# Da-Tsuchi/KLab_MultiModalModel

Measured on AMD Instinct MI355X. Metric: caption-train samples/sec (224px img, 64-tok tgt), higher is better.
Workload: dtype bf16; 1 GPU; BASELINE configs[1]: Swin-V2(C=64,(2,2,6,2),224,w7) frozen + T5-small, fwd+bwd+Adam, T5 dropout 0.1 on, random-init weights; global_batch=64, per_gpu_batch=64, src_len=9, tgt_len=64, parallelism=dp1, hipgraph=False, optimizer=klab.optim.FusedAdam (Adam update of ref/train.py:28, one kernel)

## Files before the change

### klab_multimodalmodel_amd/csrc/common.h

```cpp
#pragma once
#include <hip/hip_runtime.h>
#include <stdint.h>
#include <stdlib.h>

#define KLAB_OK 0
#define KLAB_ERR_UNSUPPORTED (-2)
#define KLAB_ERR_BADARG (-3)

#define KLAB_F32 0
#define KLAB_BF16 1

typedef __bf16 bf16_t;
typedef __attribute__((ext_vector_type(8))) __bf16 bf16x8;
typedef __attribute__((ext_vector_type(4))) __bf16 bf16x4;
typedef __attribute__((ext_vector_type(4))) float f32x4;

#define KLAB_LAUNCH_CHECK()                          \
  do {                                               \
    hipError_t e__ = hipGetLastError();              \
    if (e__ != hipSuccess) return (int)e__;          \
  } while (0)

namespace klab {

inline bool env_on(const char* name) {
  const char* v = getenv(name);
  return !v || atoi(v) != 0;
}

int ensure_dyn_lds(const void* kernel, size_t bytes);

template <typename T> struct TypeTag;
template <> struct TypeTag<float> { static constexpr int id = KLAB_F32; };
template <> struct TypeTag<bf16_t> { static constexpr int id = KLAB_BF16; };

__device__ __forceinline__ float to_f32(float x) { return x; }
__device__ __forceinline__ float to_f32(bf16_t x) { return (float)x; }
template <typename T> __device__ __forceinline__ T from_f32(float x);
template <> __device__ __forceinline__ float from_f32<float>(float x) { return x; }
template <> __device__ __forceinline__ bf16_t from_f32<bf16_t>(float x) { return (bf16_t)x; }

__device__ __forceinline__ uint32_t mix32(uint32_t x) {
  x ^= x >> 16; x *= 0x85EBCA6Bu; x ^= x >> 13; x *= 0xC2B2AE35u; x ^= x >> 16;
  return x;
}
struct DropCtx {
  uint32_t key;
  uint32_t thresh;
  float scale;
  bool on;
};
__device__ __forceinline__ DropCtx make_drop(const uint32_t* seed_dev, uint32_t tag, float p) {
  DropCtx d;
  d.on = (p > 0.f) && (seed_dev != nullptr);
  d.key = 0; d.thresh = 0; d.scale = 1.f;
  if (d.on) {
    d.key = mix32(seed_dev[0] * 0x9E3779B1u + tag * 0x7FEB352Du + 0x165667B1u);
    double t = (double)p * 4294967296.0;
    d.thresh = t >= 4294967295.0 ? 0xFFFFFFFFu : (uint32_t)t;
    d.scale = 1.f / (1.f - p);
  }
  return d;
}
__device__ __forceinline__ float drop_mult(const DropCtx& d, uint64_t idx) {
  if (!d.on) return 1.f;
  uint32_t h = mix32((uint32_t)idx * 0x9E3779B1u + d.key);
  const uint32_t hi = (uint32_t)(idx >> 32);
  if (hi) h = mix32(h ^ (hi * 0x85EBCA77u + 0x27D4EB2Fu));
  return h < d.thresh ? 0.f : d.scale;
}
__device__ __forceinline__ DropCtx drop_slab(DropCtx d, uint32_t slab) {
  if (d.on) d.key = mix32(d.key ^ (slab * 0x85EBCA77u + 0x27D4EB2Fu));
  return d;
}
__device__ __forceinline__ float drop_mult32(const DropCtx& d, uint32_t off) {
  if (!d.on) return 1.f;
  return mix32(off * 0x9E3779B1u + d.key) < d.thresh ? 0.f : d.scale;
}
__device__ __forceinline__ float drop_mult32_nb(const DropCtx& d, uint32_t off) {
  return mix32(off * 0x9E3779B1u + d.key) < d.thresh ? 0.f : d.scale;
}

__device__ __forceinline__ float wave_sum(float v) {
#pragma unroll
  for (int o = 32; o > 0; o >>= 1) v += __shfl_xor(v, o, 64);
  return v;
}
__device__ __forceinline__ float wave_max(float v) {
#pragma unroll
  for (int o = 32; o > 0; o >>= 1) v = fmaxf(v, __shfl_xor(v, o, 64));
  return v;
}
template <int G> __device__ __forceinline__ float group_sum(float v) {
#pragma unroll
  for (int o = G / 2; o > 0; o >>= 1) v += __shfl_xor(v, o, 64);
  return v;
}
template <int G> __device__ __forceinline__ float group_max(float v) {
#pragma unroll
  for (int o = G / 2; o > 0; o >>= 1) v = fmaxf(v, __shfl_xor(v, o, 64));
  return v;
}

__device__ __forceinline__ float gelu_erf(float x) { return 0.5f * x * (1.f + erff(x * 0.70710678118654752440f)); }
__device__ __forceinline__ float erf_fast(float x) {
  const float ax = fabsf(x);
  const float t = __frcp_rn(fmaf(0.3275911f, ax, 1.f));
  float pl = fmaf(1.061405429f, t, -1.453152027f);
  pl = fmaf(pl, t, 1.421413741f);
  pl = fmaf(pl, t, -0.284496736f);
  pl = fmaf(pl, t, 0.254829592f);
  const float y = 1.f - pl * t * __expf(-ax * ax);
  return copysignf(y, x);
}
typedef __attribute__((ext_vector_type(2))) float f32x2;
template <typename V> __device__ __forceinline__ V gelu_poly(V x) {
  V s = x * x;
  s = __builtin_elementwise_min(s, V(20.48f));
  V q = V(7.318504830e-11f);
  q = q * s + V(-7.769299870e-09f);
  q = q * s + V(3.614930506e-07f);
  q = q * s + V(-9.785327165e-06f);
  q = q * s + V(1.732400560e-04f);
  q = q * s + V(-2.146258019e-03f);
  q = q * s + V(1.943818480e-02f);
  q = q * s + V(-1.324543953e-01f);
  q = q * s + V(7.977233529e-01f);
  V e = __builtin_elementwise_max(__builtin_elementwise_min(x * q, V(1.f)), V(-1.f));
  const V hx = x * V(0.5f);
  return hx * e + hx;
}
template <typename T> __device__ __forceinline__ float gelu_for(float x) {
  if constexpr (sizeof(T) == 2) return gelu_poly<float>(x);
  else return gelu_erf(x);
}
__device__ __forceinline__ float gelu_erf_grad(float x) {
  float cdf = 0.5f * (1.f + erff(x * 0.70710678118654752440f));
  float pdf = 0.39894228040143267794f * __expf(-0.5f * x * x);
  return cdf + x * pdf;
}

template <typename T> struct Vec16;
template <> struct Vec16<float> { typedef f32x4 type; static constexpr int N = 4; };
template <> struct Vec16<bf16_t> { typedef bf16x8 type; static constexpr int N = 8; };

}
```

### klab_multimodalmodel_amd/csrc/engine.cpp

```cpp
#include <hip/hip_runtime.h>
#include <math.h>
#include <stdio.h>
#include <string.h>

#include <string>
#include <vector>

#include "gemm_shared.h"
#include "klab_mm.h"

namespace {

#define RC(x)                 \
  do {                        \
    int rc__ = (x);           \
    if (rc__ != 0) return rc__; \
  } while (0)

struct ParamInfo {
  std::string name;
  std::vector<long> shape;
  long numel = 0;
  long grad_off = -1;
  long warena_off = -1;
  long farena_off = -1;
};

struct T5LayerIdx { int q, k, v, o, relb, ln0, cq, ck, cv, co, ln1, wi, wi1, wo, ln2; };
struct T5Idx { int shared, lm_head = -1, head = -1; std::vector<T5LayerIdx> enc, dec; int enc_final, dec_final; };
struct SwinBlockIdx { int ls, c0w, c0b, c2w, qw, qb, kw, vw, vb, pw, pb, ln1w, ln1b, f1w, f1b, f2w, f2b, ln2w, ln2b; };
struct SwinStageIdx { std::vector<SwinBlockIdx> blk; int redw, mnw, mnb; };
struct SwinIdx { int pew, peb, penw, penb; std::vector<SwinStageIdx> st; int lnw, lnb; };

struct T5LayerBufs {
  void *xn1, *qkv, *ctx; float *lse, *rstd1;
  void *xn2, *qc, *ctx2; float *lse2, *rstd2;
  void *xn3, *hmid; float* rstd3;
  void* ab;
};
struct T5StackBufs {
  std::vector<float*> h;
  std::vector<T5LayerBufs> L;
  void* out_t = nullptr; float* rstd_f = nullptr;
  float* bias = nullptr; float* dbias = nullptr; const int* bucket = nullptr;
  int M = 0, Lseq = 0;
};
inline bool swin_attn_on_image(int C) { return C == 64 || C == 128 || C == 256; }
struct SwinBlockBufs {
  float* x_in; void* xt_in;
  void *qkv, *ctx, *po; float *lse, *mean1, *rstd1; float* h1; void* h1t;
  void *z, *a, *fo; float *mean2, *rstd2; float* h2; void* h2t;
  float *bias, *table, *hidden;
  float* btab;
  float* bimg;
  int R, w, shift, H, C; long M;
};
struct SwinStageBufs { std::vector<SwinBlockBufs> blk; void *mg, *mo; float *mmean, *mrstd; float* xm; void* xmt; };

struct Bump {
  char* base; size_t off = 0;
  explicit Bump(void* b) : base((char*)b) {}
  void* take(size_t bytes) {
    off = (off + 255) & ~(size_t)255;
    void* p = base ? base + off : nullptr;
    off += bytes;
    return p;
  }
};

struct ProcSet {
  bool on = false;
  klab_logits_proc_cfg cfg{1.f};
  std::vector<int> table;
};
struct ForcedTable {
  const long long* tok = nullptr;
  long ld = 0;
  int n = 0;
};
struct AttnMaps {
  float* p = nullptr;
  size_t bytes = 0;
};
struct GenRun {
  klab_gen_cfg cfg{};
  ProcSet lp;
  ForcedTable forced;
  AttnMaps maps;
  int cur = 0;
};

}

struct klab_engine {
  klab_model_cfg cfg;
  std::vector<ParamInfo> P[3];
  SwinIdx si; T5Idx li, mi;
  long grad_elems[3] = {0, 0, 0};
  long seg_zero_off[3] = {0, 0, 0}, seg_zero_len[3] = {0, 0, 0};
  long seg_off[3] = {0, 0, 0}, seg_len[3] = {0, 0, 0};
  long warena_elems = 0, farena_elems = 0;
  long kvall_w_off = -1, kvall_g_off = -1;
  struct Bucket { long off, len; };
  std::vector<Bucket> buckets[3];
  std::vector<hipEvent_t> bucket_ev[3];
  bool bucket_ev_live[3] = {false, false, false};
  bool bucket_events_on = false;
  int pe_k0 = 0, pe_kp = 0;
  bool bound = false;
  int B = 0, Ls = 0, Lt = 0, Le = 0, Nimg = 0;
  size_t es = 4;
  std::vector<const float*> W[3];
  float* G[3] = {nullptr, nullptr, nullptr};
  void* warena = nullptr; float* farena = nullptr;
  bool fp8 = false;
  void* w8 = nullptr; float* wscale = nullptr; void* qdesc = nullptr; int n_qdesc = 0; long q_rows = 0;
  void* x8 = nullptr; float* xscale = nullptr; long x8_bytes = 0, xscale_rows = 0;
  void* x8s = nullptr; float* xscales = nullptr; long x8s_bytes = 0, xscales_rows = 0;
  const void* q8_src[2] = {nullptr, nullptr}; int q8_rows[2] = {0, 0}, q8_k[2] = {0, 0};
  void* cast_desc = nullptr; int n_cast = 0; long cast_total4 = 0;
  void* adam_desc = nullptr; int n_adam = 0; long adam_total4 = 0, adam_split4 = 0;
  void* af_desc = nullptr; int n_af = 0; long af_totals[4] = {0, 0, 0, 0};
  float* rms_part = nullptr; long rms_part_stride = 0; float** rms_dst_dev[2] = {nullptr, nullptr}; int rms_ncalls[2] = {0, 0};
  void* cast_desc_frozen = nullptr; int n_cast_frozen = 0; long cast_total4_frozen = 0;
  bool frozen_valid = false;
  void* fcast_desc = nullptr; int n_fcast = 0; long fcast_total4 = 0;
  uint32_t* seed_dev = nullptr; int* err_dev = nullptr;
  const int *enc_bucket = nullptr, *dec_bucket = nullptr, *lang_bucket = nullptr;
  std::vector<const float*> swin_coords; std::vector<const int*> swin_index; std::vector<int> swin_ntab;
  T5StackBufs lang, enc, dec;
  GenRun gen;
  ForcedTable forced_armed;
  AttnMaps attn_armed;
  void* kv_all = nullptr; void* dkv_all = nullptr;
  void* logits = nullptr; float *loss_row = nullptr, *inv_n = nullptr, *loss = nullptr;
  float *dh_a = nullptr, *dh_b = nullptr, *dxn = nullptr, *denc = nullptr;
  void *dctx = nullptr, *ds_ws = nullptr;
  void* dh_ff = nullptr;
  std::vector<void*> dy_pool, dhmid_pool, dqkv_pool, dqc_pool;
  std::vector<hipEvent_t> evpool; int ev_next = 0;
  void *cols = nullptr, *pe_out = nullptr; float *pe_mean = nullptr, *pe_rstd = nullptr; float* x0 = nullptr; void* x0t = nullptr;
  std::vector<SwinStageBufs> sw;
  float *sw_fmean = nullptr, *sw_frstd = nullptr;
  float *sdh_a = nullptr, *sdh_b = nullptr, *sdm = nullptr; void *sdy = nullptr, *sdctx = nullptr, *sdqkv = nullptr, *sda = nullptr;
  void* sattn_ws = nullptr; size_t sattn_ws_bytes = 0;
  float *sdbias = nullptr, *sdtable = nullptr, *sdbtab = nullptr;
  long sdb_stride = 0, sdt_stride = 0; size_t sdz_bytes = 0;
  void *sdyA[2] = {nullptr, nullptr}, *sdyB[2] = {nullptr, nullptr}, *sdaP[2] = {nullptr, nullptr}, *sdqkvP[2] = {nullptr, nullptr};
  hipEvent_t swin_done_ev[2] = {nullptr, nullptr};
  hipStream_t side = nullptr; hipEvent_t ev_fork = nullptr, ev_join = nullptr;
  hipEvent_t ev_zero = nullptr;
  bool seg1_zeroed = false;
  bool dbias_zeroed[2] = {false, false};
  bool denc_in_dxn = false;
  float* loss_out = nullptr;
  bool bias_ready[3] = {false, false, false};
  bool dec_embed_ready = false;
  bool inv_n_ready = false;
  bool kv_wgrad_done = false;
  hipStream_t own = nullptr; hipEvent_t ev_in = nullptr, ev_out = nullptr;
  bool use_graph = false;
  struct GraphSlot { hipGraphExec_t exec = nullptr; int uses = 0; bool failed = false; } gs[7];
  float* pixels_buf = nullptr; long long *src_buf = nullptr, *tgt_buf = nullptr; float* dloss_buf = nullptr;
  const float* pixels_cur = nullptr;
  uint32_t seed_base = 0; bool seed_set = false;
  bool probe_on = false;
  struct Probe { std::vector<hipEvent_t> a, b; std::vector<double> flops; int n = 0; } probe[2];
  float p_train = 0.f;
  const long long* last_tgt = nullptr;
};

namespace {

int add_param(std::vector<ParamInfo>& v, const std::string& name, std::vector<long> shape) {
  ParamInfo p;
  p.name = name; p.shape = shape; p.numel = 1;
  for (long s : shape) p.numel *= s;
  v.push_back(p);
  return (int)v.size() - 1;
}

void build_t5_params(const klab_t5_cfg& c, bool encoder_only, std::vector<ParamInfo>& v, T5Idx& ix) {
  const long d = c.d_model, inner = (long)c.n_heads * c.d_kv, ff = c.d_ff;
  ix.shared = add_param(v, "shared.weight", {c.vocab, d});
  ix.lm_head = (!encoder_only && !c.tie_lm_head) ? add_param(v, "lm_head.weight", {c.vocab, d}) : -1;
  ix.head = ix.lm_head >= 0 ? ix.lm_head : ix.shared;
  auto stack = [&](const char* pre, int nl, bool dec, std::vector<T5LayerIdx>& L, int& fin) {
    for (int i = 0; i < nl; ++i) {
      T5LayerIdx l;
      memset(&l, -1, sizeof(l));
      std::string bp = std::string(pre) + "block." + std::to_string(i) + ".";
      std::string ap = bp + "layer.0.SelfAttention.";
      l.q = add_param(v, ap + "q.weight", {inner, d});
      l.k = add_param(v, ap + "k.weight", {inner, d});
      l.v = add_param(v, ap + "v.weight", {inner, d});
      l.o = add_param(v, ap + "o.weight", {d, inner});
      if (i == 0) l.relb = add_param(v, ap + "relative_attention_bias.weight", {c.rel_buckets, c.n_heads});
      l.ln0 = add_param(v, bp + "layer.0.layer_norm.weight", {d});
      int li = 1;
      if (dec) {
        std::string cp = bp + "layer.1.EncDecAttention.";
        l.cq = add_param(v, cp + "q.weight", {inner, d});
        l.ck = add_param(v, cp + "k.weight", {inner, d});
        l.cv = add_param(v, cp + "v.weight", {inner, d});
        l.co = add_param(v, cp + "o.weight", {d, inner});
        l.ln1 = add_param(v, bp + "layer.1.layer_norm.weight", {d});
        li = 2;
      }
      std::string fp = bp + "layer." + std::to_string(li) + ".";
      if (c.ffn_gated) {
        l.wi = add_param(v, fp + "DenseReluDense.wi_0.weight", {ff, d});
        l.wi1 = add_param(v, fp + "DenseReluDense.wi_1.weight", {ff, d});
      } else {
        l.wi = add_param(v, fp + "DenseReluDense.wi.weight", {ff, d});
      }
      l.wo = add_param(v, fp + "DenseReluDense.wo.weight", {d, ff});
      l.ln2 = add_param(v, fp + "layer_norm.weight", {d});
      L.push_back(l);
    }
    fin = add_param(v, std::string(pre) + "final_layer_norm.weight", {d});
  };
  if (!encoder_only) stack("decoder.", c.n_dec_layers, true, ix.dec, ix.dec_final);
  stack("encoder.", c.n_layers, false, ix.enc, ix.enc_final);
}

void build_swin_params(const klab_swin_cfg& c, std::vector<ParamInfo>& v, SwinIdx& ix) {
  const long C0 = c.embed_dim;
  ix.pew = add_param(v, "embeddings.patch_embeddings.projection.weight", {C0, c.in_ch, c.patch, c.patch});
  ix.peb = add_param(v, "embeddings.patch_embeddings.projection.bias", {C0});
  ix.penw = add_param(v, "embeddings.norm.weight", {C0});
  ix.penb = add_param(v, "embeddings.norm.bias", {C0});
  for (int s = 0; s < c.n_stages; ++s) {
    SwinStageIdx st;
    const long C = C0 << s, H = c.heads[s], F = (long)c.mlp_ratio * C;
    for (int b = 0; b < c.depths[s]; ++b) {
      SwinBlockIdx k;
      memset(&k, -1, sizeof(k));
      std::string bp = "encoder.layers." + std::to_string(s) + ".blocks." + std::to_string(b) + ".";
      std::string sp = bp + "attention.self.";
      k.ls = add_param(v, sp + "logit_scale", {H, 1, 1});
      k.c0w = add_param(v, sp + "continuous_position_bias_mlp.0.weight", {512, 2});
      k.c0b = add_param(v, sp + "continuous_position_bias_mlp.0.bias", {512});
      k.c2w = add_param(v, sp + "continuous_position_bias_mlp.2.weight", {H, 512});
      k.qw = add_param(v, sp + "query.weight", {C, C});
      if (c.qkv_bias) k.qb = add_param(v, sp + "query.bias", {C});
      k.kw = add_param(v, sp + "key.weight", {C, C});
      k.vw = add_param(v, sp + "value.weight", {C, C});
      if (c.qkv_bias) k.vb = add_param(v, sp + "value.bias", {C});
      k.pw = add_param(v, bp + "attention.output.dense.weight", {C, C});
      k.pb = add_param(v, bp + "attention.output.dense.bias", {C});
      k.ln1w = add_param(v, bp + "layernorm_before.weight", {C});
      k.ln1b = add_param(v, bp + "layernorm_before.bias", {C});
      k.f1w = add_param(v, bp + "intermediate.dense.weight", {F, C});
      k.f1b = add_param(v, bp + "intermediate.dense.bias", {F});
      k.f2w = add_param(v, bp + "output.dense.weight", {C, F});
      k.f2b = add_param(v, bp + "output.dense.bias", {C});
      k.ln2w = add_param(v, bp + "layernorm_after.weight", {C});
      k.ln2b = add_param(v, bp + "layernorm_after.bias", {C});
      st.blk.push_back(k);
    }
    st.redw = st.mnw = st.mnb = -1;
    if (s < c.n_stages - 1) {
      std::string dp = "encoder.layers." + std::to_string(s) + ".downsample.";
      st.redw = add_param(v, dp + "reduction.weight", {2 * C, 4 * C});
      st.mnw = add_param(v, dp + "norm.weight", {2 * C});
      st.mnb = add_param(v, dp + "norm.bias", {2 * C});
    }
    ix.st.push_back(st);
  }
  const long Cl = C0 << (c.n_stages - 1);
  ix.lnw = add_param(v, "layernorm.weight", {Cl});
  ix.lnb = add_param(v, "layernorm.bias", {Cl});
}

inline long pad8(long n) { return (n + 7) & ~7L; }

void plan_arenas(klab_engine* e) {
  long w = 0, f = 0;
  auto putw = [&](std::vector<ParamInfo>& v, int i) { if (i >= 0) { v[i].warena_off = w; w += (v[i].numel + 15) & ~15L; } };
  auto t5 = [&](std::vector<ParamInfo>& v, T5Idx& ix, bool is_main) {
    putw(v, ix.head);
    for (auto& l : ix.dec) { putw(v, l.q); putw(v, l.k); putw(v, l.v); putw(v, l.o); putw(v, l.cq); putw(v, l.co); putw(v, l.wi); putw(v, l.wi1); putw(v, l.wo); }
    if (is_main && !ix.dec.empty()) {
      e->kvall_w_off = w;
      for (auto& l : ix.dec) { putw(v, l.ck); putw(v, l.cv); }
    }
    for (auto& l : ix.enc) { putw(v, l.q); putw(v, l.k); putw(v, l.v); putw(v, l.o); putw(v, l.wi); putw(v, l.wi1); putw(v, l.wo); }
  };
  t5(e->P[2], e->mi, true);
  {
    auto& v = e->P[1];
    for (auto& l : e->li.enc) { putw(v, l.q); putw(v, l.k); putw(v, l.v); putw(v, l.o); putw(v, l.wi); putw(v, l.wi1); putw(v, l.wo); }
  }
  {
    auto& v = e->P[0];
    {
      const klab_swin_cfg& sc = e->cfg.swin;
      e->pe_k0 = sc.in_ch * sc.patch * sc.patch;
      e->pe_kp = (e->cfg.dtype == KLAB_BF16 && sc.patch == 4) ? ((e->pe_k0 + 31) & ~31) : e->pe_k0;
      v[e->si.pew].warena_off = w;
      w += ((long)sc.embed_dim * e->pe_kp + 15) & ~15L;
    }
    for (auto& st : e->si.st) {
      for (auto& k : st.blk) {
        putw(v, k.qw); putw(v, k.kw); putw(v, k.vw); putw(v, k.pw); putw(v, k.f1w); putw(v, k.f2w);
        const long C = v[k.qw].shape[0];
        if (k.qb >= 0) { v[k.qb].farena_off = f; v[k.vb].farena_off = f + 2 * C; }
        f += 3 * C;
      }
      putw(v, st.redw);
    }
  }
// ... 330 lines not shown
}

static bool q8_room(const Ctx& c, long M, long K, bool& side) {
  klab_engine* e = c.e;
  side = c.s == e->side;
  if (!e->fp8 || c.dt != KLAB_BF16 || !fp8_weight_ok(K)) return false;
  return M * K <= (side ? e->x8s_bytes : e->x8_bytes) && M <= (side ? e->xscales_rows : e->xscale_rows);
}
int ln_fwd_for_linear(const Ctx& c, const void* y, const float* g, const float* b, const float* shortcut, float* out, void* outt, float* mean,
                      float* rstd, int M, int C, float eps) {
  klab_engine* e = c.e;
  bool side;
  if (q8_room(c, M, C, side)) {
    RC(klab_layernorm_fwd_q8(y, g, b, shortcut, out, outt, mean, rstd, side ? e->x8s : e->x8, side ? e->xscales : e->xscale, M, C, eps, c.ws()));
    e->q8_src[side] = outt; e->q8_rows[side] = M; e->q8_k[side] = C;
    return 0;
  }
  return klab_layernorm_fwd(y, c.dt, g, b, shortcut, out, outt, c.dt, mean, rstd, M, C, eps, 0, 0, 0, 0.f, nullptr, 0, c.ws());
}
int gelu_fwd_for_linear(const Ctx& c, const void* z, void* a, int M, int F) {
  klab_engine* e = c.e;
  bool side;
  if (F <= 4096 && !(F & 7) && q8_room(c, M, F, side)) {
    RC(klab_gelu_fwd_q8(z, a, side ? e->x8s : e->x8, side ? e->xscales : e->xscale, M, F, c.ws()));
    e->q8_src[side] = a; e->q8_rows[side] = M; e->q8_k[side] = F;
    return 0;
  }
  return klab_gelu_fwd(z, a, c.dt, (long)M * F, c.ws());
}

int linear_fwd(const Ctx& c, const void* x, int M, int K, long woffv, int N, void* y, long ldy, int ydt, const float* bias = nullptr,
               int act = 0) {
  klab_gemm_args g = G0(c, M, N, K, x, K, 1, woff(c, woffv), K, 1, y, ldy, ydt);
  g.bias = bias; g.act = act;
  return fwd_gemm(c, g, woffv);
}
int linear_dgrad(const Ctx& c, const void* dy, long lddy, int M, int N, long woffv, int K, void* dx, int dxdt) {
  klab_gemm_args g = G0(c, M, K, N, dy, lddy, 1, woff(c, woffv), K, 0, dx, K, dxdt);
  return klab_gemm(&g, c.ws());
}
int linear_wgrad(const Ctx& c, const void* dy, long lddy, const void* x, long ldx, int M, int N, int K, float* dw) {
  klab_gemm_args g = G0(c, N, K, M, dy, lddy, 0, x, ldx, 0, dw, K, KLAB_F32);
  g.accumulate = 1; g.atomic_ok = 1;
  return klab_gemm(&g, c.ws());
}

int t5_sublayer_out(const Ctx& c, const void* x, int M, int K, long woffv, int d, const float* resid, float* hout, float p, uint32_t tag) {
  klab_gemm_args g = G0(c, M, d, K, x, K, 1, woff(c, woffv), K, 1, hout, d, KLAB_F32);
  g.residual = resid; g.ldr = d; g.r_dtype = KLAB_F32;
  g.drop_p = p; g.seed_dev = c.e->seed_dev; g.drop_tag = tag;
  return fwd_gemm(c, g, woffv);
}

static bool attn_fused_on() {
  static const bool on = klab::env_on("KLAB_T5_ATTN_FUSED");
  return on;
}
static bool attn_bwd_fused_on() {
  static const bool on = klab::env_on("KLAB_T5_ATTN_BWD_FUSED");
  return on;
}

int t5_stack_forward(const Ctx& c, const klab_t5_cfg& cfg, const std::vector<ParamInfo>& P, const std::vector<const float*>& W,
                     const std::vector<T5LayerIdx>& L, int final_ln, T5StackBufs& s, bool dec, int stack_id, float p, int B,
                     const void* kv_all, int Lkv, long kv_ld, float* out_f32, int grp, int grp_stride, int off, float p_final) {
  const int d = cfg.d_model, H = cfg.n_heads, dk = cfg.d_kv, inner = H * dk, ff = cfg.d_ff;
  const int M = s.M, Lq = s.Lseq;
  const int relb = L[0].relb;
  if (c.e->bias_ready[stack_id]) c.e->bias_ready[stack_id] = false;
  else RC(klab_relbias_fwd(W[relb], s.bucket, s.bias, H, Lq, Lq, c.ws()));
  int j = 0;
  for (size_t i = 0; i < L.size(); ++i) {
    const T5LayerIdx& l = L[i];
    T5LayerBufs& b = s.L[i];
    {
      klab_attn_args a;
      memset(&a, 0, sizeof(a));
      a.dtype = c.dt; a.q = b.qkv; a.ldq = 3 * inner; a.k = eoff(c, b.qkv, inner); a.ldk = 3 * inner;
      a.v = eoff(c, b.qkv, 2 * inner); a.ldv = 3 * inner; a.bias = s.bias; a.causal = dec ? 1 : 0;
      a.ctx = b.ctx; a.ldo = inner; a.lse = b.lse; a.B = B; a.H = H; a.Lq = Lq; a.Lk = Lq; a.dk = dk;
      a.drop_p = p; a.seed_dev = c.e->seed_dev; a.drop_tag = tag_of(stack_id, (int)i, SITE_PROB);
      int frc = KLAB_ERR_UNSUPPORTED;
      if (attn_fused_on() && c.dt == KLAB_BF16 && !c.e->fp8 && Lq >= 32) {
        klab_attn_fused_args fa;
        memset(&fa, 0, sizeof(fa));
        fa.x = s.h[j]; fa.gamma = W[l.ln0]; fa.eps = cfg.ln_eps; fa.d_model = d; fa.w = woff(c, P[l.q].warena_off);
        fa.xn = b.xn1; fa.rstd = b.rstd1; fa.proj = b.qkv; fa.ldproj = 3 * inner; fa.cross = 0; fa.attn = a;
        frc = klab_t5_attn_fused_fwd(&fa, c.ws());
        if (frc != 0 && frc != KLAB_ERR_UNSUPPORTED) return frc;
      }
      if (frc != 0) {
        RC(rms_fwd_for_linear(c, s.h[j], W[l.ln0], b.xn1, b.rstd1, M, d, cfg.ln_eps));
        RC(linear_fwd(c, b.xn1, M, d, P[l.q].warena_off, 3 * inner, b.qkv, 3 * inner, c.dt));
        RC(klab_t5_attn_fwd(&a, c.ws()));
      }
    }
    RC(t5_sublayer_out(c, b.ctx, M, inner, P[l.o].warena_off, d, s.h[j], s.h[j + 1], p, tag_of(stack_id, (int)i, SITE_ATTN_OUT)));
    ++j;
    if (dec) {
      klab_attn_args a;
      memset(&a, 0, sizeof(a));
      a.dtype = c.dt; a.q = b.qc; a.ldq = inner;
      a.k = eoff(c, (void*)kv_all, (long)i * 2 * inner); a.ldk = kv_ld;
      a.v = eoff(c, (void*)kv_all, (long)i * 2 * inner + inner); a.ldv = kv_ld;
      a.bias = nullptr; a.causal = 0; a.ctx = b.ctx2; a.ldo = inner; a.lse = b.lse2;
      a.B = B; a.H = H; a.Lq = Lq; a.Lk = Lkv; a.dk = dk;
      a.drop_p = p; a.seed_dev = c.e->seed_dev; a.drop_tag = tag_of(stack_id, (int)i, SITE_XPROB);
      int frc = KLAB_ERR_UNSUPPORTED;
      if (attn_fused_on() && c.dt == KLAB_BF16 && !c.e->fp8 && Lq >= 32) {
        klab_attn_fused_args fa;
        memset(&fa, 0, sizeof(fa));
        fa.x = s.h[j]; fa.gamma = W[l.ln1]; fa.eps = cfg.ln_eps; fa.d_model = d; fa.w = woff(c, P[l.cq].warena_off);
        fa.xn = b.xn2; fa.rstd = b.rstd2; fa.proj = b.qc; fa.ldproj = inner; fa.cross = 1; fa.attn = a;
        frc = klab_t5_attn_fused_fwd(&fa, c.ws());
        if (frc != 0 && frc != KLAB_ERR_UNSUPPORTED) return frc;
      }
      if (frc != 0) {
        RC(rms_fwd_for_linear(c, s.h[j], W[l.ln1], b.xn2, b.rstd2, M, d, cfg.ln_eps));
        RC(linear_fwd(c, b.xn2, M, d, P[l.cq].warena_off, inner, b.qc, inner, c.dt));
        RC(klab_t5_attn_fwd(&a, c.ws()));
      }
      RC(t5_sublayer_out(c, b.ctx2, M, inner, P[l.co].warena_off, d, s.h[j], s.h[j + 1], p, tag_of(stack_id, (int)i, SITE_XOUT)));
      ++j;
    }
    RC(rms_fwd_for_linear(c, s.h[j], W[l.ln2], b.xn3, b.rstd3, M, d, cfg.ln_eps));
    if (cfg.ffn_gated) {
      RC(linear_fwd(c, b.xn3, M, d, P[l.wi].warena_off, 2 * ff, b.ab, 2 * ff, c.dt));
      RC(klab_geglu_fwd(b.ab, 2 * ff, b.hmid, ff, c.dt, M, ff, p, c.e->seed_dev, tag_of(stack_id, (int)i, SITE_MID), c.ws()));
    } else {
      klab_gemm_args g = G0(c, M, ff, d, b.xn3, d, 1, woff(c, P[l.wi].warena_off), d, 1, b.hmid, ff, c.dt);
      g.act = KLAB_ACT_RELU; g.drop_p = p; g.seed_dev = c.e->seed_dev; g.drop_tag = tag_of(stack_id, (int)i, SITE_MID);
      RC(fwd_gemm(c, g, P[l.wi].warena_off));
    }
    RC(t5_sublayer_out(c, b.hmid, M, ff, P[l.wo].warena_off, d, s.h[j], s.h[j + 1], p, tag_of(stack_id, (int)i, SITE_FFN_OUT)));
    ++j;
  }
  RC(klab_rmsnorm_fwd(s.h[j], W[final_ln], out_f32 ? nullptr : s.out_t, c.dt, out_f32, s.rstd_f, M, d, cfg.ln_eps, grp, grp_stride, off,
                      p_final, c.e->seed_dev, out_f32 ? tag_of(STACK_ENC, 0, SITE_IN) : tag_of(stack_id, 0, SITE_FINAL), c.ws()));
  return 0;
}

int side_after_main(const Ctx& c) {
  klab_engine* e = c.e;
  hipEvent_t ev = e->evpool[e->ev_next++ % e->evpool.size()];
  RC((int)hipEventRecord(ev, c.s));
  return (int)hipStreamWaitEvent(e->side, ev, 0);
}
int main_after_side(const Ctx& c) {
  klab_engine* e = c.e;
  hipEvent_t ev = e->evpool[e->ev_next++ % e->evpool.size()];
  RC((int)hipEventRecord(ev, e->side));
  return (int)hipStreamWaitEvent(c.s, ev, 0);
}
struct PendingWgrad { const void* dy; long lddy; const void* x; long ldx; int M, N, K; float* dw; };
struct WgradQueue {
  std::vector<PendingWgrad> q;
  int layers = 0;
  void push(const void* dy, long lddy, const void* x, long ldx, int M, int N, int K, float* dw) { q.push_back({dy, lddy, x, ldx, M, N, K, dw}); }
  int flush(const Ctx& c, bool now = true, bool* launched = nullptr) {
    if (launched) *launched = false;
    ++layers;
    if (q.empty()) { layers = 0; return 0; }
    if (!now && q.size() + 8 <= 32) return 0;
    if (launched) *launched = true;
    const bool large = layers >= 2;
    layers = 0;
    RC(side_after_main(c));
    Ctx cs{c.e, c.e->side, c.dt, c.es};
    std::vector<klab_gemm_args> gs;
    gs.reserve(q.size());
    for (const PendingWgrad& w : q) {
      klab_gemm_args g = G0(cs, w.N, w.K, w.M, w.dy, w.lddy, 0, w.x, w.ldx, 0, w.dw, w.K, KLAB_F32);
      g.accumulate = 1; g.atomic_ok = 1;
      gs.push_back(g);
    }
    klab_engine::Probe& pr = c.e->probe[1];
    const bool probe = c.e->probe_on && pr.n < (int)pr.a.size();
    if (probe) { klab::tl_launch_probe.a = pr.a[pr.n]; klab::tl_launch_probe.b = pr.b[pr.n]; }
    const int grc = klab_gemm_grouped_tiles(gs.data(), (int)gs.size(), large ? 1 : 0, cs.ws());
    RC(grc);
    if (probe) {
      if (klab::tl_launch_probe.a) klab::tl_launch_probe.a = nullptr;
      else {
        double fl = 0;
        for (const PendingWgrad& w : q) fl += 2.0 * w.M * (double)w.N * w.K;
        pr.flops[pr.n++] = fl;
      }
    }
    q.clear();
    return 0;
  }
};

int t5_stack_backward(const Ctx& c, const klab_t5_cfg& cfg, const std::vector<ParamInfo>& P, const std::vector<const float*>& W,
                      float* Gflat, const std::vector<T5LayerIdx>& L, int final_ln, T5StackBufs& s, bool dec, int stack_id, float p,
                      int B, const void* kv_all, void* dkv_all, int Lkv, long kv_ld, float** dh_out) {
  klab_engine* e = c.e;
  const int d = cfg.d_model, H = cfg.n_heads, dk = cfg.d_kv, inner = H * dk, ff = cfg.d_ff;
  const int M = s.M, Lq = s.Lseq;
  const int nsub = dec ? 3 : 2;
  int j = nsub * (int)L.size();
  float* dh_cur = e->dh_a;
  float* dh_oth = e->dh_b;
  auto G = [&](int pi) { return Gflat + P[pi].grad_off; };
  const float inv_keep = p > 0.f ? 1.f / (1.f - p) : 1.f;
  int dy_i = 0, deferred = 0;
  WgradQueue wq;
  const int stk = dec ? 1 : 0;
  const bool part_ok = Gflat == e->G[2] && e->rms_part && d <= 1024 && (long)klab_rmsnorm_part_rows(M) * d <= e->rms_part_stride;
  int rms_calls = 0;
  auto rms_bwd = [&](const float* dyin, const float* x, const float* w, const float* rstd, const float* dres, float* dx, void* dxt, int pidx,
                     float p_y, uint32_t tag_y, float p_prev, uint32_t tag_prev) -> int {
    if (part_ok)
      return klab_rmsnorm_bwd_part(dyin, x, w, rstd, dres, dx, dxt, c.dt, e->rms_part + (long)(rms_calls++) * e->rms_part_stride, M, d, 0, 0, 0,
                                   p_y, tag_y, p_prev, tag_prev, e->seed_dev, c.ws());
    return klab_rmsnorm_bwd(dyin, x, w, rstd, dres, dx, dxt, c.dt, G(pidx), M, d, 0, 0, 0, p_y, tag_y, p_prev, tag_prev, e->seed_dev, c.ws());
  };
  auto next_dy = [&]() { return e->dy_pool[dy_i++ % e->dy_pool.size()]; };
  if (e->dbias_zeroed[stk]) e->dbias_zeroed[stk] = false;
  else RC(hipMemsetAsync(s.dbias, 0, (size_t)H * Lq * Lq * 4, c.s));
  void* dy = next_dy();
  bool dctx_ready = false;
  auto attn_bwd = [&](klab_attn_args& a, long wo_off) -> int {
    if (attn_bwd_fused_on() && c.dt == KLAB_BF16) {
      klab_attn_bwd_fused_args fb;
      memset(&fb, 0, sizeof(fb));
      fb.dy = dy; fb.lddy = d; fb.w = woff(c, wo_off); fb.d_model = d; fb.attn = a;
      const int frc = klab_t5_attn_bwd_fused(&fb, c.ws());
      if (frc != KLAB_ERR_UNSUPPORTED) return frc;
    }
    if (!dctx_ready) { RC(linear_dgrad(c, dy, d, M, d, wo_off, inner, e->dctx, c.dt)); dctx_ready = true; }
    return klab_t5_attn_bwd(&a, c.ws());
  };
  RC(rms_bwd(e->dxn, s.h[j], W[final_ln], s.rstd_f, nullptr, dh_cur, dy, final_ln, p, tag_of(stack_id, 0, SITE_FINAL), p,
             tag_of(stack_id, (int)L.size() - 1, SITE_FFN_OUT)));
  std::vector<int> pending_buckets;
  const int Ln = (int)L.size();
  std::vector<char> flush_at(Ln, 1);
  constexpr int GROUP_TILES = 90;
  static const bool group_on = klab::env_on("KLAB_WGRAD_GROUP_TILES");
  const bool kv_in_queue = dec && dkv_all && Gflat == e->G[2] && !e->use_graph && e->kvall_g_off >= 0;
  if (group_on && Ln >= 3 && Gflat == e->G[2] && !e->use_graph) {
    auto T2 = [](int n, int k) { return (long)((n + 255) / 256) * ((k + 255) / 256); };
    const long tl = T2(d, ff) + T2(cfg.ffn_gated ? 2 * ff : ff, d) + T2(d, inner) + T2(3 * inner, d) + (dec ? T2(d, inner) + T2(inner, d) + (kv_in_queue ? T2(2 * inner, d) : 0) : 0);
    const int per_group = (int)((GROUP_TILES + tl - 1) / tl), per_layer = dec ? 7 : 4;
    if (per_group >= 2) {
      const int body = Ln - 1;
      int ng = body / per_group;
      if (ng < 1) ng = 1;
      if (((body + ng - 1) / ng) * per_layer <= 32) {
        std::fill(flush_at.begin(), flush_at.end(), 0);
        int i = Ln - 1;
        for (int gi = 0; gi < ng; ++gi) { i -= body / ng + (gi < body % ng ? 1 : 0); flush_at[i + 1] = 1; }
        flush_at[0] = 1;
      }
    }
  }
  for (int i = (int)L.size() - 1; i >= 0; --i) {
    const T5LayerIdx& l = L[i];
    T5LayerBufs& b = s.L[i];
    void* dhmid = e->dhmid_pool[i];
    void* dqkv = e->dqkv_pool[i];
    --j;
    wq.push(dy, d, b.hmid, ff, M, d, ff, G(l.wo));
    if (cfg.ffn_gated) {
      RC(linear_dgrad(c, dy, d, M, d, P[l.wo].warena_off, ff, e->dh_ff, c.dt));
      RC(klab_geglu_bwd(e->dh_ff, ff, b.ab, 2 * ff, dhmid, 2 * ff, c.dt, M, ff, p, e->seed_dev, tag_of(stack_id, i, SITE_MID), c.ws()));
      wq.push(dhmid, 2 * ff, b.xn3, d, M, 2 * ff, d, G(l.wi));
      RC(linear_dgrad(c, dhmid, 2 * ff, M, 2 * ff, P[l.wi].warena_off, d, e->dxn, KLAB_F32));
    } else {
      {
        klab_gemm_args g = G0(c, M, ff, d, dy, d, 1, woff(c, P[l.wo].warena_off), ff, 0, dhmid, ff, c.dt);
        g.aux = b.hmid; g.ldaux = ff; g.aux_mode = KLAB_AUX_NONZERO; g.aux_scale = inv_keep;
        RC(klab_gemm(&g, c.ws()));
      }
      wq.push(dhmid, ff, b.xn3, d, M, ff, d, G(l.wi));
      RC(linear_dgrad(c, dhmid, ff, M, ff, P[l.wi].warena_off, d, e->dxn, KLAB_F32));
    }
    {
      const uint32_t tprev = dec ? tag_of(stack_id, i, SITE_XOUT) : tag_of(stack_id, i, SITE_ATTN_OUT);
      dy = next_dy();
      RC(rms_bwd(e->dxn, s.h[j], W[l.ln2], b.rstd3, dh_cur, dh_oth, dy, l.ln2, 0.f, 0, p, tprev));
      float* t = dh_cur; dh_cur = dh_oth; dh_oth = t;
    }
    if (dec) {
      --j;
      void* dqc = e->dqc_pool[i];
      wq.push(dy, d, b.ctx2, inner, M, d, inner, G(l.co));
      dctx_ready = false;
      klab_attn_args a;
      memset(&a, 0, sizeof(a));
      a.dtype = c.dt; a.q = b.qc; a.ldq = inner;
      a.k = eoff(c, (void*)kv_all, (long)i * 2 * inner); a.ldk = kv_ld;
      a.v = eoff(c, (void*)kv_all, (long)i * 2 * inner + inner); a.ldv = kv_ld;
      a.ctx = b.ctx2; a.ldo = inner; a.lse = b.lse2; a.B = B; a.H = H; a.Lq = Lq; a.Lk = Lkv; a.dk = dk;
      a.drop_p = p; a.seed_dev = e->seed_dev; a.drop_tag = tag_of(stack_id, i, SITE_XPROB);
      a.dctx = e->dctx; a.lddo = inner; a.dq = dqc; a.lddq = inner;
      a.dk_out = eoff(c, dkv_all, (long)i * 2 * inner); a.lddk = kv_ld;
      a.dv = eoff(c, dkv_all, (long)i * 2 * inner + inner); a.lddv = kv_ld;
      RC(attn_bwd(a, P[l.co].warena_off));
      if (kv_in_queue) {
        wq.push(eoff(c, dkv_all, (long)i * 2 * inner), kv_ld, e->enc.out_t, d, B * Lkv, 2 * inner, d, Gflat + e->kvall_g_off + (long)i * 2 * inner * d);
        e->kv_wgrad_done = true;
      }
      wq.push(dqc, inner, b.xn2, d, M, inner, d, G(l.cq));
      RC(linear_dgrad(c, dqc, inner, M, inner, P[l.cq].warena_off, d, e->dxn, KLAB_F32));
      dy = next_dy();
      RC(rms_bwd(e->dxn, s.h[j], W[l.ln1], b.rstd2, dh_cur, dh_oth, dy, l.ln1, 0.f, 0, p, tag_of(stack_id, i, SITE_ATTN_OUT)));
      float* t = dh_cur; dh_cur = dh_oth; dh_oth = t;
    }
    --j;
    wq.push(dy, d, b.ctx, inner, M, d, inner, G(l.o));
    dctx_ready = false;
    {
      klab_attn_args a;
      memset(&a, 0, sizeof(a));
      a.dtype = c.dt; a.q = b.qkv; a.ldq = 3 * inner; a.k = eoff(c, b.qkv, inner); a.ldk = 3 * inner;
      a.v = eoff(c, b.qkv, 2 * inner); a.ldv = 3 * inner; a.bias = s.bias; a.causal = dec ? 1 : 0;
      a.ctx = b.ctx; a.ldo = inner; a.lse = b.lse; a.B = B; a.H = H; a.Lq = Lq; a.Lk = Lq; a.dk = dk;
      a.drop_p = p; a.seed_dev = e->seed_dev; a.drop_tag = tag_of(stack_id, i, SITE_PROB);
      a.dctx = e->dctx; a.lddo = inner; a.dq = dqkv; a.lddq = 3 * inner;
      a.dk_out = eoff(c, dqkv, inner); a.lddk = 3 * inner; a.dv = eoff(c, dqkv, 2 * inner); a.lddv = 3 * inner;
      a.dbias = s.dbias;
      int arc = KLAB_ERR_UNSUPPORTED;
      if (c.dt == KLAB_BF16 && deferred == (int)L.size() - 1 - i) {
        a.ds_defer = 1;
        a.ds_ws = (char*)e->ds_ws + (size_t)deferred * B * H * Lq * ((Lq + 31) & ~31) * c.es;
        arc = attn_bwd(a, P[l.o].warena_off);
        if (arc == 0) ++deferred;
      }
      if (arc == KLAB_ERR_UNSUPPORTED) { a.ds_defer = 0; a.ds_ws = nullptr; arc = attn_bwd(a, P[l.o].warena_off); }
      RC(arc);
    }
    wq.push(dqkv, 3 * inner, b.xn1, d, M, 3 * inner, d, G(l.q));
    RC(linear_dgrad(c, dqkv, 3 * inner, M, 3 * inner, P[l.q].warena_off, d, e->dxn, KLAB_F32));
    {
      const bool first = (i == 0);
      if (!first) dy = next_dy();
      RC(rms_bwd(e->dxn, s.h[j], W[l.ln0], b.rstd1, dh_cur, dh_oth, first ? nullptr : dy, l.ln0, 0.f, 0, first ? 0.f : p,
                 first ? 0u : tag_of(stack_id, i - 1, SITE_FFN_OUT)));
      float* t = dh_cur; dh_cur = dh_oth; dh_oth = t;
    }
    bool launched = false;
    RC(wq.flush(c, flush_at[i] != 0, &launched));
    pending_buckets.push_back((int)L.size() - 1 - i);
    if (launched) {
      const int seg = dec ? 0 : 1;
      for (int bi : pending_buckets)
        if (e->bucket_events_on && Gflat == e->G[2] && !e->use_graph && bi < (int)e->bucket_ev[seg].size())
          RC((int)hipEventRecord(e->bucket_ev[seg][bi], e->side));
      pending_buckets.clear();
      if (i == 0 && e->bucket_events_on && Gflat == e->G[2] && !e->use_graph && (int)L.size() - 1 < (int)e->bucket_ev[seg].size())
        e->bucket_ev_live[seg] = true;
    }
  }
  if (part_ok && rms_calls) {
    if (rms_calls != e->rms_ncalls[stk]) return KLAB_ERR_BADARG;
    RC(klab_colpart_reduce(e->rms_part, e->rms_part_stride, klab_rmsnorm_part_rows(M), d, e->rms_dst_dev[stk], rms_calls, c.ws()));
  }
  if (deferred) RC(klab_dbias_reduce(e->ds_ws, c.dt, s.dbias, deferred * B, H, Lq, Lq, c.ws()));
  RC(klab_relbias_bwd(s.dbias, s.bucket, G(L[0].relb), H, Lq, Lq, cfg.rel_buckets, c.ws()));
  *dh_out = dh_cur;
  return 0;
}

int swin_forward(const Ctx& c, const float* pixels, float p_in, bool refresh_bias) {
  klab_engine* e = c.e;
  const klab_swin_cfg& s = e->cfg.swin;
  const auto& P = e->P[0];
  const auto& W = e->W[0];
  const int B = e->B, R0 = s.image_size / s.patch, K0 = s.in_ch * s.patch * s.patch, C0 = s.embed_dim;
  const long M0 = (long)B * R0 * R0;
  const int Kp = e->pe_kp;
  (void)K0;
  static const bool fused_pe = klab::env_on("KLAB_SWIN_FUSED_EMBED");
  int perc = KLAB_ERR_UNSUPPORTED;
  if (!e->cfg.train_swin && fused_pe && !e->fp8 && Kp >= 64)
    perc = klab_swin_patch_embed_fused(pixels, woff(c, P[e->si.pew].warena_off), Kp, W[e->si.peb], W[e->si.penw], W[e->si.penb], e->x0, e->x0t, c.dt,
                                       B, s.in_ch, s.image_size, s.patch, C0, s.ln_eps, c.ws());
  if (perc != 0 && perc != KLAB_ERR_UNSUPPORTED) return perc;
  if (perc != 0) {
  RC(klab_im2col_patch_ld(pixels, e->cols, c.dt, B, s.in_ch, s.image_size, s.patch, Kp, c.ws()));
  {
    klab_gemm_args g = G0(c, (int)M0, C0, Kp, e->cols, Kp, 1, woff(c, P[e->si.pew].warena_off), Kp, 1, e->pe_out, C0, c.dt);
    g.bias = W[e->si.peb];
    RC(klab_gemm(&g, c.ws()));
  }
  RC(klab_layernorm_fwd(e->pe_out, c.dt, W[e->si.penw], W[e->si.penb], nullptr, e->x0, e->x0t, c.dt, e->pe_mean, e->pe_rstd, (int)M0, C0,
                        s.ln_eps, 0, 0, 0, 0.f, nullptr, 0, c.ws()));
  }
  float* x = e->x0;
  void* xt = e->x0t;
  long bias_off = 0;
  for (int st = 0; st < s.n_stages; ++st) {
    SwinStageBufs& sb = e->sw[st];
    for (size_t k = 0; k < sb.blk.size(); ++k) {
      SwinBlockBufs& q = sb.blk[k];
      const SwinBlockIdx& ix = e->si.st[st].blk[k];
      const int C = q.C, M = (int)q.M, F = s.mlp_ratio * C, n = q.w * q.w;
      q.x_in = x; q.xt_in = xt;
      if (refresh_bias) {
        if (q.btab)
          RC(klab_swin_cpb_table(e->swin_coords[st], W[ix.c0w], W[ix.c0b], W[ix.c2w], q.table, q.hidden, q.btab, e->swin_ntab[st], q.H, 512,
                                 c.ws()));
        else
          RC(klab_swin_cpb_bias(e->swin_coords[st], e->swin_index[st], W[ix.c0w], W[ix.c0b], W[ix.c2w], q.table, q.hidden, q.bias,
                                e->swin_ntab[st], n, q.H, 512, c.ws()));
        if (q.bimg) RC(klab_swin_bias_image(q.bias, q.bimg, q.R, q.w, q.shift, q.H, c.ws()));
      }
      const float* qkvb = ix.qb >= 0 ? e->farena + bias_off : nullptr;
      bias_off += 3 * C;
      int qrc = KLAB_ERR_UNSUPPORTED;
      if (q.bimg)
        qrc = klab_swin_qkv_attn_fused_img(xt, woff(c, P[ix.qw].warena_off), qkvb, q.ctx, q.bimg, W[ix.ls], c.dt, B, q.R, q.w, q.shift, q.H, C,
                                           c.ws());
      else if (!e->cfg.train_swin && q.bias)
        qrc = klab_swin_qkv_attn_fused(xt, woff(c, P[ix.qw].warena_off), qkvb, q.ctx, q.bias, W[ix.ls], c.dt, B, q.R, q.w, q.shift, q.H, C,
                                       c.ws());
      if (qrc != 0 && qrc != KLAB_ERR_UNSUPPORTED) return qrc;
      if (qrc != 0) {
        RC(linear_fwd(c, xt, M, C, P[ix.qw].warena_off, 3 * C, q.qkv, 3 * C, c.dt, qkvb));
        klab_swin_attn_args a;
        memset(&a, 0, sizeof(a));
        a.dtype = c.dt; a.qkv = q.qkv; a.ctx = q.ctx; a.bias = q.bias; a.bias_table = q.btab; a.logit_scale = W[ix.ls]; a.lse = q.lse;
        a.B = B; a.R = q.R; a.w = q.w; a.shift = q.shift; a.H = q.H; a.C = C;
        a.bwd_ws = e->sattn_ws; a.bwd_ws_bytes = e->sattn_ws_bytes;
        a.v_bias = qkvb ? qkvb + 2 * C : nullptr;
        RC(klab_swin_attn_fwd(&a, c.ws()));
      }
      int prc = KLAB_ERR_UNSUPPORTED;
      if (!e->cfg.train_swin)
        prc = klab_swin_proj_ln_fused(q.ctx, x, woff(c, P[ix.pw].warena_off), W[ix.pb], W[ix.ln1w], W[ix.ln1b], q.h1, q.h1t, c.dt, M, C, s.ln_eps,
                                      c.ws());
      if (prc != 0 && prc != KLAB_ERR_UNSUPPORTED) return prc;
      static const bool fused_lin_ln = klab::env_on("KLAB_SWIN_FUSED_LIN_LN");
      const bool wide_ln = !e->cfg.train_swin && !e->fp8 && fused_lin_ln;
      if (prc != 0 && wide_ln) {
        prc = klab_swin_linear_ln_fused(q.ctx, x, woff(c, P[ix.pw].warena_off), W[ix.pb], W[ix.ln1w], W[ix.ln1b], q.h1, q.h1t, c.dt, M, C, C,
                                        s.ln_eps, c.ws());
        if (prc != 0 && prc != KLAB_ERR_UNSUPPORTED) return prc;
      }
      if (prc != 0) {
        RC(linear_fwd(c, q.ctx, M, C, P[ix.pw].warena_off, C, q.po, C, c.dt, W[ix.pb]));
        RC(ln_fwd_for_linear(c, q.po, W[ix.ln1w], W[ix.ln1b], x, q.h1, q.h1t, q.mean1, q.rstd1, M, C, s.ln_eps));
      }
      if (e->cfg.train_swin) {
        RC(linear_fwd(c, q.h1t, M, C, P[ix.f1w].warena_off, F, q.z, F, c.dt, W[ix.f1b]));
        RC(gelu_fwd_for_linear(c, q.z, q.a, M, F));
      } else {
        const int frc = klab_swin_mlp_fused(q.h1t, q.h1, woff(c, P[ix.f1w].warena_off), W[ix.f1b], woff(c, P[ix.f2w].warena_off), W[ix.f2b],
                                            W[ix.ln2w], W[ix.ln2b], q.h2, q.h2t, c.dt, M, C, s.ln_eps, c.ws());
        if (frc == 0) { x = q.h2; xt = q.h2t; continue; }
        if (frc != KLAB_ERR_UNSUPPORTED) return frc;
        RC(linear_fwd(c, q.h1t, M, C, P[ix.f1w].warena_off, F, q.a, F, c.dt, W[ix.f1b], KLAB_ACT_GELU));
      }
      int f2rc = KLAB_ERR_UNSUPPORTED;
      if (wide_ln)
        f2rc = klab_swin_linear_ln_fused(q.a, q.h1, woff(c, P[ix.f2w].warena_off), W[ix.f2b], W[ix.ln2w], W[ix.ln2b], q.h2, q.h2t, c.dt, M, F, C,
                                         s.ln_eps, c.ws());
      if (f2rc != 0 && f2rc != KLAB_ERR_UNSUPPORTED) return f2rc;
      if (f2rc != 0) {
        RC(linear_fwd(c, q.a, M, F, P[ix.f2w].warena_off, C, q.fo, C, c.dt, W[ix.f2b]));
        RC(ln_fwd_for_linear(c, q.fo, W[ix.ln2w], W[ix.ln2b], q.h1, q.h2, q.h2t, q.mean2, q.rstd2, M, C, s.ln_eps));
      }
      x = q.h2; xt = q.h2t;
    }
    if (st < s.n_stages - 1) {
      const int R = R0 >> st, C = C0 << st;
      const long M2 = (long)B * (R / 2) * (R / 2);
      RC(klab_merge_gather(x, sb.mg, c.dt, B, R, C, c.ws()));
      RC(linear_fwd(c, sb.mg, (int)M2, 4 * C, P[e->si.st[st].redw].warena_off, 2 * C, sb.mo, 2 * C, c.dt));
      RC(klab_layernorm_fwd(sb.mo, c.dt, W[e->si.st[st].mnw], W[e->si.st[st].mnb], nullptr, sb.xm, sb.xmt, c.dt, sb.mmean, sb.mrstd, (int)M2,
                            2 * C, s.ln_eps, 0, 0, 0, 0.f, nullptr, 0, c.ws()));
      x = sb.xm; xt = sb.xmt;
    }
  }
  const int Cl = C0 << (s.n_stages - 1);
  RC(klab_layernorm_fwd(x, KLAB_F32, W[e->si.lnw], W[e->si.lnb], nullptr, e->enc.h[0], nullptr, c.dt, e->sw_fmean, e->sw_frstd,
                        B * e->Nimg, Cl, s.ln_eps, e->Nimg, e->Le, 0, p_in, e->seed_dev, tag_of(STACK_ENC, 0, SITE_IN), c.ws()));
  return 0;
}

int swin_backward(const Ctx& c, const float* dh0, float p_in);

}

extern "C" int klab_sizeof_t5_cfg(void) { return (int)sizeof(klab_t5_cfg); }
// ... 32 lines not shown
}

extern "C" void klab_engine_destroy(klab_engine* e) {
  if (!e) return;
  drain_engine(e);
  for (auto& g : e->gs) if (g.exec) { hipGraphExecDestroy(g.exec); g.exec = nullptr; }
  if (e->ev_fork) hipEventDestroy(e->ev_fork);
  if (e->ev_join) hipEventDestroy(e->ev_join);
  if (e->ev_zero) hipEventDestroy(e->ev_zero);
  if (e->ev_in) hipEventDestroy(e->ev_in);
  if (e->ev_out) hipEventDestroy(e->ev_out);
  for (auto ev : e->evpool) if (ev) hipEventDestroy(ev);
  for (auto& v : e->bucket_ev) for (auto ev : v) if (ev) hipEventDestroy(ev);
  for (auto ev : e->swin_done_ev) if (ev) hipEventDestroy(ev);
  for (auto& pr : e->probe) {
    for (auto ev : pr.a) if (ev) hipEventDestroy(ev);
    for (auto ev : pr.b) if (ev) hipEventDestroy(ev);
  }
  if (e->side) hipStreamDestroy(e->side);
  if (e->own) hipStreamDestroy(e->own);
  delete e;
}

extern "C" int klab_engine_num_params(const klab_engine* e, int model) {
  if (!e || model < 0 || model > 2) return -1;
  return (int)e->P[model].size();
}

extern "C" int klab_engine_param_info(const klab_engine* e, int model, int i, char* name, int name_cap, long* shape4, int* ndim,
                                      long* grad_off) {
  if (!e || model < 0 || model > 2 || i < 0 || i >= (int)e->P[model].size()) return KLAB_ERR_BADARG;
  const ParamInfo& p = e->P[model][i];
  if (name && name_cap > 0) { strncpy(name, p.name.c_str(), name_cap - 1); name[name_cap - 1] = 0; }
  if (ndim) *ndim = (int)p.shape.size();
  if (shape4) for (size_t k = 0; k < 4; ++k) shape4[k] = k < p.shape.size() ? p.shape[k] : 1;
  if (grad_off) *grad_off = p.grad_off;
  return 0;
}

extern "C" long klab_engine_grad_elems(const klab_engine* e, int model) { return (e && model >= 0 && model <= 2) ? e->grad_elems[model] : -1; }

extern "C" int klab_engine_segment(const klab_engine* e, int seg, int* model, long* off, long* len) {
  if (!e || seg < 0 || seg > 2) return KLAB_ERR_BADARG;
  if (model) *model = seg == 2 ? 0 : 2;
  if (off) *off = e->seg_off[seg];
  if (len) *len = e->seg_len[seg];
  return 0;
}

extern "C" int klab_engine_num_buckets(const klab_engine* e, int segment) {
  if (!e || segment < 0 || segment > 2) return -1;
  return (int)e->buckets[segment].size();
}
extern "C" int klab_engine_bucket(const klab_engine* e, int segment, int i, long* off, long* len) {
  if (!e || segment < 0 || segment > 2 || i < 0 || i >= (int)e->buckets[segment].size()) return KLAB_ERR_BADARG;
  if (off) *off = e->buckets[segment][i].off;
  if (len) *len = e->buckets[segment][i].len;
  return KLAB_OK;
}
extern "C" int klab_engine_set_bucket_events(klab_engine* e, int on) {
  if (!e) return KLAB_ERR_BADARG;
  e->bucket_events_on = on != 0;
  if (!on) for (auto& b : e->bucket_ev_live) b = false;
  return KLAB_OK;
}
extern "C" int klab_engine_bucket_wait(klab_engine* e, int segment, int i, void* stream) {
  if (!e || !e->bound || segment < 0 || segment > 2 || i < 0 || i >= (int)e->bucket_ev[segment].size()) return KLAB_ERR_BADARG;
  if (!e->bucket_ev_live[segment]) return KLAB_ERR_UNSUPPORTED;
  return (int)hipStreamWaitEvent((hipStream_t)stream, e->bucket_ev[segment][i], 0);
}

extern "C" size_t klab_engine_workspace_bytes(klab_engine* e, int B, int Ls, int Lt) {
  if (!e || B <= 0 || Ls <= 0 || Lt <= 0) return 0;
  klab_engine tmp;
  tmp.cfg = e->cfg;
  for (int m = 0; m < 3; ++m) tmp.P[m].resize(e->P[m].size());
  tmp.warena_elems = e->warena_elems; tmp.farena_elems = e->farena_elems; tmp.fp8 = e->fp8;
  return plan_workspace(&tmp, nullptr, B, Ls, Lt);
}

extern "C" int klab_engine_bind(klab_engine* e, int B, int Ls, int Lt, void* workspace, size_t ws_bytes, const void* const* swin_params,
                                const void* const* lang_params, const void* const* main_params, float* main_grads, float* swin_grads,
                                const int* lang_bucket, const int* enc_bucket, const int* dec_bucket, const void* const* swin_coords,
                                const void* const* swin_index, void* stream) {
  if (!e || !workspace || !swin_params || !lang_params || !main_params || !main_grads) return KLAB_ERR_BADARG;
  if (e->cfg.train_swin && !swin_grads) return KLAB_ERR_BADARG;
  uint32_t carry[3] = {0, 0, 0};
  bool carry_rng = false;
  if (e->bound) {
    e->bound = false;
    drain_engine(e);
    if (e->seed_set && e->seed_dev) carry_rng = hipMemcpy(carry, e->seed_dev, sizeof(carry), hipMemcpyDeviceToHost) == hipSuccess;
  }
  const size_t need = plan_workspace(e, workspace, B, Ls, Lt);
  if (need > ws_bytes) return KLAB_ERR_BADARG;
  const void* const* src[3] = {swin_params, lang_params, main_params};
  for (int m = 0; m < 3; ++m) {
    e->W[m].resize(e->P[m].size());
    for (size_t i = 0; i < e->P[m].size(); ++i) {
      e->W[m][i] = (const float*)src[m][i];
      if (!e->W[m][i]) return KLAB_ERR_BADARG;
    }
  }
  e->G[0] = swin_grads; e->G[2] = main_grads;
  e->lang_bucket = lang_bucket; e->enc_bucket = enc_bucket; e->dec_bucket = dec_bucket;
  e->lang.bucket = lang_bucket; e->enc.bucket = enc_bucket; e->dec.bucket = dec_bucket;
  const klab_swin_cfg& s = e->cfg.swin;
  e->swin_coords.resize(s.n_stages); e->swin_index.resize(s.n_stages); e->swin_ntab.resize(s.n_stages);
  const int R0 = s.image_size / s.patch;
  for (int st = 0; st < s.n_stages; ++st) {
    e->swin_coords[st] = (const float*)swin_coords[st];
    e->swin_index[st] = (const int*)swin_index[st];
    const int R = R0 >> st, w = R < s.window ? R : s.window;
    if (w <= 0) return KLAB_ERR_UNSUPPORTED;
    e->swin_ntab[st] = (2 * w - 1) * (2 * w - 1);
  }
  hipStream_t hs = (hipStream_t)stream;
  for (int grp = 0; grp < 2; ++grp) {
    std::vector<long> d;
    long pre = 0; int n = 0;
    for (int m = 0; m < 3; ++m) {
      const bool frozen = (m == 1) || (m == 0 && !e->cfg.train_swin);
      if (frozen != (grp == 1)) continue;
      for (size_t i = 0; i < e->P[m].size(); ++i) {
        const ParamInfo& p = e->P[m][i];
        if (p.warena_off < 0) continue;
        if (p.numel % 4) return KLAB_ERR_UNSUPPORTED;
        if (m == 0 && (int)i == e->si.pew && e->pe_kp != e->pe_k0) {
          if (e->pe_k0 % 4) return KLAB_ERR_UNSUPPORTED;
          for (int r = 0; r < e->cfg.swin.embed_dim; ++r) {
            d.push_back((long)(e->W[m][i] + (long)r * e->pe_k0)); d.push_back(p.warena_off + (long)r * e->pe_kp); d.push_back(pre);
            pre += e->pe_k0 / 4; ++n;
          }
          continue;
        }
        d.push_back((long)e->W[m][i]); d.push_back(p.warena_off); d.push_back(pre);
        pre += p.numel / 4; ++n;
      }
    }
    const size_t grp_cap = e->P[0].size() + e->P[1].size() + e->P[2].size() + e->cfg.swin.embed_dim + 1;
    void* dst = grp == 0 ? e->cast_desc : (void*)((char*)e->cast_desc + sizeof(long) * 3 * grp_cap);
    if (grp == 1) { e->cast_desc_frozen = dst; e->n_cast_frozen = n; e->cast_total4_frozen = pre; }
    if (n == 0) { if (grp == 0) { e->n_cast = 0; e->cast_total4 = 0; } continue; }
    hipError_t er0 = hipMemcpyAsync(dst, d.data(), d.size() * sizeof(long), hipMemcpyHostToDevice, hs);
    if (er0 != hipSuccess) return (int)er0;
    er0 = hipStreamSynchronize(hs);
    if (er0 != hipSuccess) return (int)er0;
    if (grp == 1) continue;
    e->n_cast = n; e->cast_total4 = pre;
  }
  e->frozen_valid = false;
  e->seg1_zeroed = e->dbias_zeroed[0] = e->dbias_zeroed[1] = e->denc_in_dxn = false;
  e->bias_ready[0] = e->bias_ready[1] = e->bias_ready[2] = e->dec_embed_ready = e->inv_n_ready = e->kv_wgrad_done = false;
  e->loss_out = nullptr;
  e->forced_armed = ForcedTable();
  e->attn_armed = AttnMaps();
  e->gen.maps = AttnMaps();
  if (e->pe_kp != e->pe_k0)
    RC((int)hipMemsetAsync((char*)e->warena + (size_t)e->P[0][e->si.pew].warena_off * e->es, 0,
                           (size_t)e->cfg.swin.embed_dim * e->pe_kp * e->es, hs));
  {
    std::vector<long> d;
    long pre = 0; int n = 0;
    for (size_t i = 0; i < e->P[0].size(); ++i) {
      const ParamInfo& p = e->P[0][i];
      if (p.farena_off < 0) continue;
      if (p.numel % 4) return KLAB_ERR_UNSUPPORTED;
      d.push_back((long)e->W[0][i]); d.push_back(p.farena_off); d.push_back(pre);
      pre += p.numel / 4; ++n;
    }
    e->n_fcast = n; e->fcast_total4 = pre;
    RC((int)hipMemsetAsync(e->farena, 0, (size_t)e->farena_elems * 4, hs));
    if (n) {
      hipError_t er = hipMemcpyAsync(e->fcast_desc, d.data(), d.size() * sizeof(long), hipMemcpyHostToDevice, hs);
      if (er != hipSuccess) return (int)er;
      er = hipStreamSynchronize(hs);
      if (er != hipSuccess) return (int)er;
    }
  }
  if (e->fp8) {
    std::vector<long> d;
    long row0 = 0; int n = 0;
    for (int m = 0; m < 3; ++m)
      for (size_t i = 0; i < e->P[m].size(); ++i) {
        const ParamInfo& p = e->P[m][i];
        if (p.warena_off < 0 || p.shape.empty() || (m == 0 && (int)i == e->si.pew)) continue;
        const long rows = p.shape[0], K = p.numel / rows;
        if (!fp8_weight_ok(K) || (p.warena_off & 15)) continue;
        d.push_back(p.warena_off); d.push_back(rows); d.push_back(K); d.push_back(row0);
        row0 += rows; ++n;
      }
    e->n_qdesc = n; e->q_rows = row0;
    if (n) {
      hipError_t er = hipMemcpyAsync(e->qdesc, d.data(), d.size() * sizeof(long), hipMemcpyHostToDevice, hs);
      if (er != hipSuccess) return (int)er;
      er = hipStreamSynchronize(hs);
      if (er != hipSuccess) return (int)er;
    }
  }
  std::vector<long> adam_tab;
  {
    std::vector<long> d;
    long pre = 0; int n = 0;
    bool ok = true;
    for (int seg = 0; seg < 2 && ok; ++seg) {
      if (seg == 1) e->adam_split4 = pre;
      for (size_t i = 0; i < e->P[2].size(); ++i) {
        const ParamInfo& p = e->P[2][i];
        if (p.grad_off < 0 || (p.grad_off >= e->seg_off[1]) != (seg == 1)) continue;
        if (p.numel % 4 || (p.grad_off & 3) || (p.warena_off >= 0 && (p.warena_off & 3))) { ok = false; break; }
        d.push_back((long)e->W[2][i]); d.push_back(p.grad_off); d.push_back(p.warena_off); d.push_back(pre);
        pre += p.numel / 4; ++n;
      }
    }
    e->n_adam = ok ? n : 0; e->adam_total4 = pre;
    if (e->n_adam) {
      hipError_t er = hipMemcpyAsync(e->adam_desc, d.data(), d.size() * sizeof(long), hipMemcpyHostToDevice, hs);
      if (er != hipSuccess) return (int)er;
    }
    adam_tab.swap(d);
  }
  {
    std::vector<long> rows, cols, idx;
    std::vector<int> fact;
    for (int seg = 0; seg < 2; ++seg)
      for (size_t i = 0; i < e->P[2].size(); ++i) {
        const ParamInfo& p = e->P[2][i];
        if (p.grad_off < 0 || (p.grad_off >= e->seg_off[1]) != (seg == 1)) continue;
        const long c = p.shape.empty() ? 1 : p.shape.back();
        fact.push_back(p.shape.size() >= 2); rows.push_back(p.shape.size() >= 2 ? p.numel / c : 1);
        cols.push_back(p.shape.size() >= 2 ? c : p.numel); idx.push_back((long)i);
      }
    const int n = (int)idx.size();
    std::vector<long> plan((size_t)n * 4), d;
    e->n_af = 0;
    if (e->n_adam == n && n > 0 && klab_adafactor_plan(n, rows.data(), cols.data(), fact.data(), plan.data(), e->af_totals) == KLAB_OK) {
      for (int k = 0; k < n; ++k) {
        const ParamInfo& p = e->P[2][idx[k]];
        const long v[10] = {(long)e->W[2][idx[k]], p.grad_off, p.warena_off, rows[k], cols[k], plan[k * 4 + 0], plan[k * 4 + 1],
                            plan[k * 4 + 2], plan[k * 4 + 3], (long)fact[k]};
        d.insert(d.end(), v, v + 10);
      }
      hipError_t er = hipMemcpyAsync(e->af_desc, d.data(), d.size() * sizeof(long), hipMemcpyHostToDevice, hs);
      if (er != hipSuccess) return (int)er;
      e->n_af = n;
    }
    if (e->n_adam) {
      hipError_t er = hipStreamSynchronize(hs);
      if (er != hipSuccess) return (int)er;
    }
  }
  for (int st = 0; st < 2; ++st) {
    const bool dec = st == 1;
    const auto& L = dec ? e->mi.dec : e->mi.enc;
    std::vector<float*> dst;
    float* Gm = e->G[2];
    dst.push_back(Gm + e->P[2][dec ? e->mi.dec_final : e->mi.enc_final].grad_off);
    for (int i = (int)L.size() - 1; i >= 0; --i) {
      dst.push_back(Gm + e->P[2][L[i].ln2].grad_off);
      if (dec) dst.push_back(Gm + e->P[2][L[i].ln1].grad_off);
      dst.push_back(Gm + e->P[2][L[i].ln0].grad_off);
    }
    e->rms_ncalls[st] = (int)dst.size();
    hipError_t er = hipMemcpyAsync(e->rms_dst_dev[st], dst.data(), dst.size() * sizeof(float*), hipMemcpyHostToDevice, hs);
    if (er != hipSuccess) return (int)er;
    er = hipStreamSynchronize(hs);
    if (er != hipSuccess) return (int)er;
  }
  RC((int)hipMemsetAsync(e->seed_dev, 0, 512, hs));
  for (auto& g : e->gs) {
    if (g.exec) hipGraphExecDestroy(g.exec);
    g = klab_engine::GraphSlot();
  }
  e->seed_set = false;
  if (carry_rng) {
    RC((int)hipMemcpyAsync(e->seed_dev, carry, sizeof(carry), hipMemcpyHostToDevice, hs));
    RC((int)hipStreamSynchronize(hs));
    e->seed_set = true;
  }
  if (!e->side) {
    RC((int)hipStreamCreateWithFlags(&e->side, hipStreamNonBlocking));
    RC((int)hipEventCreateWithFlags(&e->ev_fork, hipEventDisableTiming));
    RC((int)hipEventCreateWithFlags(&e->ev_join, hipEventDisableTiming));
    RC((int)hipEventCreateWithFlags(&e->ev_zero, hipEventDisableTiming));
    RC((int)hipStreamCreateWithFlags(&e->own, hipStreamNonBlocking));
    e->evpool.resize(256);
    for (auto& ev : e->evpool) RC((int)hipEventCreateWithFlags(&ev, hipEventDisableTiming));
    RC((int)hipEventCreateWithFlags(&e->ev_in, hipEventDisableTiming));
    RC((int)hipEventCreateWithFlags(&e->ev_out, hipEventDisableTiming));
    for (auto& ev : e->swin_done_ev) RC((int)hipEventCreateWithFlags(&ev, hipEventDisableTiming));
    for (int sg = 0; sg < 3; ++sg) {
      e->bucket_ev[sg].assign(e->buckets[sg].size(), nullptr);
      for (auto& ev : e->bucket_ev[sg]) RC((int)hipEventCreateWithFlags(&ev, hipEventDisableTiming));
    }
  }
  for (int sg = 0; sg < 3; ++sg) e->bucket_ev_live[sg] = false;
  e->bound = true;
  return 0;
}

namespace {

__global__ void seed_set_kernel(uint32_t* st, uint32_t base) { st[1] = base; st[2] = 0; }
__global__ void seed_restore_kernel(uint32_t* st, uint32_t base, uint32_t counter) { st[1] = base; st[2] = counter; }
__global__ void seed_step_kernel(uint32_t* st) {
  const uint32_t n = st[2] + 1;
// ... 521 lines not shown
  e->forced_armed.tok = tokens_dev; e->forced_armed.ld = ld; e->forced_armed.n = n_forced;
  return 0;
}

static size_t gen_attn_bytes(const klab_engine* e, const klab_gen_cfg& g) {
  if (g.mode == KLAB_GEN_BEAM) return 0;
  return (size_t)e->cfg.main.n_dec_layers * e->B * g.n * g.max_length * e->Le * sizeof(float);
}

extern "C" size_t klab_engine_gen_attn_bytes(klab_engine* e, const klab_gen_cfg* cfg) {
  ProcSet lp;
  if (!e || !cfg || make_procs(e, cfg->procs, lp) || !gen_shape_ok(e, *cfg, lp)) return 0;
  return gen_attn_bytes(e, *cfg);
}

extern "C" int klab_engine_gen_set_attn(klab_engine* e, float* maps_dev, size_t bytes, void* stream) {
  (void)stream;
  if (!e) return KLAB_ERR_BADARG;
  e->attn_armed = AttnMaps();
  if (!maps_dev && bytes == 0) return 0;
  if (!maps_dev || bytes == 0) return KLAB_ERR_BADARG;
  e->attn_armed.p = maps_dev; e->attn_armed.bytes = bytes;
  return 0;
}

extern "C" int klab_engine_gen_begin(klab_engine* e, const klab_gen_cfg* cfg, void* ws, void* stream) {
  if (!e) return KLAB_ERR_BADARG;
  const ForcedTable forced = e->forced_armed;
  e->forced_armed = ForcedTable();
  const AttnMaps maps = e->attn_armed;
  e->attn_armed = AttnMaps();
  if (!cfg || !ws) return KLAB_ERR_BADARG;
  ProcSet lp;
  RC(make_procs(e, cfg->procs, lp));
  if (!gen_shape_ok(e, *cfg, lp)) return KLAB_ERR_BADARG;
  if (maps.p && (cfg->mode == KLAB_GEN_BEAM || maps.bytes < gen_attn_bytes(e, *cfg))) return KLAB_ERR_BADARG;
  if (cfg->mode == KLAB_GEN_FORCE ? forced.n < cfg->max_length - 1
                                  : forced.n > 0 && (cfg->mode == KLAB_GEN_BEAM || forced.n > cfg->max_length - 1 || cfg->want_logprobs))
    return KLAB_ERR_BADARG;
  GenRun& g = e->gen;
  g.cfg = *cfg; g.cfg.procs = nullptr;
  g.lp = std::move(lp);
  g.forced = forced;
  g.maps = maps;
  g.cur = 0;
  Ctx c{e, (hipStream_t)stream, e->cfg.dtype, e->es};
  const klab_t5_cfg& mc = e->cfg.main;
  const int n = g.cfg.n, Lm = g.cfg.max_length, B = e->B, inner = mc.n_heads * mc.d_kv;
  GenWs w;
  plan_gen(e, g.cfg, g.lp, ws, w);
  if (!g.lp.table.empty()) RC((int)hipMemcpyAsync(w.table, g.lp.table.data(), g.lp.table.size() * 4, hipMemcpyHostToDevice, c.s));
  if (g.cfg.mode == KLAB_GEN_BEAM) {
    klab_beam_update_args a = beam_args(e, w, 1);
    RC(klab_beam_init(&a, mc.start_id, g.cfg.pad_id, c.ws()));
  } else {
    RC((int)hipMemsetAsync(w.done, 0, (size_t)B * n * 4, c.s));
    RC((int)hipMemsetAsync(w.stop, 0, (size_t)Lm * 4, c.s));
    if (w.logprob) RC((int)hipMemsetAsync(w.logprob, 0, (size_t)B * n * Lm * 4, c.s));
  }
  for (int i = 0; i < mc.n_dec_layers; ++i)
    RC(klab_beam_copy_rows((int)e->es, e->dec.L[i].qkv, (long)e->Lt * 3 * inner, n, eoff(c, w.rows.cache, (long)i * w.rows.cache_layer),
                           (long)Lm * 3 * inner, B * n, 3 * inner, c.ws()));
  if (g.maps.p) {
    const int Le = e->Le;
    const long kv_ld = (long)mc.n_dec_layers * 2 * inner;
    RC((int)hipMemsetAsync(g.maps.p, 0, gen_attn_bytes(e, g.cfg), c.s));
    for (int i = 0; i < mc.n_dec_layers; ++i)
      RC(klab_t5_decode_attn_map(c.dt, e->dec.L[i].qc, (long)e->Lt * inner, n, eoff(c, e->kv_all, (long)i * 2 * inner), (long)Le * kv_ld,
                                 kv_ld, n, nullptr, 0, w.done, g.maps.p + (((long)i * B * n * Lm) + 1) * Le, (long)Lm * Le, B * n,
                                 mc.n_heads, Le, mc.d_kv, c.ws()));
  }
  RC(gen_pos(e, c, w, e->logits, (long)e->Lt * mc.vocab, n, 1));
  g.cur = 1;
  return 0;
}

extern "C" int klab_engine_gen_step(klab_engine* e, int t, void* ws, void* stream) {
  if (!e || !ws) return KLAB_ERR_BADARG;
  GenRun& g = e->gen;
  if (g.cur < 1 || t != g.cur || t > g.cfg.max_length - 2 || !gen_shape_ok(e, g.cfg, g.lp)) return KLAB_ERR_BADARG;
  Ctx c{e, (hipStream_t)stream, e->cfg.dtype, e->es};
  GenWs w;
  plan_gen(e, g.cfg, g.lp, ws, w);
  DecodeRows r = w.rows;
  if (g.cfg.mode == KLAB_GEN_BEAM) r.kv_slot = w.slot[t & 1];
  if (g.maps.p) { r.maps = g.maps.p; r.done = w.done; }
  RC(decode_rows(e, c, t, w.prev, r));
  RC(gen_pos(e, c, w, r.logits, e->cfg.main.vocab, 1, t + 1));
  g.cur = t + 1;
  return 0;
}

extern "C" const int* klab_engine_gen_stop_word(klab_engine* e, void* ws, int pos) {
  if (!e || !ws || e->gen.cur < 1 || pos < 1 || pos >= e->gen.cfg.max_length) return nullptr;
  GenWs w;
  plan_gen(e, e->gen.cfg, e->gen.lp, ws, w);
  return w.stop + pos;
}

extern "C" const void* klab_engine_gen_buffer(klab_engine* e, void* ws, const char* name, long* rows, long* cols, int* dtype) {
  if (!e || !ws || !name || e->gen.cur < 1) return nullptr;
  GenWs w;
  plan_gen(e, e->gen.cfg, e->gen.lp, ws, w);
  if (rows) *rows = w.rows.M;
  if (!strcmp(name, "logits")) {
    if (cols) *cols = e->cfg.main.vocab;
    if (dtype) *dtype = e->cfg.dtype;
    return w.rows.logits;
  }
  if (!strcmp(name, "tokens")) {
    if (cols) *cols = 1;
    return w.prev;
  }
  if (!strcmp(name, "logprobs") && w.logprob) {
    if (cols) *cols = e->gen.cfg.max_length;
    if (dtype) *dtype = KLAB_F32;
    return w.logprob;
  }
  return nullptr;
}

extern "C" int klab_engine_gen_result(klab_engine* e, void* ws, int n, int length, long long* seq, float* scores, int* len, void* stream) {
  if (!e || !ws || e->gen.cur < 1 || !seq) return KLAB_ERR_BADARG;
  const klab_gen_cfg& g = e->gen.cfg;
  GenWs w;
  plan_gen(e, g, e->gen.lp, ws, w);
  const size_t Lm = g.max_length, k = g.n, B = e->B;
  hipStream_t s = (hipStream_t)stream;
  if (g.mode != KLAB_GEN_BEAM) {
    if (n != g.n || length < 1 || length > e->gen.cur + 1) return KLAB_ERR_BADARG;
    return (int)hipMemcpy2DAsync(seq, (size_t)length * 8, w.seq, Lm * 8, (size_t)length * 8, B * k, hipMemcpyDeviceToDevice, s);
  }
  if (n < 1 || n > g.n || length != g.max_length || !scores || !len) return KLAB_ERR_BADARG;
  hipError_t rc = hipMemcpy2DAsync(seq, n * Lm * 8, w.fin_seq[e->gen.cur & 1], k * Lm * 8, n * Lm * 8, B, hipMemcpyDeviceToDevice, s);
  if (rc == hipSuccess) rc = hipMemcpy2DAsync(scores, n * 4, w.fin_score, k * 4, n * 4, B, hipMemcpyDeviceToDevice, s);
  if (rc == hipSuccess) rc = hipMemcpy2DAsync(len, n * 4, w.fin_len, k * 4, n * 4, B, hipMemcpyDeviceToDevice, s);
  return (int)rc;
}

extern "C" int klab_engine_gen_scores(klab_engine* e, void* ws, int length, int n_out, float length_penalty, float* token_logprobs,
                                      float* score, int* len, int* order, void* stream) {
  if (!e || !ws || e->gen.cur < 1 || !e->gen.cfg.want_logprobs || !score || !len) return KLAB_ERR_BADARG;
  const klab_gen_cfg& g = e->gen.cfg;
  if (length < 2 || length > e->gen.cur + 1) return KLAB_ERR_BADARG;
  GenWs w;
  plan_gen(e, g, e->gen.lp, ws, w);
  const size_t Lm = g.max_length;
  RC(klab_gen_finalize(w.logprob, (long)Lm, w.seq, (long)Lm, e->B, g.n, length, g.eos_id, length_penalty, n_out, score, len, order, stream));
  if (!token_logprobs) return 0;
  return (int)hipMemcpy2DAsync(token_logprobs, (size_t)length * 4, w.logprob, Lm * 4, (size_t)length * 4, (size_t)e->B * g.n,
                               hipMemcpyDeviceToDevice, (hipStream_t)stream);
}

static int backward_segment(klab_engine* e, int segment, const float* dloss_dev, void* stream) {
  Ctx c{e, (hipStream_t)stream, e->cfg.dtype, e->es};
  const klab_model_cfg& cfg = e->cfg;
  const int B = e->B, d = cfg.main.d_model, inner = cfg.main.n_heads * cfg.main.d_kv, nld = cfg.main.n_dec_layers;
  const float p = e->p_train;
  float* Gm = e->G[2];
  e->bucket_ev_live[segment] = false;
  if (segment == 0) {
    e->ev_next = 0;
    const int Md = B * e->Lt, V = cfg.main.vocab;
    const float alpha = cfg.main.scale_decoder_outputs ? 1.f / sqrtf((float)d) : 1.f;
    Ctx cs{e, e->side, c.dt, c.es};
    static const bool zero_side = klab::env_on("KLAB_ZERO_ON_SIDE");
    const bool zside = zero_side && !e->use_graph;
    if (zside) {
      RC(side_after_main(c));
      RC((int)hipMemsetAsync(Gm + e->seg_off[0], 0, (size_t)e->seg_len[0] * 4, e->side));
      RC((int)hipMemsetAsync(Gm + e->seg_off[1], 0, (size_t)e->seg_len[1] * 4, e->side));
      RC((int)hipMemsetAsync(e->dec.dbias, 0, (size_t)cfg.main.n_heads * e->Lt * e->Lt * 4, e->side));
      RC((int)hipMemsetAsync(e->enc.dbias, 0, (size_t)cfg.main.n_heads * e->Le * e->Le * 4, e->side));
      RC((int)hipEventRecord(e->ev_zero, e->side));
      e->seg1_zeroed = e->dbias_zeroed[0] = e->dbias_zeroed[1] = true;
    } else {
      RC((int)hipMemsetAsync(Gm + e->seg_off[0], 0, (size_t)e->seg_len[0] * 4, c.s));
    }
    {
      RC((int)hipMemsetAsync(e->dxn, 0, (size_t)Md * d * 4, c.s));
      klab_gemm_args g = G0(c, Md, d, V, e->logits, V, 1, woff(c, e->P[2][e->mi.head].warena_off), d, 0, e->dxn, d, KLAB_F32);
      g.alpha = alpha; g.alpha_dev = dloss_dev; g.accumulate = 1; g.atomic_ok = 1;
      RC(klab_gemm(&g, c.ws()));
    }
    if (zside) RC((int)hipStreamWaitEvent(c.s, e->ev_zero, 0));
    RC(side_after_main(c));
    {
      klab_gemm_args g = G0(cs, V, d, Md, e->logits, V, 0, e->dec.out_t, d, 0, Gm + e->P[2][e->mi.head].grad_off, d, KLAB_F32);
      g.alpha = alpha; g.alpha_dev = dloss_dev; g.accumulate = 1; g.atomic_ok = 1;
      RC(klab_gemm(&g, cs.ws()));
    }
    float* dh0 = nullptr;
    RC(t5_stack_backward(c, cfg.main, e->P[2], e->W[2], Gm, e->mi.dec, e->mi.dec_final, e->dec, true, STACK_DEC, p, B, e->kv_all, e->dkv_all,
                         e->Le, (long)nld * 2 * inner, &dh0));
    RC(side_after_main(c));
    RC(klab_embed_bwd(e->last_tgt, 1, e->Lt, cfg.main.start_id, cfg.main.pad_id, dh0, Gm + e->P[2][e->mi.shared].grad_off, V, Md, d, p,
                      e->seed_dev, tag_of(STACK_DEC, 0, SITE_IN), cs.ws()));
    const int Me = B * e->Le, Nkv = nld * 2 * inner;
    if (e->kv_wgrad_done) e->kv_wgrad_done = false;
    else RC(linear_wgrad(cs, e->dkv_all, Nkv, e->enc.out_t, d, Me, Nkv, d, Gm + e->kvall_g_off));
    e->denc_in_dxn = !e->use_graph;
    RC(linear_dgrad(c, e->dkv_all, Nkv, Me, Nkv, e->kvall_w_off, d, e->denc_in_dxn ? e->dxn : e->denc, KLAB_F32));
    return main_after_side(c);
  }
  if (segment == 1) {
    e->ev_next = 0;
    if (e->seg1_zeroed) e->seg1_zeroed = false;
    else RC((int)hipMemsetAsync(Gm + e->seg_off[1], 0, (size_t)e->seg_len[1] * 4, c.s));
    const int Me = B * e->Le;
    if (e->denc_in_dxn) e->denc_in_dxn = false;
    else RC((int)hipMemcpyAsync(e->dxn, e->denc, (size_t)Me * d * 4, hipMemcpyDeviceToDevice, c.s));
    float* dh0 = nullptr;
    RC(t5_stack_backward(c, cfg.main, e->P[2], e->W[2], Gm, e->mi.enc, e->mi.enc_final, e->enc, false, STACK_ENC, p, B, nullptr, nullptr, 0, 0,
                         &dh0));
    if (cfg.train_swin) RC((int)hipMemcpyAsync(e->denc, dh0, (size_t)Me * d * 4, hipMemcpyDeviceToDevice, c.s));
    return main_after_side(c);
  }
  if (segment == 2) {
    if (!cfg.train_swin) return 0;
    return swin_backward(c, e->denc, p);
  }
  return KLAB_ERR_BADARG;
}


extern "C" int klab_engine_backward(klab_engine* e, int segment, const float* dloss_dev, void* stream) {
  if (!e || !e->bound || segment < 0 || segment > 2) return KLAB_ERR_BADARG;
  int erc = 0;
  const hipStream_t s = enter_stream(e, (hipStream_t)stream, erc);
  if (erc) return erc;
  const float* dl = e->dloss_buf;
  if (segment == 0) {
    if (dloss_dev && !e->use_graph) dl = dloss_dev;
    else if (dloss_dev) RC((int)hipMemcpyAsync(e->dloss_buf, dloss_dev, 4, hipMemcpyDeviceToDevice, s));
    else { static const float one = 1.f; RC((int)hipMemcpyAsync(e->dloss_buf, &one, 4, hipMemcpyHostToDevice, s)); }
  }
  RC(run_graphed(e, 4 + segment, s, [&]() { return backward_segment(e, segment, dl, (void*)s); }));
  return leave_stream(e, (hipStream_t)stream, s);
}

namespace {

int swin_backward(const Ctx& c, const float* dh0, float p_in) {
  klab_engine* e = c.e;
  const klab_swin_cfg& s = e->cfg.swin;
  const auto& P = e->P[0];
  const auto& W = e->W[0];
  float* Gs = e->G[0];
  auto G = [&](int pi) { return Gs + P[pi].grad_off; };
  const int B = e->B, R0 = s.image_size / s.patch, C0 = s.embed_dim;
  RC((int)hipMemsetAsync(Gs + e->seg_off[2], 0, (size_t)e->seg_len[2] * 4, c.s));
  RC((int)hipMemsetAsync(e->sdbias, 0, e->sdz_bytes, c.s));
  const int last = s.n_stages - 1;
  const int Cl = C0 << last;
  const SwinStageBufs& lsb = e->sw[last];
  const float* xlast = lsb.blk.empty() ? (last > 0 ? e->sw[last - 1].xm : e->x0) : lsb.blk.back().h2;
  float* dh = e->sdh_a;
  float* dh2 = e->sdh_b;
  RC(klab_layernorm_bwd(dh0, xlast, KLAB_F32, W[e->si.lnw], e->sw_fmean, e->sw_frstd, dh, G(e->si.lnw), G(e->si.lnb), B * e->Nimg, Cl,
                        e->Nimg, e->Le, 0, p_in, e->seed_dev, tag_of(STACK_ENC, 0, SITE_IN), c.ws()));
  long bias_off_total = 0;
  for (int st = 0; st < s.n_stages; ++st) bias_off_total += 3L * (C0 << st) * s.depths[st];
  long bias_off = bias_off_total;
  (void)bias_off;
  int swin_bucket = 0, blk_no = 0;
  const bool side_on = e->sdyA[0] != nullptr;
  const Ctx cs{e, e->side, c.dt, c.es};
  for (int st = last; st >= 0; --st) {
    SwinStageBufs& sb = e->sw[st];
    const int R = R0 >> st, C = C0 << st;
    if (st < last) {
      const long M2 = (long)B * (R / 2) * (R / 2);
      RC(klab_layernorm_bwd(dh, sb.mo, c.dt, W[e->si.st[st].mnw], sb.mmean, sb.mrstd, e->sdy, G(e->si.st[st].mnw), G(e->si.st[st].mnb), (int)M2,
                            2 * C, 0, 0, 0, 0.f, nullptr, 0, c.ws()));
      RC(linear_wgrad(c, e->sdy, 2 * C, sb.mg, 4 * C, (int)M2, 2 * C, 4 * C, G(e->si.st[st].redw)));
      RC(linear_dgrad(c, e->sdy, 2 * C, (int)M2, 2 * C, P[e->si.st[st].redw].warena_off, 4 * C, e->sdm, KLAB_F32));
      RC(klab_merge_scatter(e->sdm, dh2, B, R, C, c.ws()));
      float* t = dh; dh = dh2; dh2 = t;
    }
    for (int k = (int)sb.blk.size() - 1; k >= 0; --k) {
      SwinBlockBufs& q = sb.blk[k];
      const SwinBlockIdx& ix = e->si.st[st].blk[k];
      const int M = (int)q.M, F = s.mlp_ratio * C, n = q.w * q.w;
      const int par = blk_no & 1;
      if (side_on && blk_no >= 2) RC((int)hipStreamWaitEvent(c.s, e->swin_done_ev[par], 0));
      void* dyA = side_on ? e->sdyA[par] : e->sdy;
      void* dyB = side_on ? e->sdyB[par] : e->sdy;
      void* da = side_on ? e->sdaP[par] : e->sda;
      void* dqkv = side_on ? e->sdqkvP[par] : e->sdqkv;
      const Ctx& cw = side_on ? cs : c;
      RC(klab_layernorm_bwd_bias(dh, q.fo, c.dt, W[ix.ln2w], q.mean2, q.rstd2, dyA, G(ix.ln2w), G(ix.ln2b), G(ix.f2b), M, C, 0, 0, 0, 0.f, nullptr,
                                 0, c.ws()));
      if (!side_on) RC(linear_wgrad(c, dyA, C, q.a, F, M, C, F, G(ix.f2w)));
      {
        klab_gemm_args g = G0(c, M, F, C, dyA, C, 1, woff(c, P[ix.f2w].warena_off), F, 0, da, F, c.dt);
        g.aux = q.z; g.ldaux = F; g.aux_mode = KLAB_AUX_DGELU;
        RC(klab_gemm(&g, c.ws()));
      }
      if (!side_on) {
        RC(klab_colsum(da, F, c.dt, M, F, G(ix.f1b), c.ws()));
        RC(linear_wgrad(c, da, F, q.h1t, C, M, F, C, G(ix.f1w)));
      }
      {
        klab_gemm_args g = G0(c, M, C, F, da, F, 1, woff(c, P[ix.f1w].warena_off), C, 0, dh, C, KLAB_F32);
        g.accumulate = 1;
        RC(klab_gemm(&g, c.ws()));
      }
      RC(klab_layernorm_bwd_bias(dh, q.po, c.dt, W[ix.ln1w], q.mean1, q.rstd1, dyB, G(ix.ln1w), G(ix.ln1b), G(ix.pb), M, C, 0, 0, 0, 0.f, nullptr,
                                 0, c.ws()));
      if (!side_on) RC(linear_wgrad(c, dyB, C, q.ctx, C, M, C, C, G(ix.pw)));
      RC(linear_dgrad(c, dyB, C, M, C, P[ix.pw].warena_off, C, e->sdctx, c.dt));
      klab_swin_attn_args a;
      memset(&a, 0, sizeof(a));
      a.dtype = c.dt; a.qkv = q.qkv; a.ctx = q.ctx; a.bias = q.bias; a.bias_table = q.btab; a.logit_scale = W[ix.ls]; a.lse = q.lse;
      a.B = B; a.R = q.R; a.w = q.w; a.shift = q.shift; a.H = q.H; a.C = C;
      a.dctx = e->sdctx; a.dqkv = dqkv; a.dlogit_scale = G(ix.ls);
      a.bwd_ws = e->sattn_ws; a.bwd_ws_bytes = e->sattn_ws_bytes;
      if (ix.vb >= 0) { a.v_bias = e->farena + P[ix.vb].farena_off; a.dv_bias = G(ix.vb); }
      float* blk_dbias = e->sdbias + blk_no * e->sdb_stride;
      float* blk_dbtab = e->sdbtab + blk_no * e->sdt_stride;
      float* blk_dtable = e->sdtable + blk_no * e->sdt_stride;
      if (q.btab) {
        a.dbias_table = blk_dbtab;
        RC(klab_swin_attn_bwd(&a, c.ws()));
        RC(klab_swin_cpb_table_bwd(blk_dbtab, q.btab, e->swin_coords[st], q.hidden, W[ix.c2w], blk_dtable, G(ix.c0w), G(ix.c0b), G(ix.c2w),
                                   e->swin_ntab[st], q.H, 512, c.ws()));
      } else {
        a.dbias = blk_dbias;
        RC(klab_swin_attn_bwd(&a, c.ws()));
        RC(klab_swin_cpb_bias_bwd_pz(blk_dbias, q.bias, e->swin_index[st], e->swin_coords[st], q.hidden, W[ix.c0w], W[ix.c2w], blk_dtable,
                                     G(ix.c0w), G(ix.c0b), G(ix.c2w), e->swin_ntab[st], n, q.H, 512, 1, c.ws()));
      }
      if (side_on) {
        RC(side_after_main(c));
        RC(klab_colsum(da, F, c.dt, M, F, G(ix.f1b), cw.ws()));
      }
      if (ix.qb >= 0) {
        RC(klab_colsum(dqkv, 3 * C, c.dt, M, C, G(ix.qb), cw.ws()));
        RC(klab_colsum((char*)dqkv + (size_t)2 * C * c.es, 3 * C, c.dt, M, C, G(ix.vb), cw.ws()));
      }
      if (side_on) {
        klab_gemm_args gs[4];
        auto wg = [&](int i, const void* dy, long lddy, const void* x, long ldx, int N, int K, float* dw) {
          gs[i] = G0(cw, N, K, M, dy, lddy, 0, x, ldx, 0, dw, K, KLAB_F32);
          gs[i].accumulate = 1; gs[i].atomic_ok = 1;
        };
        wg(0, dyA, C, q.a, F, C, F, G(ix.f2w));
        wg(1, da, F, q.h1t, C, F, C, G(ix.f1w));
        wg(2, dyB, C, q.ctx, C, C, C, G(ix.pw));
        wg(3, dqkv, 3 * C, q.xt_in, C, 3 * C, C, G(ix.qw));
        RC(klab_gemm_grouped(gs, 4, cw.ws()));
      } else {
        RC(linear_wgrad(cw, dqkv, 3 * C, q.xt_in, C, M, 3 * C, C, G(ix.qw)));
      }
      if (e->bucket_events_on && !e->use_graph && swin_bucket < (int)e->bucket_ev[2].size())
        RC((int)hipEventRecord(e->bucket_ev[2][swin_bucket], cw.s));
      ++swin_bucket;
      if (side_on) RC((int)hipEventRecord(e->swin_done_ev[par], cs.s));
      ++blk_no;
      {
// ... 18 lines not shown
```

### klab_multimodalmodel_amd/csrc/gemm.hip

```cpp
#include <stdlib.h>

#include <map>
#include <mutex>
#include <vector>

#include "common.h"
#include <type_traits>
#include <utility>
#include "klab_mm.h"
#include "gemm_shared.h"

#ifndef KLAB_GLDS_STAGES
#define KLAB_GLDS_STAGES 4
#endif

namespace klab {

template <typename T> struct MmaTraits;
template <> struct MmaTraits<bf16_t> {
  static constexpr int BK = 64;
  static constexpr int KSTEP = 32;
};
template <> struct MmaTraits<float> {
  static constexpr int BK = 32;
// ... 62 lines not shown
        if (!ok) z = V{};
        v[c] = z;
      }
    }
  }
  __device__ __forceinline__ void store(char* lds, int tid) const {
    if constexpr (KMAJOR) {
#pragma unroll
      for (int c = 0; c < NCH; ++c) {
        int ch = tid + c * 256;
        int r = ch >> 3, kc = ch & 7;
        *reinterpret_cast<V*>(lds + r * ROWB + kc * 16) = v[c];
      }
    } else if constexpr (TR) {
      constexpr int CPR = ROWS / 8;
      using TL = TrLayout<ROWS>;
#pragma unroll
      for (int c = 0; c < NCH; ++c) {
        int ch = tid + c * 256;
        int kk = ch / CPR, m8 = ch % CPR;
        *reinterpret_cast<V*>(lds + (kk >> 3) * TL::GROUPB + (kk & 7) * TL::PITCHB + m8 * 16) = v[c];
      }
    } else {
      constexpr int RG = ROWS / VEC;
      int rg = tid % RG, kg = tid / RG;
#pragma unroll
      for (int i = 0; i < VEC; ++i) {
        T* dst = reinterpret_cast<T*>(lds + (rg * VEC + i) * ROWB) + kg * KPT;
#pragma unroll
        for (int c = 0; c < KPT; ++c) dst[c] = v[c][i];
      }
    }
  }
};

template <int ROWS, bool KMAJOR>
__device__ __forceinline__ bf16x8 load_frag_bf16(const char* tile, int r0, int ks, int lane) {
  if constexpr (KMAJOR) {
    return *reinterpret_cast<const bf16x8*>(tile + (r0 + (lane & 15)) * ROWB + ks * 64 + (lane >> 4) * 16);
  } else {
    using TL = TrLayout<ROWS>;
    typedef __attribute__((address_space(3))) bf16x4 lds_bf16x4;
    const int q = (lane & 15) >> 2, pp = lane & 3;
    const char* base = tile + (ks * 4 + (lane >> 4)) * TL::GROUPB + q * TL::PITCHB + (r0 + 4 * pp) * 2;
    bf16x4 lo = __builtin_amdgcn_ds_read_tr16_b64_v4bf16((lds_bf16x4*)(base));
    bf16x4 hi = __builtin_amdgcn_ds_read_tr16_b64_v4bf16((lds_bf16x4*)(base + 4 * TL::PITCHB));
    return bf16x8{lo[0], lo[1], lo[2], lo[3], hi[0], hi[1], hi[2], hi[3]};
  }
}



template <int ROWS> __device__ __forceinline__ int mmajor_f(int kr) {
  if constexpr (ROWS == 128) return (kr & 3) | (((kr >> 3) & 1) << 2);
  else return ((kr >> 1) & 1) | (((kr >> 3) & 1) << 1);
}

typedef __attribute__((ext_vector_type(4))) unsigned u32x4;
typedef __attribute__((ext_vector_type(2))) unsigned u32x2;

template <int OFF> __device__ __forceinline__ u32x4 lds_read_b128(unsigned addr) {
  u32x4 v;
  asm volatile("ds_read_b128 %0, %1 offset:%2" : "=v"(v) : "v"(addr), "n"(OFF) : "memory");
  return v;
}
template <int OFF> __device__ __forceinline__ u32x2 lds_read_tr(unsigned addr) {
  u32x2 v;
  asm volatile("ds_read_b64_tr_b16 %0, %1 offset:%2" : "=v"(v) : "v"(addr), "n"(OFF) : "memory");
  return v;
}
__device__ __forceinline__ void mfma_bf16_asm(f32x4& acc, const u32x4& x, const u32x4& y) {
  asm volatile("v_mfma_f32_16x16x32_bf16 %0, %1, %2, %0" : "+v"(acc) : "v"(x), "v"(y));
}
template <int LPS> __device__ __forceinline__ void wait_groups(int g) {
  switch (g) {
    case 0: wait_vmcnt<0>(); break;
    case 1: wait_vmcnt<LPS>(); break;
    case 2: wait_vmcnt<2 * LPS>(); break;
    default: wait_vmcnt<3 * LPS>(); break;
  }
}

template <int ROWS, bool KMAJOR, int NWAVES = 4, int NFRAG = ROWS / 32, typename E = bf16_t>
struct GldsOperand {
  static_assert(KMAJOR || sizeof(E) == 2, "the transposing LDS read is a 16-bit one");
  static constexpr int L = ROWS / (16 * NWAVES);
  static constexpr int BYTES = ROWS * 64;
  static constexpr int NF = NFRAG;
  static constexpr int RPF = KMAJOR ? 1 : 2;
  const E* src[L];
  long kstep;
  unsigned foff[KMAJOR ? 1 : NF];
  __device__ __forceinline__ void init(const E* base, long ld, int row0, int nrows, int wave, int lane, int wrow0) {
    if constexpr (KMAJOR) {
      const int lrow = lane >> 2, lpos = lane & 3;
      const int lchunk = lpos ^ (((lrow >> 2) & 1) << 1);
#pragma unroll
      for (int i = 0; i < L; ++i) {
        int r = row0 + (wave * L + i) * 16 + lrow;
        r = r < nrows ? r : nrows - 1;
        src[i] = base + (long)r * ld + lchunk * (16 / (int)sizeof(E));
      }
      kstep = 64 / (int)sizeof(E);
      const int fr = lane & 15, fc = lane >> 4;
      foff[0] = (unsigned)((wrow0 + fr) * 64 + ((fc ^ (((fr >> 2) & 1) << 1)) * 16));
    } else {
      constexpr int CPR = ROWS / 8, KR = 64 / CPR;
      const int kl = lane / CPR, pos = lane % CPR;
#pragma unroll
      for (int i = 0; i < L; ++i) {
        const int kr = (wave * L + i) * KR + kl;
        int m = row0 + ((pos ^ (mmajor_f<ROWS>(kr) << 1)) * 8);
        m = m + 8 <= nrows ? m : nrows - 8;
        src[i] = base + (long)kr * ld + m;
      }
      kstep = 32 * ld;
      const int g = lane >> 4, q4 = (lane & 15) >> 2, pp = lane & 3;
      const int kr0 = 8 * g + q4;
#pragma unroll
      for (int i = 0; i < NF; ++i) {
        const int chunk = ((wrow0 + i * 16) >> 3) + (pp >> 1);
        foff[i] = (unsigned)(kr0 * (ROWS * 2) + ((chunk ^ (mmajor_f<ROWS>(kr0) << 1)) * 16) + (pp & 1) * 8);
      }
    }
  }
  __device__ __forceinline__ void issue1(int i, int kt, char* stage, int wave) const {
    __builtin_amdgcn_global_load_lds((const __attribute__((address_space(1))) void*)(src[i] + kt * kstep),
                                     (__attribute__((address_space(3))) void*)(stage + (wave * L + i) * 1024), 16, 0, 0);
  }
  template <int R, int SOFF>
  __device__ __forceinline__ void read1(unsigned sbase, u32x4 (&fr)[NF]) const {
    if constexpr (KMAJOR) {
      fr[R] = lds_read_b128<SOFF + R * 1024>(sbase + foff[0]);
    } else {
      constexpr int i = R >> 1;
      const u32x2 h = lds_read_tr<SOFF + (R & 1) * 8 * ROWS>(sbase + foff[i]);
      if constexpr ((R & 1) == 0) { fr[i][0] = h[0]; fr[i][1] = h[1]; }
      else { fr[i][2] = h[0]; fr[i][3] = h[1]; }
    }
  }
};

#define KLAB_GLDS_WORK(BK)                                                              \
  const int tiles = ((p.M + BM - 1) / BM) * ((p.N + BN - 1) / BN);                      \
  const int tile = bid % tiles, split = bid / tiles;                                    \
  int bm0, bn0;                                                                         \
  tile_of_block(p, BM, BN, tile, bm0, bn0);                                             \
  const int nt_all = p.K / (BK);                                                        \
  const int per = (nt_all + p.splits - 1) / p.splits;                                   \
  const int kt0 = split * per, kt1 = (kt0 + per < nt_all) ? kt0 + per : nt_all;         \
  const int nt = kt1 - kt0;                                                             \
  if (nt <= 0) return;

template <int BM, int BN, bool AK, bool BKM, bool ATOMIC>
__device__ __forceinline__ void gemm_glds_body(const GemmP& p, const int bid = blockIdx.x) {
  typedef bf16_t T;
  constexpr int WTM = BM / 2, WTN = BN / 2, MI = WTM / 16, NI = WTN / 16;
  typedef GldsOperand<BM, AK> OA;
  typedef GldsOperand<BN, BKM> OB;
  extern __shared__ __attribute__((aligned(16))) char smem[];
  const int tid = threadIdx.x, lane = tid & 63;
  const int wave = __builtin_amdgcn_readfirstlane(tid >> 6);
  const int wm = (wave >> 1) * WTM, wn = (wave & 1) * WTN;
  KLAB_GLDS_WORK(32)

  OA oa; OB ob;
  oa.init(reinterpret_cast<const T*>(p.A), p.lda, bm0, p.M, wave, lane, wm);
  ob.init(reinterpret_cast<const T*>(p.B), p.ldb, bn0, p.N, wave, lane, wn);
#define KLAB_RING_MMA(ACC, A, B) if constexpr (ATOMIC) mfma_bf16_asm(ACC, A, B); else mfma_bf16_asm(ACC, B, A);
#define KLAB_RING_TWO_BASES 0
#define KLAB_RING_DRAIN4 1
#include "gemm_glds_loop.h"
  float alpha = p.alpha;
  if (p.alpha_dev) alpha *= p.alpha_dev[0];
  if constexpr (ATOMIC) {
    float* Cf = reinterpret_cast<float*>(p.C);
#pragma unroll
    for (int i = 0; i < MI; ++i)
#pragma unroll
      for (int j = 0; j < NI; ++j) {
        const int n = bn0 + wn + j * 16 + (lane & 15);
        if (n >= p.N) continue;
#pragma unroll
        for (int r = 0; r < 4; ++r) {
          const int m = bm0 + wm + i * 16 + (lane >> 4) * 4 + r;
          if (m < p.M) atomicAdd(Cf + (long)m * p.ldc + n, acc[i][j][r] * alpha);
        }
      }
  } else {
    __syncthreads();
    staged_epilogue<T, BM, BN, MI, NI>(p, acc, alpha, smem, bm0, bn0, wm, wn, tid, lane);
  }
}
template <bool BKM>
__device__ __forceinline__ void gemm_glds_w8_body(const GemmP& p, const int bid = blockIdx.x) {
  typedef bf16_t T;
  constexpr int BM = 256, BN = 128;
  constexpr int WTM = BM / 4, WTN = BN / 2, MI = WTM / 16, NI = WTN / 16;
  typedef GldsOperand<BM, true, 8, MI> OA;
  typedef GldsOperand<BN, BKM, 8, NI> OB;
  extern __shared__ __attribute__((aligned(16))) char smem[];
  const int tid = threadIdx.x, lane = tid & 63;
  const int wave = __builtin_amdgcn_readfirstlane(tid >> 6);
  const int wm = (wave >> 1) * WTM, wn = (wave & 1) * WTN;
  KLAB_GLDS_WORK(32)

  OA oa; OB ob;
  oa.init(reinterpret_cast<const T*>(p.A), p.lda, bm0, p.M, wave, lane, wm);
  ob.init(reinterpret_cast<const T*>(p.B), p.ldb, bn0, p.N, wave, lane, wn);
#define KLAB_RING_MMA(ACC, A, B) mfma_bf16_asm(ACC, B, A);
#define KLAB_RING_TWO_BASES 1
#define KLAB_RING_DRAIN4 0
#include "gemm_glds_loop.h"
  float alpha = p.alpha;
  if (p.alpha_dev) alpha *= p.alpha_dev[0];
  __syncthreads();
  staged_epilogue<T, BM, BN, MI, NI, 512>(p, acc, alpha, smem, bm0, bn0, wm, wn, tid, lane);
}
template <bool BKM>
__global__ __launch_bounds__(512) void gemm_glds_w8_kernel(GemmP p) { gemm_glds_w8_body<BKM>(p); }

template <int BM, int BN, bool AK, bool BKM, bool ATOMIC>
__global__ __launch_bounds__(256) void gemm_glds_kernel(GemmP p) { gemm_glds_body<BM, BN, AK, BKM, ATOMIC>(p); }

struct GroupEntry { const void* A; long lda; const void* B; long ldb; float* C; long ldc; int M, N, K, splits, start; float alpha; };
struct GroupP { GroupEntry e[8]; int n; };
template <int BN>
__global__ __launch_bounds__(256) void gemm_glds_grouped_tn_kernel(GroupP g) {
  int k = 0;
#pragma unroll
  for (int i = 1; i < 8; ++i)
    if (i < g.n && (int)blockIdx.x >= g.e[i].start) k = i;
  const GroupEntry& e = g.e[k];
  GemmP p;
  p.M = e.M; p.N = e.N; p.K = e.K;
  p.A = e.A; p.lda = e.lda; p.a_kmajor = 0; p.B = e.B; p.ldb = e.ldb; p.b_kmajor = 0;
  p.C = e.C; p.ldc = e.ldc; p.c_f32 = 1; p.accumulate = 1;
  p.alpha = e.alpha; p.alpha_dev = nullptr; p.bias = nullptr; p.act = 0;
  p.aux = nullptr; p.ldaux = 0; p.aux_mode = 0; p.aux_scale = 1.f; p.residual = nullptr; p.ldr = 0; p.r_f32 = 1;
  p.drop_p = 0.f; p.seed = nullptr; p.tag = 0; p.splits = e.splits; p.epi = 0;
  gemm_glds_body<128, BN, false, false, true>(p, (int)blockIdx.x - e.start);
}

template <typename T, int BM, int BN, bool AK, bool BKM, bool ATOMIC>
__device__ __forceinline__ void gemm_body(const GemmP& p) {
  constexpr int BK = MmaTraits<T>::BK;
  constexpr int WTM = BM / 2, WTN = BN / 2;
  constexpr int MI = WTM / 16, NI = WTN / 16;
  constexpr int ABYTES = TileBytes<T, BM, AK>::value, BBYTES = TileBytes<T, BN, BKM>::value;
  constexpr int STAGE = ABYTES + BBYTES;
  extern __shared__ __attribute__((aligned(16))) char smem[];

  const int tid = threadIdx.x, lane = tid & 63, wave = tid >> 6;
  const int wm = (wave >> 1) * WTM, wn = (wave & 1) * WTN;
  const int tiles_m = (p.M + BM - 1) / BM, tiles_n = (p.N + BN - 1) / BN;
  const int tiles = tiles_m * tiles_n;
  const int tile = blockIdx.x % tiles, split = blockIdx.x / tiles;
  int bm0, bn0;
  tile_of_block(p, BM, BN, tile, bm0, bn0);

  const T* A = reinterpret_cast<const T*>(p.A);
  const T* B = reinterpret_cast<const T*>(p.B);
  Stager<T, BM, AK> sa;
  Stager<T, BN, BKM> sb;

  f32x4 acc[MI][NI];
#pragma unroll
  for (int i = 0; i < MI; ++i)
#pragma unroll
    for (int j = 0; j < NI; ++j) acc[i][j] = f32x4{0.f, 0.f, 0.f, 0.f};

  const int nt_all = (p.K + BK - 1) / BK;
  const int per = (nt_all + p.splits - 1) / p.splits;
  const int kt0 = split * per, kt1 = (kt0 + per < nt_all) ? kt0 + per : nt_all;
  const int nt = kt1 - kt0;
  if (nt <= 0) return;
  sa.load(A, p.lda, bm0, kt0 * BK, p.M, p.K, tid);
  sb.load(B, p.ldb, bn0, kt0 * BK, p.N, p.K, tid);
  sa.store(smem, tid);
  sb.store(smem + ABYTES, tid);
  __syncthreads();

  for (int t = 0; t < nt; ++t) {
    const int cur = t & 1;
    if (t + 1 < nt) {
      sa.load(A, p.lda, bm0, (kt0 + t + 1) * BK, p.M, p.K, tid);
      sb.load(B, p.ldb, bn0, (kt0 + t + 1) * BK, p.N, p.K, tid);
    }
    const char* ta = smem + cur * STAGE;
    const char* tb = ta + ABYTES;
    if constexpr (sizeof(T) == 2) {
#pragma unroll
      for (int ks = 0; ks < BK / 32; ++ks) {
        bf16x8 af[MI], bfr[NI];
#pragma unroll
        for (int i = 0; i < MI; ++i) af[i] = load_frag_bf16<BM, AK>(ta, wm + i * 16, ks, lane);
#pragma unroll
        for (int j = 0; j < NI; ++j) bfr[j] = load_frag_bf16<BN, BKM>(tb, wn + j * 16, ks, lane);
#pragma unroll
        for (int i = 0; i < MI; ++i)
#pragma unroll
          for (int j = 0; j < NI; ++j) {
            if constexpr (ATOMIC) acc[i][j] = __builtin_amdgcn_mfma_f32_16x16x32_bf16(af[i], bfr[j], acc[i][j], 0, 0, 0);
            else acc[i][j] = __builtin_amdgcn_mfma_f32_16x16x32_bf16(bfr[j], af[i], acc[i][j], 0, 0, 0);
          }
      }
    } else {
      const char* la = ta + (wm + (lane & 15)) * ROWB;
      const char* lb = tb + (wn + (lane & 15)) * ROWB;
#pragma unroll
      for (int ks = 0; ks < BK / 4; ++ks) {
        float af[MI], bfr[NI];
        const int koff = (ks * 4 + (lane >> 4)) * 4;
#pragma unroll
        for (int i = 0; i < MI; ++i) af[i] = *reinterpret_cast<const float*>(la + i * 16 * ROWB + koff);
#pragma unroll
        for (int j = 0; j < NI; ++j) bfr[j] = *reinterpret_cast<const float*>(lb + j * 16 * ROWB + koff);
#pragma unroll
        for (int i = 0; i < MI; ++i)
#pragma unroll
          for (int j = 0; j < NI; ++j) {
            if constexpr (ATOMIC) acc[i][j] = __builtin_amdgcn_mfma_f32_16x16x4f32(af[i], bfr[j], acc[i][j], 0, 0, 0);
            else acc[i][j] = __builtin_amdgcn_mfma_f32_16x16x4f32(bfr[j], af[i], acc[i][j], 0, 0, 0);
          }
      }
    }
    if (t + 1 < nt) {
      sa.store(smem + (cur ^ 1) * STAGE, tid);
      sb.store(smem + (cur ^ 1) * STAGE + ABYTES, tid);
    }
    __syncthreads();
  }

  float alpha = p.alpha;
  if (p.alpha_dev) alpha *= p.alpha_dev[0];
  if constexpr (ATOMIC) {
    float* Cf = reinterpret_cast<float*>(p.C);
#pragma unroll
    for (int i = 0; i < MI; ++i)
#pragma unroll
      for (int j = 0; j < NI; ++j) {
        const int n = bn0 + wn + j * 16 + (lane & 15);
        if (n >= p.N) continue;
#pragma unroll
        for (int r = 0; r < 4; ++r) {
          const int m = bm0 + wm + i * 16 + (lane >> 4) * 4 + r;
          if (m < p.M) atomicAdd(Cf + (long)m * p.ldc + n, acc[i][j][r] * alpha);
        }
      }
  } else {
    staged_epilogue<T, BM, BN, MI, NI>(p, acc, alpha, smem, bm0, bn0, wm, wn, tid, lane);
  }
}

template <typename T, int BM, int BN, bool AK, bool BKM, bool ATOMIC>
__global__ __launch_bounds__(256) void gemm_kernel(GemmP p) { gemm_body<T, BM, BN, AK, BKM, ATOMIC>(p); }
template <typename T>
__global__ __launch_bounds__(256) void klab_lmhead_gemm(GemmP p) {
  if constexpr (sizeof(T) == 2) gemm_glds_body<128, 128, true, true, false>(p);
  else gemm_body<T, 128, 128, true, true, false>(p);
}

template <typename K>
static int launch_kernel(K kern, const GemmP& p, int BM, int BN, size_t lds, hipStream_t s) {
  {
    const int rc = ensure_dyn_lds(reinterpret_cast<const void*>(kern), lds);
    if (rc) return rc;
  }
  const long tm = (p.M + BM - 1) / BM, tn = (p.N + BN - 1) / BN;
  probed_launch(kern, dim3((unsigned)(tm * tn * p.splits)), dim3(256), lds, s, p);
  KLAB_LAUNCH_CHECK();
  return KLAB_OK;
}

template <typename T, int BM, int BN, bool AK, bool BKM>
static int launch_gemm(const GemmP& p, bool atomic, hipStream_t s) {
  size_t lds = 2 * (size_t)(TileBytes<T, BM, AK>::value + TileBytes<T, BN, BKM>::value);
  const size_t epi = (size_t)epilogue_lds_bytes<BM, BN>(p.c_f32 || sizeof(T) == 4);
  if (!atomic && epi > lds) lds = epi;
  if (atomic) return launch_kernel(gemm_kernel<T, BM, BN, AK, BKM, true>, p, BM, BN, lds, s);
  return launch_kernel(gemm_kernel<T, BM, BN, AK, BKM, false>, p, BM, BN, lds, s);
}

template <int BM, int BN, bool AK, bool BKM>
static int launch_glds(const GemmP& p, bool atomic, hipStream_t s) {
  const int nt = (p.K / 32 + p.splits - 1) / p.splits;
  size_t lds = (size_t)(nt < KLAB_GLDS_STAGES ? nt : KLAB_GLDS_STAGES) * (BM + BN) * 64;
  if (!atomic) {
    const size_t epi = (size_t)epilogue_lds_bytes<BM, BN>(p.c_f32);
    if (epi > lds) lds = epi;
    return launch_kernel(gemm_glds_kernel<BM, BN, AK, BKM, false>, p, BM, BN, lds, s);
  }
  return launch_kernel(gemm_glds_kernel<BM, BN, AK, BKM, true>, p, BM, BN, lds, s);
}
// ... 146 lines not shown
    if (t + 1 < nt) store(smem + (cur ^ 1) * STAGE);
    __syncthreads();
  }
#pragma unroll
  for (int i = 0; i < MI; ++i) {
    const int m = bm0 + wm + i * 16 + (lane & 15);
    const float sam = sc.sa[m < p.M ? m : p.M - 1];
#pragma unroll
    for (int j = 0; j < NI; ++j) {
      const int n0 = bn0 + wn + j * 16 + (lane >> 4) * 4;
#pragma unroll
      for (int r = 0; r < 4; ++r) {
        const int n = n0 + r < p.N ? n0 + r : p.N - 1;
        acc[i][j][r] *= sam * sc.sb[(long)n * sc.sb_stride];
      }
    }
  }
  float alpha = p.alpha;
  if (p.alpha_dev) alpha *= p.alpha_dev[0];
  staged_epilogue<bf16_t, BM, BN, MI, NI>(p, acc, alpha, smem, bm0, bn0, wm, wn, tid, lane);
}


__device__ __forceinline__ void mfma_fp8_asm2(f32x4& acc, const u32x4& x, const u32x4& y) {
  asm volatile("v_mfma_f32_16x16x32_fp8_fp8 %0, %1, %2, %0\n\tv_mfma_f32_16x16x32_fp8_fp8 %0, %3, %4, %0"
               : "+v"(acc)
               : "v"(__builtin_shufflevector(x, x, 0, 1)), "v"(__builtin_shufflevector(y, y, 0, 1)), "v"(__builtin_shufflevector(x, x, 2, 3)),
                 "v"(__builtin_shufflevector(y, y, 2, 3)));
}

template <int BM, int BN>
__device__ __forceinline__ void gemm_glds_fp8_body(const GemmP& p, const Fp8Scales& sc, const int bid = blockIdx.x) {
  typedef bf16_t T;
  constexpr int BK = 64;
  constexpr int WTM = BM / 2, WTN = BN / 2, MI = WTM / 16, NI = WTN / 16;
  typedef GldsOperand<BM, true, 4, BM / 32, char> OA;
  typedef GldsOperand<BN, true, 4, BN / 32, char> OB;
  extern __shared__ __attribute__((aligned(16))) char smem[];
  const int tid = threadIdx.x, lane = tid & 63;
  const int wave = __builtin_amdgcn_readfirstlane(tid >> 6);
  const int wm = (wave >> 1) * WTM, wn = (wave & 1) * WTN;
  KLAB_GLDS_WORK(BK)

  OA oa; OB ob;
  oa.init(reinterpret_cast<const char*>(p.A), p.lda, bm0, p.M, wave, lane, wm);
  ob.init(reinterpret_cast<const char*>(p.B), p.ldb, bn0, p.N, wave, lane, wn);
#define KLAB_RING_MMA(ACC, A, B) mfma_fp8_asm2(ACC, B, A);
#define KLAB_RING_TWO_BASES 0
#define KLAB_RING_DRAIN4 0
#include "gemm_glds_loop.h"
  float alpha = p.alpha;
  if (p.alpha_dev) alpha *= p.alpha_dev[0];
#pragma unroll
  for (int i = 0; i < MI; ++i) {
    const int m = bm0 + wm + i * 16 + (lane & 15);
    const float sam = sc.sa[m < p.M ? m : p.M - 1];
#pragma unroll
    for (int j = 0; j < NI; ++j) {
      const int n0 = bn0 + wn + j * 16 + (lane >> 4) * 4;
#pragma unroll
      for (int r = 0; r < 4; ++r) {
        const int n = n0 + r < p.N ? n0 + r : p.N - 1;
        acc[i][j][r] *= sam * sc.sb[(long)n * sc.sb_stride];
      }
    }
  }
  __syncthreads();
  staged_epilogue<T, BM, BN, MI, NI>(p, acc, alpha, smem, bm0, bn0, wm, wn, tid, lane);
}
template <int BM, int BN>
__global__ __launch_bounds__(256) void gemm_glds_fp8_kernel(GemmP p, Fp8Scales sc) { gemm_glds_fp8_body<BM, BN>(p, sc); }

__device__ __forceinline__ uint32_t pack4_fp8(float a, float b, float c, float d) {
  int w = __builtin_amdgcn_cvt_pk_fp8_f32(a, b, 0, false);
  w = __builtin_amdgcn_cvt_pk_fp8_f32(c, d, w, true);
  return (uint32_t)w;
}
__device__ __forceinline__ void quant_row_fp8(const bf16_t* __restrict__ src, int K, uint8_t* __restrict__ dst, float* __restrict__ scale, int lane) {
  constexpr int MAXV = 8;
  bf16x8 v[MAXV];
  float amax = 0.f;
#pragma unroll
  for (int u = 0; u < MAXV; ++u) {
    const int k = (u * 64 + lane) * 8;
    v[u] = bf16x8{};
    if (k < K) {
      v[u] = *reinterpret_cast<const bf16x8*>(src + k);
#pragma unroll
      for (int e = 0; e < 8; ++e) amax = fmaxf(amax, fabsf((float)v[u][e]));
    }
  }
#pragma unroll
  for (int o = 32; o > 0; o >>= 1) amax = fmaxf(amax, __shfl_xor(amax, o, 64));
  const float sc = amax > 0.f ? amax * (1.f / 448.f) : 1.f;
  const float inv = 1.f / sc;
  if (lane == 0) *scale = sc;
#pragma unroll
  for (int u = 0; u < MAXV; ++u) {
    const int k = (u * 64 + lane) * 8;
    if (k < K) {
      float f[8];
#pragma unroll
      for (int e = 0; e < 8; ++e) f[e] = fminf(fmaxf((float)v[u][e] * inv, -448.f), 448.f);
      uint2 o2;
      o2.x = pack4_fp8(f[0], f[1], f[2], f[3]);
      o2.y = pack4_fp8(f[4], f[5], f[6], f[7]);
      *reinterpret_cast<uint2*>(dst + k) = o2;
    }
  }
}
__global__ __launch_bounds__(256) void quant_fp8_rows_kernel(const bf16_t* __restrict__ x, long ldx, int M, int K, uint8_t* __restrict__ x8,
                                                             long ld8, float* __restrict__ scale, long scale_stride) {
  const int row = blockIdx.x * 4 + (threadIdx.x >> 6);
  if (row >= M) return;
  quant_row_fp8(x + (long)row * ldx, K, x8 + (long)row * ld8, scale + (long)row * scale_stride, threadIdx.x & 63);
}
struct QuantDesc { long off; long rows; long K; long row0; };
__global__ __launch_bounds__(256) void quant_fp8_arena_kernel(const QuantDesc* __restrict__ dglob, int nd, long total_rows,
                                                              const bf16_t* __restrict__ arena, uint8_t* __restrict__ w8,
                                                              float* __restrict__ wscale) {
  constexpr int MAXD = 1024;
  __shared__ QuantDesc dsh[MAXD];
  const bool in_lds = nd <= MAXD;
  if (in_lds) {
    for (int i = threadIdx.x; i < nd; i += blockDim.x) dsh[i] = dglob[i];
    __syncthreads();
  }
  const QuantDesc* d = in_lds ? dsh : dglob;
  for (long row = (long)blockIdx.x * 4 + (threadIdx.x >> 6); row < total_rows; row += (long)gridDim.x * 4) {
    int lo = 0, hi = nd - 1;
    while (lo < hi) {
      const int mid = (lo + hi + 1) >> 1;
      if (d[mid].row0 <= row) lo = mid; else hi = mid - 1;
    }
    const long e = d[lo].off + (row - d[lo].row0) * d[lo].K;
    quant_row_fp8(arena + e, (int)d[lo].K, w8 + e, wscale + (e >> 3), threadIdx.x & 63);
  }
}

}

extern "C" int klab_gemm(const klab_gemm_args* a, void* stream);
extern "C" int klab_gemm_grouped_tiles(const klab_gemm_args* list, int n, int large_tiles, void* stream) {
  using namespace klab;
  if (!list || n < 0) return KLAB_ERR_BADARG;
  {
    const int rc = mm8p_grouped_try(list, n, large_tiles != 0, (hipStream_t)stream);
    if (rc != KLAB_ERR_UNSUPPORTED) return rc;
  }
  GroupP g;
  g.n = 0;
  int blocks = 0;
  auto fits = [&](const klab_gemm_args* a) {
    return a->dtype == KLAB_BF16 && !a->a_kmajor && !a->b_kmajor && a->c_dtype == KLAB_F32 && a->accumulate && a->atomic_ok &&
           !a->bias && !a->act && !a->aux && !a->residual && a->drop_p == 0.f && !a->alpha_dev && a->name_tag == 0 && a->M >= 128 &&
           a->N >= 64 && (a->K % 32) == 0 && a->K >= 512 && !(a->M & 7) && !(a->N & 7) && !(a->lda & 7) && !(a->ldb & 7) &&
           !((uintptr_t)a->A & 15) && !((uintptr_t)a->B & 15) && !((uintptr_t)a->C & 15);
  };
  bool wide = true;
  for (int i = 0; i < n; ++i)
    if (fits(&list[i]) && list[i].N < 128) wide = false;
  const int BNr = wide ? 128 : 64;
  auto flush = [&]() -> int {
    if (!g.n) return KLAB_OK;
    const size_t lds = (size_t)KLAB_GLDS_STAGES * (128 + BNr) * 64;
    int rc = ensure_dyn_lds(wide ? reinterpret_cast<const void*>(gemm_glds_grouped_tn_kernel<128>)
                                 : reinterpret_cast<const void*>(gemm_glds_grouped_tn_kernel<64>), lds);
    if (rc) return rc;
    if (wide) probed_launch(gemm_glds_grouped_tn_kernel<128>, dim3((unsigned)blocks), dim3(256), lds, (hipStream_t)stream, g);
    else probed_launch(gemm_glds_grouped_tn_kernel<64>, dim3((unsigned)blocks), dim3(256), lds, (hipStream_t)stream, g);
    KLAB_LAUNCH_CHECK();
    g.n = 0; blocks = 0;
    return KLAB_OK;
  };
  long work = 0;
  for (int i = 0; i < n; ++i)
    if (fits(&list[i])) work += (long)((list[i].M + 127) / 128) * ((list[i].N + BNr - 1) / BNr) * (list[i].K / 32);
  constexpr int GROUP_TARGET = 384;
  long per_wg = work / (wide ? GROUP_TARGET / 2 : GROUP_TARGET);
  if (per_wg < 16) per_wg = 16;
  for (int i = 0; i < n; ++i) {
    const klab_gemm_args* a = &list[i];
    if (!fits(a)) {
      const int rc = klab_gemm(a, stream);
      if (rc) return rc;
      continue;
    }
    const long t = (long)((a->M + 127) / 128) * ((a->N + BNr - 1) / BNr);
    const int nt = a->K / 32;
    long sp = (nt + per_wg / 2) / per_wg;
    if (sp > nt / 16) sp = nt / 16;
    if (sp > 16) sp = 16;
    if (sp < 1) sp = 1;
    GroupEntry& e = g.e[g.n];
    e.A = a->A; e.lda = a->lda; e.B = a->B; e.ldb = a->ldb; e.C = (float*)a->C; e.ldc = a->ldc;
    e.M = a->M; e.N = a->N; e.K = a->K; e.splits = (int)sp; e.start = blocks; e.alpha = a->alpha;
    blocks += (int)(t * sp);
    if (++g.n == 8) { const int rc = flush(); if (rc) return rc; }
  }
  return flush();
}
extern "C" int klab_gemm_grouped(const klab_gemm_args* list, int n, void* stream) { return klab_gemm_grouped_tiles(list, n, 0, stream); }

namespace klab {
static void fill_gemmp(const klab_gemm_args* a, GemmP& p) {
  p.M = a->M; p.N = a->N; p.K = a->K;
  p.A = a->A; p.lda = a->lda; p.a_kmajor = a->a_kmajor;
  p.B = a->B; p.ldb = a->ldb; p.b_kmajor = a->b_kmajor;
  p.C = a->C; p.ldc = a->ldc; p.c_f32 = (a->c_dtype == KLAB_F32); p.accumulate = a->accumulate;
  p.alpha = a->alpha; p.alpha_dev = a->alpha_dev; p.bias = a->bias; p.act = a->act;
  p.aux = a->aux; p.ldaux = a->ldaux; p.aux_mode = a->aux_mode; p.aux_scale = a->aux_scale;
  p.residual = a->residual; p.ldr = a->ldr; p.r_f32 = (a->r_dtype == KLAB_F32);
  p.drop_p = a->drop_p; p.seed = a->seed_dev; p.tag = a->drop_tag;
  p.splits = 1;
  {
    int f = 0;
    if (a->bias) f |= EF_BIAS;
    if (a->act == KLAB_ACT_RELU) f |= EF_RELU;
    if (a->act == KLAB_ACT_GELU) f |= EF_GELU;
    if (a->aux && a->aux_mode == KLAB_AUX_NONZERO) f |= EF_AUXNZ;
    if (a->aux && a->aux_mode == KLAB_AUX_DGELU) f |= EF_DGELU;
    if (a->drop_p > 0.f && a->seed_dev) f |= EF_DROP;
    if (a->residual) f |= EF_RES;
    if (!a->accumulate && a->dtype == KLAB_BF16) {
      if (f == EF_AUXNZ && a->c_dtype == KLAB_BF16 && !(a->N & 7) && !(a->ldc & 7) && !(a->ldaux & 7) && !((uintptr_t)a->aux & 15)) f = EF_AUXNZ_CO;
      if (f == EF_DGELU && a->c_dtype == KLAB_BF16 && !(a->N & 7) && !(a->ldc & 7) && !(a->ldaux & 7) && !((uintptr_t)a->aux & 15)) f = EF_DGELU_CO;
      if ((f == EF_RES || f == (EF_DROP | EF_RES)) && a->c_dtype == KLAB_F32 && a->r_dtype == KLAB_F32 && !(a->N & 3) && !(a->ldc & 3) &&
          !(a->ldr & 3) && !((uintptr_t)a->residual & 15))
        f = (f & ~EF_RES) | EF_RES_CO;
    }
    if ((f & EF_DROP) && (long)a->M * a->N >= (1L << 32)) f = EF_GENERIC;
    p.epi = f;
  }
}
}

namespace klab {
struct GemmProbe {
  std::mutex mu;
  bool on = false;
  std::vector<hipEvent_t> a, b;
  std::vector<double> flops;
  size_t n = 0;
};
static GemmProbe& gemm_probe() { static GemmProbe p; return p; }
}
static int klab_gemm_impl(const klab_gemm_args* a, void* stream);
extern "C" int klab_gemm_probe_enable(int on) {
  klab::GemmProbe& pr = klab::gemm_probe();
  std::lock_guard<std::mutex> lk(pr.mu);
  if (on && pr.a.empty()) {
    const size_t cap = 8192;
    pr.a.assign(cap, nullptr); pr.b.assign(cap, nullptr); pr.flops.assign(cap, 0.0);
    for (size_t i = 0; i < cap; ++i)
      if (hipEventCreate(&pr.a[i]) != hipSuccess || hipEventCreate(&pr.b[i]) != hipSuccess) return KLAB_ERR_UNSUPPORTED;
  }
  pr.on = on != 0;
  if (on) pr.n = 0;
  return KLAB_OK;
}
extern "C" int klab_gemm_probe_read(int* launches, float* total_ms, double* flops_total) {
  klab::GemmProbe& pr = klab::gemm_probe();
  std::lock_guard<std::mutex> lk(pr.mu);
  float tot = 0.f;
  double fl = 0;
  int cnt = 0;
  for (size_t i = 0; i < pr.n; ++i) {
    if (pr.flops[i] < 0) continue;
    float ms = 0.f;
    const hipError_t er = hipEventElapsedTime(&ms, pr.a[i], pr.b[i]);
    if (er != hipSuccess) { (void)hipGetLastError(); continue; }
    tot += ms;
    fl += pr.flops[i];
    ++cnt;
  }
  if (launches) *launches = cnt;
  if (total_ms) *total_ms = tot;
  if (flops_total) *flops_total = fl;
  return KLAB_OK;
}
extern "C" int klab_gemm(const klab_gemm_args* a, void* stream) {
  klab::GemmProbe& pr = klab::gemm_probe();
  if (!pr.on || !a) return klab_gemm_impl(a, stream);
  size_t slot;
  {
    std::lock_guard<std::mutex> lk(pr.mu);
    if (pr.n >= pr.a.size()) return klab_gemm_impl(a, stream);
    slot = pr.n++;
    pr.flops[slot] = 2.0 * a->M * (double)a->N * a->K;
  }
  klab::tl_launch_probe.a = pr.a[slot];
  klab::tl_launch_probe.b = pr.b[slot];
  const int rc = klab_gemm_impl(a, stream);
  if (klab::tl_launch_probe.a) {
    klab::tl_launch_probe.a = nullptr;
    std::lock_guard<std::mutex> lk(pr.mu);
    pr.flops[slot] = -1.0;
  }
  return rc;
}

namespace klab { int lmhead_areg_try(const GemmP& p, hipStream_t s); }
static int klab_gemm_impl(const klab_gemm_args* a, void* stream) {
  using namespace klab;
  if (!a || !a->A || !a->B || !a->C) return KLAB_ERR_BADARG;
  if (a->M <= 0 || a->N <= 0 || a->K <= 0) return KLAB_OK;
  const int vec = a->dtype == KLAB_BF16 ? 8 : 4;
  if (a->lda % vec || a->ldb % vec) return KLAB_ERR_UNSUPPORTED;
  if (a->a_kmajor ? (a->K % vec) : (a->M % vec)) return KLAB_ERR_UNSUPPORTED;
  if (a->b_kmajor ? (a->K % vec) : (a->N % vec)) return KLAB_ERR_UNSUPPORTED;
  if (((uintptr_t)a->A & 15) || ((uintptr_t)a->B & 15) || ((uintptr_t)a->C & 15)) return KLAB_ERR_UNSUPPORTED;
  if (a->dtype != KLAB_F32 && a->dtype != KLAB_BF16) return KLAB_ERR_BADARG;
  if (a->c_dtype != KLAB_F32 && a->c_dtype != a->dtype) return KLAB_ERR_BADARG;
  GemmP p;
  fill_gemmp(a, p);
  hipStream_t s = (hipStream_t)stream;
  if (a->name_tag == 1 && a->a_kmajor && a->b_kmajor) {
    if (a->dtype == KLAB_BF16) {
      if (a->K % 32) return KLAB_ERR_UNSUPPORTED;
      {
        const int rc = lmhead_areg_try(p, s);
        if (rc != KLAB_ERR_UNSUPPORTED) return rc;
      }
      size_t lds = KLAB_GLDS_STAGES * (size_t)(128 + 128) * 64;
      const size_t epi = (size_t)epilogue_lds_bytes<128, 128>(p.c_f32);
      return launch_kernel(klab_lmhead_gemm<bf16_t>, p, 128, 128, epi > lds ? epi : lds, s);
    }
    size_t lds = 2 * (size_t)(128 + 128) * ROWB;
    const size_t epi = (size_t)epilogue_lds_bytes<128, 128>(true);
    return launch_kernel(klab_lmhead_gemm<float>, p, 128, 128, epi > lds ? epi : lds, s);
  }
  const bool atomic_ok = a->atomic_ok && p.c_f32 && a->accumulate && !a->bias && !a->act && !a->aux && !a->residual && a->drop_p == 0.f;
  const int p8_force = a->name_tag == 2 ? 1 : (a->name_tag == 3 ? -1 : 0);
  if (a->dtype == KLAB_BF16) return dispatch_tile<bf16_t>(p, atomic_ok, s, p8_force);
  return dispatch_tile<float>(p, atomic_ok, s);
}

extern "C" int klab_quant_fp8_rows(const void* x, long ldx, int M, int K, void* x8, long ld8, float* row_scale, void* stream) {
  using namespace klab;
  if (!x || !x8 || !row_scale) return KLAB_ERR_BADARG;
  if (M <= 0) return KLAB_OK;
  if (K <= 0 || K > 4096 || (K & 7) || (ldx & 7) || (ld8 & 7) || ((uintptr_t)x & 15) || ((uintptr_t)x8 & 7)) return KLAB_ERR_UNSUPPORTED;
  hipLaunchKernelGGL(quant_fp8_rows_kernel, dim3((unsigned)((M + 3) / 4)), dim3(256), 0, (hipStream_t)stream, (const bf16_t*)x, ldx, M, K,
                     (uint8_t*)x8, ld8, row_scale, 1L);
  KLAB_LAUNCH_CHECK();
  return KLAB_OK;
}

extern "C" int klab_quant_fp8_arena(const void* desc_dev, int ndesc, long total_rows, const void* arena_bf16, void* arena_fp8, float* scales,
// ... 66 lines not shown
```

### klab_multimodalmodel_amd/csrc/misc.hip

```cpp
#include <math.h>

#include <map>
#include <mutex>

#include "common.h"
#include "klab_mm.h"

namespace klab {

int ensure_dyn_lds(const void* kernel, size_t bytes) {
  static std::mutex mu;
  static std::map<const void*, size_t> set;
  if (bytes > 160 * 1024) return KLAB_ERR_UNSUPPORTED;
  std::lock_guard<std::mutex> g(mu);
  auto it = set.find(kernel);
  if (it != set.end() && it->second >= bytes) return KLAB_OK;
  hipError_t e = hipFuncSetAttribute(kernel, hipFuncAttributeMaxDynamicSharedMemorySize, (int)bytes);
  if (e != hipSuccess) return (int)e;
  set[kernel] = bytes;
  return KLAB_OK;
}

struct CastDesc { const float* src; long dst_off; long n4_prefix; };

// ... 292 lines not shown
  if ((threadIdx.x & 63) == 0) red[threadIdx.x >> 6] = a;
  __syncthreads();
  if (threadIdx.x == 0) loss[0] = (red[0] + red[1] + red[2] + red[3]) * inv_n[0];
}

template <typename T>
__global__ __launch_bounds__(256) void im2col_kernel(const float* __restrict__ pix, T* __restrict__ out, int B, int Cin, int Himg, int P) {
  const int R = Himg / P;
  const int K = Cin * P * P;
  const long total = (long)B * R * R * K;
  for (long idx = (long)blockIdx.x * blockDim.x + threadIdx.x; idx < total; idx += (long)gridDim.x * blockDim.x) {
    const int k = idx % K;
    const long t = idx / K;
    const int px = k % P, py = (k / P) % P, c = k / (P * P);
    const int x = t % R, y = (t / R) % R;
    const long b = t / ((long)R * R);
    out[idx] = from_f32<T>(pix[((b * Cin + c) * Himg + (y * P + py)) * Himg + (x * P + px)]);
  }
}

template <typename T>
__global__ __launch_bounds__(256) void im2col4_kernel(const float* __restrict__ pix, T* __restrict__ out, int B, int Cin, int Himg, int ldo) {
  const int R = Himg / 4;
  const long npatch = (long)B * R * R;
  for (long t = (long)blockIdx.x * blockDim.x + threadIdx.x; t < npatch; t += (long)gridDim.x * blockDim.x) {
    const int x = t % R, y = (t / R) % R;
    const long b = t / ((long)R * R);
    T* o = out + t * ldo;
    for (int c = 0; c < Cin; ++c) {
      f32x4 v[4];
#pragma unroll
      for (int py = 0; py < 4; ++py) v[py] = *reinterpret_cast<const f32x4*>(pix + ((b * Cin + c) * Himg + (y * 4 + py)) * Himg + x * 4);
      if constexpr (sizeof(T) == 2) {
        *reinterpret_cast<bf16x8*>(o + c * 16) = bf16x8{(bf16_t)v[0][0], (bf16_t)v[0][1], (bf16_t)v[0][2], (bf16_t)v[0][3],
                                                        (bf16_t)v[1][0], (bf16_t)v[1][1], (bf16_t)v[1][2], (bf16_t)v[1][3]};
        *reinterpret_cast<bf16x8*>(o + c * 16 + 8) = bf16x8{(bf16_t)v[2][0], (bf16_t)v[2][1], (bf16_t)v[2][2], (bf16_t)v[2][3],
                                                            (bf16_t)v[3][0], (bf16_t)v[3][1], (bf16_t)v[3][2], (bf16_t)v[3][3]};
      } else {
#pragma unroll
        for (int py = 0; py < 4; ++py) *reinterpret_cast<f32x4*>(o + c * 16 + py * 4) = v[py];
      }
    }
    for (int k = Cin * 16; k < ldo; k += 8) {
      if constexpr (sizeof(T) == 2) *reinterpret_cast<bf16x8*>(o + k) = bf16x8{};
      else { *reinterpret_cast<f32x4*>(o + k) = f32x4{0.f, 0.f, 0.f, 0.f}; *reinterpret_cast<f32x4*>(o + k + 4) = f32x4{0.f, 0.f, 0.f, 0.f}; }
    }
  }
}

template <typename T>
__global__ __launch_bounds__(256) void merge_gather_kernel(const float* __restrict__ x, T* __restrict__ out, int B, int R, int C) {
  const int R2 = R / 2;
  const long total4 = (long)B * R2 * R2 * C;
  for (long g = (long)blockIdx.x * blockDim.x + threadIdx.x; g < total4; g += (long)gridDim.x * blockDim.x) {
    const int c4 = g % C;
    const long t = g / C;
    const int q = (c4 * 4) / C, c = (c4 * 4) % C;
    const int dy = q & 1, dx = q >> 1;
    const int x2 = t % R2, y2 = (t / R2) % R2;
    const long b = t / ((long)R2 * R2);
    const f32x4 v = *reinterpret_cast<const f32x4*>(x + ((b * R + (2 * y2 + dy)) * R + (2 * x2 + dx)) * C + c);
    T* o = out + t * 4L * C + c4 * 4;
    if constexpr (sizeof(T) == 2) *reinterpret_cast<bf16x4*>(o) = bf16x4{(bf16_t)v[0], (bf16_t)v[1], (bf16_t)v[2], (bf16_t)v[3]};
    else *reinterpret_cast<f32x4*>(o) = v;
  }
}
__global__ __launch_bounds__(256) void merge_scatter_kernel(const float* __restrict__ dm, float* __restrict__ dx, int B, int R, int C) {
  const int R2 = R / 2;
  const long total4 = (long)B * R2 * R2 * C;
  for (long g = (long)blockIdx.x * blockDim.x + threadIdx.x; g < total4; g += (long)gridDim.x * blockDim.x) {
    const int c4 = g % C;
    const long t = g / C;
    const int q = (c4 * 4) / C, c = (c4 * 4) % C;
    const int dy = q & 1, dxo = q >> 1;
    const int x2 = t % R2, y2 = (t / R2) % R2;
    const long b = t / ((long)R2 * R2);
    *reinterpret_cast<f32x4*>(dx + ((b * R + (2 * y2 + dy)) * R + (2 * x2 + dxo)) * C + c) =
        *reinterpret_cast<const f32x4*>(dm + t * 4L * C + c4 * 4);
  }
}

template <typename T>
__global__ __launch_bounds__(256) void colsum_kernel(const T* __restrict__ dy, long ld, int M, int N, float* __restrict__ out) {
  __shared__ float red[4][64];
  const int col = blockIdx.x * 64 + (threadIdx.x & 63);
  const int rl = threadIdx.x >> 6;
  float a = 0.f;
  if (col < N)
    for (long m = (long)blockIdx.y * 4 + rl; m < M; m += (long)gridDim.y * 4) a += to_f32(dy[m * ld + col]);
  red[rl][threadIdx.x & 63] = a;
  __syncthreads();
  if (rl == 0 && col < N) atomicAdd(out + col, red[0][threadIdx.x] + red[1][threadIdx.x] + red[2][threadIdx.x] + red[3][threadIdx.x]);
}

__global__ __launch_bounds__(256) void colsum8_kernel(const bf16_t* __restrict__ dy, long ld, int M, int N, float* __restrict__ out) {
  __shared__ float red[32][65];
  const int cl = threadIdx.x & 7, rl = threadIdx.x >> 3;
  const int col = blockIdx.x * 64 + cl * 8;
  float a[8] = {0.f, 0.f, 0.f, 0.f, 0.f, 0.f, 0.f, 0.f};
  if (col < N)
    for (long m = (long)blockIdx.y * 32 + rl; m < M; m += (long)gridDim.y * 32) {
      const bf16x8 v = *reinterpret_cast<const bf16x8*>(dy + m * ld + col);
#pragma unroll
      for (int u = 0; u < 8; ++u) a[u] += (float)v[u];
    }
#pragma unroll
  for (int u = 0; u < 8; ++u) red[rl][cl * 8 + u] = a[u];
  __syncthreads();
  if (threadIdx.x < 64 && blockIdx.x * 64 + threadIdx.x < N) {
    float t = 0.f;
#pragma unroll
    for (int r = 0; r < 32; ++r) t += red[r][threadIdx.x];
    atomicAdd(out + blockIdx.x * 64 + threadIdx.x, t);
  }
}

template <typename T>
__global__ __launch_bounds__(256) void convert_kernel(const float* __restrict__ x, T* __restrict__ y, long n4, float scale) {
  for (long g = (long)blockIdx.x * blockDim.x + threadIdx.x; g < n4; g += (long)gridDim.x * blockDim.x) {
    f32x4 v = *reinterpret_cast<const f32x4*>(x + g * 4);
    if constexpr (sizeof(T) == 2) *reinterpret_cast<bf16x4*>(y + g * 4) = bf16x4{(bf16_t)(v[0] * scale), (bf16_t)(v[1] * scale), (bf16_t)(v[2] * scale), (bf16_t)(v[3] * scale)};
    else *reinterpret_cast<f32x4*>(y + g * 4) = f32x4{v[0] * scale, v[1] * scale, v[2] * scale, v[3] * scale};
  }
}
__global__ __launch_bounds__(256) void add_f32_kernel(float* __restrict__ y, const float* __restrict__ x, long n4) {
  for (long g = (long)blockIdx.x * blockDim.x + threadIdx.x; g < n4; g += (long)gridDim.x * blockDim.x) {
    f32x4 a = *reinterpret_cast<const f32x4*>(y + g * 4);
    const f32x4 b = *reinterpret_cast<const f32x4*>(x + g * 4);
    a[0] += b[0]; a[1] += b[1]; a[2] += b[2]; a[3] += b[3];
    *reinterpret_cast<f32x4*>(y + g * 4) = a;
  }
}

template <typename T>
__global__ __launch_bounds__(256) void gelu_fwd_kernel(const T* __restrict__ x, T* __restrict__ y, long n) {
  constexpr int VEC = Vec16<T>::N;
  using VT = typename Vec16<T>::type;
  for (long g = (long)blockIdx.x * blockDim.x + threadIdx.x; g < n / VEC; g += (long)gridDim.x * blockDim.x) {
    VT v = *reinterpret_cast<const VT*>(x + g * VEC);
    VT o;
#pragma unroll
    for (int u = 0; u < VEC; ++u) o[u] = from_f32<T>(gelu_for<T>(to_f32(v[u])));
    *reinterpret_cast<VT*>(y + g * VEC) = o;
  }
}

static inline unsigned stream_grid(long work_items) {
  long g = (work_items + 255) / 256;
  if (g < 1) g = 1;
  if (g > 2048) g = 2048;
  return (unsigned)g;
}

}

using namespace klab;

extern "C" int klab_cast_pack(const void* desc_dev, int ndesc, long total4, void* dst, int dtype, void* stream) {
  if (!desc_dev || !dst || ndesc <= 0) return KLAB_ERR_BADARG;
  hipStream_t s = (hipStream_t)stream;
  if (dtype == KLAB_BF16)
    hipLaunchKernelGGL(cast_pack_kernel<bf16_t>, dim3(stream_grid((total4 + 7) / 8)), dim3(256), 0, s, (const CastDesc*)desc_dev, ndesc, total4, (bf16_t*)dst);
  else
    hipLaunchKernelGGL(cast_pack_kernel<float>, dim3(stream_grid((total4 + 7) / 8)), dim3(256), 0, s, (const CastDesc*)desc_dev, ndesc, total4, (float*)dst);
  KLAB_LAUNCH_CHECK();
  return KLAB_OK;
}

extern "C" int klab_adam_step_range(const void* desc_dev, int ndesc, long begin4, long end4, const float* grads, float* m, float* v, void* arena,
                                    int dtype, float lr, float beta1, float beta2, float eps, float weight_decay, float bias_corr1,
                                    float bias_corr2, void* stream) {
  if (!desc_dev || ndesc <= 0 || !grads || !m || !v || !arena || bias_corr1 <= 0.f || bias_corr2 <= 0.f || begin4 < 0 || end4 < begin4)
    return KLAB_ERR_BADARG;
  if (end4 == begin4) return KLAB_OK;
  AdamHyper h{lr / bias_corr1, beta1, beta2, eps, weight_decay, 1.f / sqrtf(bias_corr2)};
  hipStream_t s = (hipStream_t)stream;
  constexpr int ADAM_GRID = 1024;
  constexpr int U = 4;
  long gl = ((end4 - begin4 + U - 1) / U + 255) / 256;
  const unsigned grid = (unsigned)(gl < 1 ? 1 : (gl > ADAM_GRID ? ADAM_GRID : gl));
  if (dtype == KLAB_BF16)
    hipLaunchKernelGGL((adam_step_kernel<bf16_t, U>), dim3(grid), dim3(256), 0, s, (const AdamDesc*)desc_dev, ndesc, begin4, end4, grads, m, v,
                       (bf16_t*)arena, h);
  else
    hipLaunchKernelGGL((adam_step_kernel<float, U>), dim3(grid), dim3(256), 0, s, (const AdamDesc*)desc_dev, ndesc, begin4, end4, grads, m, v,
                       (float*)arena, h);
  KLAB_LAUNCH_CHECK();
  return KLAB_OK;
}
extern "C" int klab_adam_step(const void* desc_dev, int ndesc, long total4, const float* grads, float* m, float* v, void* arena, int dtype,
                              float lr, float beta1, float beta2, float eps, float weight_decay, float bias_corr1, float bias_corr2,
                              void* stream) {
  return klab_adam_step_range(desc_dev, ndesc, 0, total4, grads, m, v, arena, dtype, lr, beta1, beta2, eps, weight_decay, bias_corr1, bias_corr2,
                              stream);
}

extern "C" int klab_embed_fwd(const long long* ids, int shift_right, int L, int start_id, int pad_id, const float* table, int vocab,
                              float* out, int rows, int d, float drop_p, const uint32_t* seed_dev, uint32_t tag, int* err_flag,
                              void* stream) {
  if (!ids || !table || !out || (d & 3)) return KLAB_ERR_BADARG;
  if (rows <= 0) return KLAB_OK;
  hipLaunchKernelGGL(embed_fwd_kernel, dim3(stream_grid((long)rows * 64)), dim3(256), 0, (hipStream_t)stream, ids, shift_right, L, start_id,
                     pad_id, table, vocab, out, rows, d, drop_p, seed_dev, tag, err_flag);
  KLAB_LAUNCH_CHECK();
  return KLAB_OK;
}

extern "C" int klab_embed_bwd(const long long* ids, int shift_right, int L, int start_id, int pad_id, const float* dh, float* dtable,
                              int vocab, int rows, int d, float drop_p, const uint32_t* seed_dev, uint32_t tag, void* stream) {
  if (!ids || !dh || !dtable) return KLAB_ERR_BADARG;
  if (rows <= 0) return KLAB_OK;
  hipLaunchKernelGGL(embed_bwd_kernel, dim3(stream_grid((long)rows * 64)), dim3(256), 0, (hipStream_t)stream, ids, shift_right, L, start_id,
                     pad_id, dh, dtable, vocab, rows, d, drop_p, seed_dev, tag);
  KLAB_LAUNCH_CHECK();
  return KLAB_OK;
}

extern "C" int klab_relbias_fwd(const float* table, const int* bucket, float* bias, int heads, int Lq, int Lk, void* stream) {
  if (!table || !bucket || !bias) return KLAB_ERR_BADARG;
  const long tot = (long)heads * Lq * Lk;
  hipLaunchKernelGGL(relbias_fwd_kernel, dim3((unsigned)((tot + 255) / 256)), dim3(256), 0, (hipStream_t)stream, table, bucket, bias, heads, Lq * Lk);
  KLAB_LAUNCH_CHECK();
  return KLAB_OK;
}

extern "C" int klab_relbias_bwd(const float* dbias, const int* bucket, float* dtable, int heads, int Lq, int Lk, int nbuckets, void* stream) {
  if (!dbias || !bucket || !dtable) return KLAB_ERR_BADARG;
  if (nbuckets > 64) return KLAB_ERR_UNSUPPORTED;
  hipLaunchKernelGGL(relbias_bwd_kernel, dim3(heads), dim3(256), 0, (hipStream_t)stream, dbias, bucket, dtable, heads, Lq * Lk, nbuckets);
  KLAB_LAUNCH_CHECK();
  return KLAB_OK;
}

extern "C" int klab_ce_count(const long long* labels, int rows, float* inv_n, void* stream) {
  if (!labels || !inv_n || rows <= 0) return KLAB_ERR_BADARG;
  hipLaunchKernelGGL(ce_count_kernel, dim3(1), dim3(256), 0, (hipStream_t)stream, labels, rows, inv_n);
  KLAB_LAUNCH_CHECK();
  return KLAB_OK;
}

extern "C" int klab_ce_fwd(void* logits, long ld, int dtype, const long long* labels, int rows, int V, float* inv_n, float* loss_row,
                           float* loss, int write_grad, void* stream) {
  if (!logits || !labels || !inv_n || !loss_row || !loss) return KLAB_ERR_BADARG;
  const int vec = dtype == KLAB_BF16 ? 8 : 4;
  if (V % vec || ld % vec) return KLAB_ERR_UNSUPPORTED;
  hipStream_t s = (hipStream_t)stream;
  if (!(write_grad & 2)) {
    hipLaunchKernelGGL(ce_count_kernel, dim3(1), dim3(256), 0, s, labels, rows, inv_n);
    KLAB_LAUNCH_CHECK();
  }
  write_grad &= 1;
  if (dtype == KLAB_BF16 && V <= 256 * 8 * 16 && V > 256 * 8 * 8)
    hipLaunchKernelGGL((ce_fwd_onepass_kernel<bf16_t, 16>), dim3(rows), dim3(256), 0, s, (bf16_t*)logits, ld, labels, V, inv_n, loss_row, write_grad);
  else if (dtype == KLAB_BF16 && V <= 256 * 8 * 8)
    hipLaunchKernelGGL((ce_fwd_onepass_kernel<bf16_t, 8>), dim3(rows), dim3(256), 0, s, (bf16_t*)logits, ld, labels, V, inv_n, loss_row, write_grad);
  else if (dtype == KLAB_BF16)
    hipLaunchKernelGGL(ce_fwd_kernel<bf16_t>, dim3(rows), dim3(256), 0, s, (bf16_t*)logits, ld, labels, V, inv_n, loss_row, write_grad);
  else
    hipLaunchKernelGGL(ce_fwd_kernel<float>, dim3(rows), dim3(256), 0, s, (float*)logits, ld, labels, V, inv_n, loss_row, write_grad);
  KLAB_LAUNCH_CHECK();
  hipLaunchKernelGGL(ce_reduce_kernel, dim3(1), dim3(256), 0, s, loss_row, rows, inv_n, loss);
  KLAB_LAUNCH_CHECK();
  return KLAB_OK;
}

extern "C" int klab_im2col_patch(const float* pixels, void* out, int dtype, int B, int Cin, int Himg, int P, void* stream) {
  if (!pixels || !out || Himg % P) return KLAB_ERR_BADARG;
  const long total = (long)B * (Himg / P) * (Himg / P) * Cin * P * P;
  hipStream_t s = (hipStream_t)stream;
  if (dtype == KLAB_BF16) hipLaunchKernelGGL(im2col_kernel<bf16_t>, dim3(stream_grid(total)), dim3(256), 0, s, pixels, (bf16_t*)out, B, Cin, Himg, P);
  else hipLaunchKernelGGL(im2col_kernel<float>, dim3(stream_grid(total)), dim3(256), 0, s, pixels, (float*)out, B, Cin, Himg, P);
  KLAB_LAUNCH_CHECK();
  return KLAB_OK;
}

extern "C" int klab_im2col_patch_ld(const float* pixels, void* out, int dtype, int B, int Cin, int Himg, int P, int ldo, void* stream) {
  if (!pixels || !out || Himg % P || ldo < Cin * P * P) return KLAB_ERR_BADARG;
  if (P != 4 || (Himg & 3) || (ldo & 7) || ((uintptr_t)pixels & 15) || ((uintptr_t)out & 15)) {
    if (ldo == Cin * P * P) return klab_im2col_patch(pixels, out, dtype, B, Cin, Himg, P, stream);
    return KLAB_ERR_UNSUPPORTED;
  }
  const long npatch = (long)B * (Himg / 4) * (Himg / 4);
  hipStream_t s = (hipStream_t)stream;
  if (dtype == KLAB_BF16) hipLaunchKernelGGL(im2col4_kernel<bf16_t>, dim3(stream_grid(npatch)), dim3(256), 0, s, pixels, (bf16_t*)out, B, Cin, Himg, ldo);
  else hipLaunchKernelGGL(im2col4_kernel<float>, dim3(stream_grid(npatch)), dim3(256), 0, s, pixels, (float*)out, B, Cin, Himg, ldo);
  KLAB_LAUNCH_CHECK();
  return KLAB_OK;
}

extern "C" int klab_merge_gather(const float* x, void* out, int dtype, int B, int R, int C, void* stream) {
  if (!x || !out || (R & 1) || (C & 3)) return KLAB_ERR_BADARG;
  const long total4 = (long)B * (R / 2) * (R / 2) * C;
  hipStream_t s = (hipStream_t)stream;
  if (dtype == KLAB_BF16) hipLaunchKernelGGL(merge_gather_kernel<bf16_t>, dim3(stream_grid(total4)), dim3(256), 0, s, x, (bf16_t*)out, B, R, C);
  else hipLaunchKernelGGL(merge_gather_kernel<float>, dim3(stream_grid(total4)), dim3(256), 0, s, x, (float*)out, B, R, C);
  KLAB_LAUNCH_CHECK();
  return KLAB_OK;
}

extern "C" int klab_merge_scatter(const float* dmerged, float* dx, int B, int R, int C, void* stream) {
  if (!dmerged || !dx || (R & 1) || (C & 3)) return KLAB_ERR_BADARG;
  const long total4 = (long)B * (R / 2) * (R / 2) * C;
  hipLaunchKernelGGL(merge_scatter_kernel, dim3(stream_grid(total4)), dim3(256), 0, (hipStream_t)stream, dmerged, dx, B, R, C);
  KLAB_LAUNCH_CHECK();
  return KLAB_OK;
}
// ... 101 lines not shown
```

### klab_multimodalmodel_amd/csrc/mm8p.hip

```cpp
#include <stdlib.h>

#include <type_traits>

#include "gemm_shared.h"

namespace klab {

namespace p8 {
constexpr int BM = 256, BN = 256, BK = 64, NT = 512;
constexpr int HALF = 16384;
constexpr int LDS_RING = 8 * HALF;
typedef __attribute__((address_space(3))) char lds_char;

__device__ __forceinline__ int mmajor_f(int kr) { return (kr & 3) | (((kr >> 3) & 1) << 2); }

template <bool KMAJOR, int BLK>
struct Operand {
  static __device__ __forceinline__ int tile_row(int R, int H) { return (R / BLK) * (2 * BLK) + H * BLK + (R % BLK); }
  const bf16_t* src[2][2];
  long kstep;
  __device__ __forceinline__ void init(const bf16_t* base, long ld, int row0, int nrows, int wave, int lane) {
#pragma unroll
    for (int h = 0; h < 2; ++h)
#pragma unroll
// ... 201 lines not shown
#pragma unroll
    for (int j = 0; j < 4; ++j) acc[i][j] = f32x4{0.f, 0.f, 0.f, 0.f};

  issue_half(0, W0{}, 0); issue_half(0, W1{}, 1); issue_half(0, W2{}, 2); issue_half(0, W3{}, 3);
  issue_half(1, W0{}, 4); issue_half(1, W1{}, 5); issue_half(1, W2{}, 6);
  if (nt >= 2) wait_vmcnt<6>(); else wait_vmcnt<0>();
  __builtin_amdgcn_s_barrier();

  const int a_img_row0 = (wave >> 2) * 64;
  const int b_img_row0 = (wave & 3) * 32;

  auto ktile_body = [&](auto buf_c, int t) {
    constexpr int BUF = decltype(buf_c)::value;
    const char* A0 = smem + (BUF * 4 + 0) * HALF;
    const char* B0 = smem + (BUF * 4 + 1) * HALF;
    const char* B1 = smem + (BUF * 4 + 2) * HALF;
    const char* A1 = smem + (BUF * 4 + 3) * HALF;
    bf16x8 af[4][2], bf0[2][2], bf1[2][2];
#pragma unroll
    for (int i = 0; i < 4; ++i)
#pragma unroll
      for (int s = 0; s < 2; ++s) af[i][s] = frag<AK>(A0, (a_img_row0 >> 4) + i, s, lane);
#pragma unroll
    for (int j = 0; j < 2; ++j)
#pragma unroll
      for (int s = 0; s < 2; ++s) bf0[j][s] = frag<BKM>(B0, (b_img_row0 >> 4) + j, s, lane);
    issue_half(t + 1, W3{}, (BUF ^ 1) * 4 + 3);
    __builtin_amdgcn_sched_barrier(0);
    __builtin_amdgcn_s_barrier();
    wait_lgkmcnt<0>();
    __builtin_amdgcn_sched_barrier(0);
    __builtin_amdgcn_s_setprio(1);
#pragma unroll
    for (int s = 0; s < 2; ++s)
#pragma unroll
      for (int i = 0; i < 4; ++i)
#pragma unroll
        for (int j = 0; j < 2; ++j) {
          if constexpr (ATOMIC) acc[i][j] = __builtin_amdgcn_mfma_f32_16x16x32_bf16(af[i][s], bf0[j][s], acc[i][j], 0, 0, 0);
          else acc[i][j] = __builtin_amdgcn_mfma_f32_16x16x32_bf16(bf0[j][s], af[i][s], acc[i][j], 0, 0, 0);
        }
    __builtin_amdgcn_s_setprio(0);
    __builtin_amdgcn_sched_barrier(0);
    __builtin_amdgcn_s_barrier();
#pragma unroll
    for (int j = 0; j < 2; ++j)
#pragma unroll
      for (int s = 0; s < 2; ++s) bf1[j][s] = frag<BKM>(B1, (b_img_row0 >> 4) + j, s, lane);
    issue_half(t + 2, W0{}, BUF * 4 + 0);
    __builtin_amdgcn_sched_barrier(0);
    __builtin_amdgcn_s_barrier();
    wait_lgkmcnt<0>();
    __builtin_amdgcn_sched_barrier(0);
    __builtin_amdgcn_s_setprio(1);
#pragma unroll
    for (int s = 0; s < 2; ++s)
#pragma unroll
      for (int i = 0; i < 4; ++i)
#pragma unroll
        for (int j = 0; j < 2; ++j) {
          if constexpr (ATOMIC) acc[i][2 + j] = __builtin_amdgcn_mfma_f32_16x16x32_bf16(af[i][s], bf1[j][s], acc[i][2 + j], 0, 0, 0);
          else acc[i][2 + j] = __builtin_amdgcn_mfma_f32_16x16x32_bf16(bf1[j][s], af[i][s], acc[i][2 + j], 0, 0, 0);
        }
    __builtin_amdgcn_s_setprio(0);
    __builtin_amdgcn_sched_barrier(0);
    __builtin_amdgcn_s_barrier();
#pragma unroll
    for (int i = 0; i < 4; ++i)
#pragma unroll
      for (int s = 0; s < 2; ++s) af[i][s] = frag<AK>(A1, (a_img_row0 >> 4) + i, s, lane);
    issue_half(t + 2, W1{}, BUF * 4 + 1);
    __builtin_amdgcn_sched_barrier(0);
    __builtin_amdgcn_s_barrier();
    wait_lgkmcnt<0>();
    __builtin_amdgcn_sched_barrier(0);
    __builtin_amdgcn_s_setprio(1);
#pragma unroll
    for (int s = 0; s < 2; ++s)
#pragma unroll
      for (int i = 0; i < 4; ++i)
#pragma unroll
        for (int j = 0; j < 2; ++j) {
          if constexpr (ATOMIC) acc[4 + i][2 + j] = __builtin_amdgcn_mfma_f32_16x16x32_bf16(af[i][s], bf1[j][s], acc[4 + i][2 + j], 0, 0, 0);
          else acc[4 + i][2 + j] = __builtin_amdgcn_mfma_f32_16x16x32_bf16(bf1[j][s], af[i][s], acc[4 + i][2 + j], 0, 0, 0);
        }
    __builtin_amdgcn_s_setprio(0);
    __builtin_amdgcn_sched_barrier(0);
    __builtin_amdgcn_s_barrier();
    issue_half(t + 2, W2{}, BUF * 4 + 2);
    if (t + 2 < nt) wait_vmcnt<6>(); else wait_vmcnt<0>();
    __builtin_amdgcn_sched_barrier(0);
    __builtin_amdgcn_s_barrier();
    __builtin_amdgcn_sched_barrier(0);
    __builtin_amdgcn_s_setprio(1);
#pragma unroll
    for (int s = 0; s < 2; ++s)
#pragma unroll
      for (int i = 0; i < 4; ++i)
#pragma unroll
        for (int j = 0; j < 2; ++j) {
          if constexpr (ATOMIC) acc[4 + i][j] = __builtin_amdgcn_mfma_f32_16x16x32_bf16(af[i][s], bf0[j][s], acc[4 + i][j], 0, 0, 0);
          else acc[4 + i][j] = __builtin_amdgcn_mfma_f32_16x16x32_bf16(bf0[j][s], af[i][s], acc[4 + i][j], 0, 0, 0);
        }
    __builtin_amdgcn_s_setprio(0);
    __builtin_amdgcn_sched_barrier(0);
    __builtin_amdgcn_s_barrier();
  };

  int t = 0;
  for (; t + 1 < nt; t += 2) {
    ktile_body(std::integral_constant<int, 0>{}, t);
    ktile_body(std::integral_constant<int, 1>{}, t + 1);
  }
  if (t < nt) ktile_body(std::integral_constant<int, 0>{}, t);

  wait_vmcnt<0>();
  float alpha = p.alpha;
  if (p.alpha_dev) alpha *= p.alpha_dev[0];
  if constexpr (ATOMIC) {
    float* Cf = reinterpret_cast<float*>(p.C);
#pragma unroll
    for (int i = 0; i < 8; ++i)
#pragma unroll
      for (int j = 0; j < 4; ++j) {
        const int n = bn0 + wn + j * 16 + (lane & 15);
        if (n >= p.N) continue;
#pragma unroll
        for (int r = 0; r < 4; ++r) {
          const int m = bm0 + wm + i * 16 + (lane >> 4) * 4 + r;
          if (m < p.M) atomicAdd(Cf + (long)m * p.ldc + n, acc[i][j][r] * alpha);
        }
      }
  } else {
#pragma unroll 1
    for (int half = 0; half < 2; ++half) {
      __syncthreads();
      if ((wave >> 2) == half) {
#pragma unroll
        for (int i = 0; i < 8; ++i)
#pragma unroll
          for (int j = 0; j < 4; ++j)
            *reinterpret_cast<f32x4*>(smem + (i * 16 + (lane & 15)) * SLAB_PITCH + (wn + j * 16 + (lane >> 4) * 4) * 4) = acc[i][j];
      }
      __syncthreads();
      if (p.c_f32) slab_out<float>(p, smem, bm0 + half * 128, bn0, tid, alpha);
      else slab_out<bf16_t>(p, smem, bm0 + half * 128, bn0, tid, alpha);
    }
  }
}

template <bool AK, bool BKM, bool ATOMIC>
__global__ __launch_bounds__(512) void mm8p_kernel(GemmP p) { mm8p_body<AK, BKM, ATOMIC>(p, blockIdx.x); }

struct Group8Entry { const void* A; long lda; const void* B; long ldb; float* C; long ldc; int M, N, K, start; float alpha; };
constexpr int GROUP_MAX = 32;
struct Group8P { Group8Entry e[GROUP_MAX]; int n; };
__global__ __launch_bounds__(512) void mm8p_grouped_tn_kernel(Group8P g) {
  int i = 0;
#pragma unroll
  for (int k = 1; k < GROUP_MAX; ++k)
    if (k < g.n && (int)blockIdx.x >= g.e[k].start) i = k;
  const Group8Entry& e = g.e[i];
  GemmP p;
  p.M = e.M; p.N = e.N; p.K = e.K;
  p.A = e.A; p.lda = e.lda; p.a_kmajor = 0;
  p.B = e.B; p.ldb = e.ldb; p.b_kmajor = 0;
  p.C = e.C; p.ldc = e.ldc; p.c_f32 = 1; p.accumulate = 1;
  p.alpha = e.alpha; p.alpha_dev = nullptr; p.bias = nullptr; p.act = 0;
  p.aux = nullptr; p.ldaux = 0; p.aux_mode = 0; p.aux_scale = 1.f;
  p.residual = nullptr; p.ldr = 0; p.r_f32 = 1;
  p.drop_p = 0.f; p.seed = nullptr; p.tag = 0;
  p.splits = 1; p.epi = 0;
  mm8p_body<false, false, false>(p, (int)blockIdx.x - e.start);
}

}

int mm8p_grouped_try(const klab_gemm_args* list, int n, bool large_tiles, hipStream_t s) {
  using namespace p8;
  if (!large_tiles || n <= 0 || n > GROUP_MAX) return KLAB_ERR_UNSUPPORTED;
  Group8P g;
  g.n = 0;
  int blocks = 0;
  for (int i = 0; i < n; ++i) {
    const klab_gemm_args* a = &list[i];
    const bool ok = a->dtype == KLAB_BF16 && !a->a_kmajor && !a->b_kmajor && a->c_dtype == KLAB_F32 && a->accumulate && !a->bias && !a->act &&
                    !a->aux && !a->residual && a->drop_p == 0.f && !a->alpha_dev && a->M >= 128 && a->N >= 128 && (a->K % BK) == 0 &&
                    a->K >= 1024 && !(a->M & 7) && !(a->N & 7) && !(a->lda & 7) && !(a->ldb & 7) && !(a->ldc & 3) &&
                    !((uintptr_t)a->A & 15) && !((uintptr_t)a->B & 15) && !((uintptr_t)a->C & 15);
    if (!ok) return KLAB_ERR_UNSUPPORTED;
    Group8Entry& e = g.e[g.n++];
    e.A = a->A; e.lda = a->lda; e.B = a->B; e.ldb = a->ldb; e.C = (float*)a->C; e.ldc = a->ldc;
    e.M = a->M; e.N = a->N; e.K = a->K; e.start = blocks; e.alpha = a->alpha;
    blocks += ((a->M + BM - 1) / BM) * ((a->N + BN - 1) / BN);
  }
  const size_t epi_bytes = (size_t)128 * SLAB_PITCH;
  const size_t lds = LDS_RING > epi_bytes ? LDS_RING : epi_bytes;
  int rc = ensure_dyn_lds(reinterpret_cast<const void*>(mm8p_grouped_tn_kernel), lds);
  if (rc) return rc;
  probed_launch(mm8p_grouped_tn_kernel, dim3((unsigned)blocks), dim3(NT), lds, s, g);
  KLAB_LAUNCH_CHECK();
  return KLAB_OK;
}

int mm8p_try(const GemmP& pin, bool atomic_ok, int force, hipStream_t s) {
  using namespace p8;
  static const bool on = env_on("KLAB_GEMM_P8");
  if (!on && force <= 0) return KLAB_ERR_UNSUPPORTED;
  GemmP p = pin;
  if (p.K % BK || p.K < 2 * BK) return KLAB_ERR_UNSUPPORTED;
  if (!p.a_kmajor && (p.M % 8)) return KLAB_ERR_UNSUPPORTED;
  if (!p.b_kmajor && (p.N % 8)) return KLAB_ERR_UNSUPPORTED;
  if (p.M < 8 || p.N < 8) return KLAB_ERR_UNSUPPORTED;
  const long tiles = (long)((p.M + BM - 1) / BM) * ((p.N + BN - 1) / BN);
  const int ncu = 256;
  int splits = 1;
  if (atomic_ok) {
    const int nt = p.K / BK;
    while (tiles * splits * 2 <= ncu && nt / (splits * 2) >= 8) splits *= 2;
  }
  if (force <= 0) {
    const long wgs = tiles * splits;
    const long rounds = (wgs + ncu - 1) / ncu;
    const long tiles_m = (p.M + BM - 1) / BM, tiles_n = (p.N + BN - 1) / BN;
    if (p.K / splits < 1024) return KLAB_ERR_UNSUPPORTED;
    if (wgs * 100 < rounds * ncu * (p.K / splits >= 2048 ? 80 : 90)) return KLAB_ERR_UNSUPPORTED;
    if (splits == 1 && (tiles_m < 4 || tiles_n < 4)) return KLAB_ERR_UNSUPPORTED;
  }
  p.splits = splits;
  if (p.epi == EF_AUXNZ_CO) p.epi = EF_AUXNZ;
  else if (p.epi == EF_DGELU_CO) p.epi = EF_DGELU;
  else if (p.epi == EF_RES_CO) p.epi = EF_RES;
  else if (p.epi == (EF_DROP | EF_RES_CO)) p.epi = EF_DROP | EF_RES;
  const bool atomic = atomic_ok && splits > 1;
  const size_t epi_bytes = (size_t)128 * (BN + 4) * 4;
  const size_t lds = LDS_RING > epi_bytes ? LDS_RING : epi_bytes;
  const dim3 grid((unsigned)(tiles * splits));
  int rc;
#define KLAB_P8(AKv, BKv, ATv)                                                                           \
  {                                                                                                     \
    rc = ensure_dyn_lds(reinterpret_cast<const void*>(mm8p_kernel<AKv, BKv, ATv>), lds);                \
    if (rc) return rc;                                                                                  \
    probed_launch(mm8p_kernel<AKv, BKv, ATv>, grid, dim3(NT), lds, s, p);                               \
  }
  if (atomic) {
    if (p.a_kmajor && p.b_kmajor) KLAB_P8(true, true, true)
    else if (p.a_kmajor) KLAB_P8(true, false, true)
    else if (p.b_kmajor) KLAB_P8(false, true, true)
    else KLAB_P8(false, false, true)
  } else {
    if (p.a_kmajor && p.b_kmajor) KLAB_P8(true, true, false)
    else if (p.a_kmajor) KLAB_P8(true, false, false)
    else if (p.b_kmajor) KLAB_P8(false, true, false)
    else KLAB_P8(false, false, false)
  }
#undef KLAB_P8
  KLAB_LAUNCH_CHECK();
  return KLAB_OK;
}

}
```

Measured before the change: 11940 samples/s.

## Store weight gradients directly instead of zero-then-accumulate for grouped wgrads

Weight-gradient GEMMs that are flushed in grouped batches now write their results with plain stores instead of atomically adding into a pre-zeroed buffer. A write plan records which gradient ranges will be fully overwritten, and the memsets are replaced by a multi-range zeroing kernel that clears only the remaining gaps. The aim is to cut memset traffic and atomic-add overhead on the fp32 gradient arena. In exchange, store-mode entries lose split-K (splits forced to 1), and the bookkeeping must stay consistent with graph mode and the KV-gradient path.

```diff
diff --git a/klab_multimodalmodel_amd/csrc/common.h b/klab_multimodalmodel_amd/csrc/common.h
--- a/klab_multimodalmodel_amd/csrc/common.h
+++ b/klab_multimodalmodel_amd/csrc/common.h
@@ -29,6 +29,9 @@
 }
 
 int ensure_dyn_lds(const void* kernel, size_t bytes);
+
+constexpr int ZERO_RANGES_MAX = 16;
+int zero_ranges(float* const* ptrs, const long* counts, int n, hipStream_t s);
 
 template <typename T> struct TypeTag;
 template <> struct TypeTag<float> { static constexpr int id = KLAB_F32; };
diff --git a/klab_multimodalmodel_amd/csrc/engine.cpp b/klab_multimodalmodel_amd/csrc/engine.cpp
--- a/klab_multimodalmodel_amd/csrc/engine.cpp
+++ b/klab_multimodalmodel_amd/csrc/engine.cpp
@@ -3,7 +3,9 @@
 #include <stdio.h>
 #include <string.h>
 
+#include <algorithm>
 #include <string>
+#include <utility>
 #include <vector>
 
 #include "gemm_shared.h"
@@ -158,6 +160,13 @@
   bool dec_embed_ready = false;
   bool inv_n_ready = false;
   bool kv_wgrad_done = false;
+  struct WritePlan {
+    bool valid = false, graph = false, kv = false;
+    bool head_store = false, any_store = false;
+    std::vector<char> store[2];
+    std::vector<std::pair<long, long>> stored;
+    std::vector<std::pair<long, long>> clear[2];
+  } wplan;
   hipStream_t own = nullptr; hipEvent_t ev_in = nullptr, ev_out = nullptr;
   bool use_graph = false;
   struct GraphSlot { hipGraphExec_t exec = nullptr; int uses = 0; bool failed = false; } gs[7];
@@ -794,11 +803,66 @@
   RC((int)hipEventRecord(ev, e->side));
   return (int)hipStreamWaitEvent(c.s, ev, 0);
 }
-struct PendingWgrad { const void* dy; long lddy; const void* x; long ldx; int M, N, K; float* dw; };
+static bool wgrad_store_on() {
+  static const bool on = klab::env_on("KLAB_WGRAD_STORE");
+  return on;
+}
+struct WgradRelease { std::vector<char> flush_at, store; bool kv_in_queue = false; };
+static WgradRelease wgrad_release_plan(const klab_engine* e, const klab_t5_cfg& cfg, int Ln, bool dec, bool have_dkv, const float* Gflat) {
+  const int d = cfg.d_model, inner = cfg.n_heads * cfg.d_kv, ff = cfg.d_ff;
+  WgradRelease r;
+  r.flush_at.assign(Ln, 1);
+  r.store.assign(Ln, 0);
+  constexpr int GROUP_TILES = 90;
+  static const bool group_on = klab::env_on("KLAB_WGRAD_GROUP_TILES");
+  const bool eager_main = Gflat == e->G[2] && !e->use_graph;
+  r.kv_in_queue = dec && have_dkv && eager_main && e->kvall_g_off >= 0;
+  if (group_on && Ln >= 3 && eager_main) {
+    auto T2 = [](int n, int k) { return (long)((n + 255) / 256) * ((k + 255) / 256); };
+    const long tl = T2(d, ff) + T2(cfg.ffn_gated ? 2 * ff : ff, d) + T2(d, inner) + T2(3 * inner, d) + (dec ? T2(d, inner) + T2(inner, d) + (r.kv_in_queue ? T2(2 * inner, d) : 0) : 0);
+    const int per_group = (int)((GROUP_TILES + tl - 1) / tl), per_layer = dec ? 7 : 4;
+    if (per_group >= 2) {
+      const int body = Ln - 1;
+      int ng = body / per_group;
+      if (ng < 1) ng = 1;
+      if (((body + ng - 1) / ng) * per_layer <= 32) {
+        std::fill(r.flush_at.begin(), r.flush_at.end(), 0);
+        int i = Ln - 1;
+        for (int gi = 0; gi < ng; ++gi) { i -= body / ng + (gi < body % ng ? 1 : 0); r.flush_at[i + 1] = 1; }
+        r.flush_at[0] = 1;
+      }
+    }
+  }
+  if (wgrad_store_on() && eager_main) {
+    const size_t per_layer = dec ? 6 + (r.kv_in_queue ? 1 : 0) : 4;
+    size_t queued = 0;
+    int first = Ln - 1;
+    for (int i = Ln - 1; i >= 0; --i) {
+      queued += per_layer;
+      if (!r.flush_at[i] && queued + 8 <= 32) continue;
+      if (first - i + 1 >= 2)
+        for (int k = i; k <= first; ++k) r.store[k] = 1;
+      queued = 0; first = i - 1;
+    }
+  }
+  return r;
+}
+
+struct PendingWgrad { const void* dy; long lddy; const void* x; long ldx; int M, N, K; float* dw; bool store; };
 struct WgradQueue {
   std::vector<PendingWgrad> q;
   int layers = 0;
-  void push(const void* dy, long lddy, const void* x, long ldx, int M, int N, int K, float* dw) { q.push_back({dy, lddy, x, ldx, M, N, K, dw}); }
+  const klab_engine::WritePlan* plan = nullptr; const float* Gbase = nullptr;
+  int push(const void* dy, long lddy, const void* x, long ldx, int M, int N, int K, float* dw, bool store = false) {
+    if (store) {
+      bool ok = false;
+      if (plan && plan->valid)
+        for (const auto& s : plan->stored) ok = ok || (s.first == dw - Gbase && s.second == (long)N * K);
+      if (!ok) return KLAB_ERR_BADARG;
+    }
+    q.push_back({dy, lddy, x, ldx, M, N, K, dw, store});
+    return 0;
+  }
   int flush(const Ctx& c, bool now = true, bool* launched = nullptr) {
     if (launched) *launched = false;
     ++layers;
@@ -813,7 +877,7 @@
     gs.reserve(q.size());
     for (const PendingWgrad& w : q) {
       klab_gemm_args g = G0(cs, w.N, w.K, w.M, w.dy, w.lddy, 0, w.x, w.ldx, 0, w.dw, w.K, KLAB_F32);
-      g.accumulate = 1; g.atomic_ok = 1;
+      g.accumulate = w.store ? 0 : 1; g.atomic_ok = 1;
       gs.push_back(g);
     }
     klab_engine::Probe& pr = c.e->probe[1];
@@ -877,38 +941,24 @@
   RC(rms_bwd(e->dxn, s.h[j], W[final_ln], s.rstd_f, nullptr, dh_cur, dy, final_ln, p, tag_of(stack_id, 0, SITE_FINAL), p,
              tag_of(stack_id, (int)L.size() - 1, SITE_FFN_OUT)));
   std::vector<int> pending_buckets;
-  const int Ln = (int)L.size();
-  std::vector<char> flush_at(Ln, 1);
-  constexpr int GROUP_TILES = 90;
-  static const bool group_on = klab::env_on("KLAB_WGRAD_GROUP_TILES");
-  const bool kv_in_queue = dec && dkv_all && Gflat == e->G[2] && !e->use_graph && e->kvall_g_off >= 0;
-  if (group_on && Ln >= 3 && Gflat == e->G[2] && !e->use_graph) {
-    auto T2 = [](int n, int k) { return (long)((n + 255) / 256) * ((k + 255) / 256); };
-    const long tl = T2(d, ff) + T2(cfg.ffn_gated ? 2 * ff : ff, d) + T2(d, inner) + T2(3 * inner, d) + (dec ? T2(d, inner) + T2(inner, d) + (kv_in_queue ? T2(2 * inner, d) : 0) : 0);
-    const int per_group = (int)((GROUP_TILES + tl - 1) / tl), per_layer = dec ? 7 : 4;
-    if (per_group >= 2) {
-      const int body = Ln - 1;
-      int ng = body / per_group;
-      if (ng < 1) ng = 1;
-      if (((body + ng - 1) / ng) * per_layer <= 32) {
-        std::fill(flush_at.begin(), flush_at.end(), 0);
-        int i = Ln - 1;
-        for (int gi = 0; gi < ng; ++gi) { i -= body / ng + (gi < body % ng ? 1 : 0); flush_at[i + 1] = 1; }
-        flush_at[0] = 1;
-      }
-    }
-  }
+  const WgradRelease rel = wgrad_release_plan(e, cfg, (int)L.size(), dec, dkv_all != nullptr, Gflat);
+  const std::vector<char>& flush_at = rel.flush_at;
+  const bool kv_in_queue = rel.kv_in_queue;
+  const bool plan_live = Gflat == e->G[2];
+  if (plan_live && (!e->wplan.valid || e->wplan.store[stk] != rel.store)) return KLAB_ERR_BADARG;
+  wq.plan = &e->wplan; wq.Gbase = Gflat;
   for (int i = (int)L.size() - 1; i >= 0; --i) {
     const T5LayerIdx& l = L[i];
     T5LayerBufs& b = s.L[i];
     void* dhmid = e->dhmid_pool[i];
     void* dqkv = e->dqkv_pool[i];
+    const bool st = plan_live && rel.store[i];
     --j;
-    wq.push(dy, d, b.hmid, ff, M, d, ff, G(l.wo));
+    RC(wq.push(dy, d, b.hmid, ff, M, d, ff, G(l.wo), st));
     if (cfg.ffn_gated) {
       RC(linear_dgrad(c, dy, d, M, d, P[l.wo].warena_off, ff, e->dh_ff, c.dt));
       RC(klab_geglu_bwd(e->dh_ff, ff, b.ab, 2 * ff, dhmid, 2 * ff, c.dt, M, ff, p, e->seed_dev, tag_of(stack_id, i, SITE_MID), c.ws()));
-      wq.push(dhmid, 2 * ff, b.xn3, d, M, 2 * ff, d, G(l.wi));
+      RC(wq.push(dhmid, 2 * ff, b.xn3, d, M, 2 * ff, d, G(l.wi), st));
       RC(linear_dgrad(c, dhmid, 2 * ff, M, 2 * ff, P[l.wi].warena_off, d, e->dxn, KLAB_F32));
     } else {
       {
@@ -916,7 +966,7 @@
         g.aux = b.hmid; g.ldaux = ff; g.aux_mode = KLAB_AUX_NONZERO; g.aux_scale = inv_keep;
         RC(klab_gemm(&g, c.ws()));
       }
-      wq.push(dhmid, ff, b.xn3, d, M, ff, d, G(l.wi));
+      RC(wq.push(dhmid, ff, b.xn3, d, M, ff, d, G(l.wi), st));
       RC(linear_dgrad(c, dhmid, ff, M, ff, P[l.wi].warena_off, d, e->dxn, KLAB_F32));
     }
     {
@@ -928,7 +978,7 @@
     if (dec) {
       --j;
       void* dqc = e->dqc_pool[i];
-      wq.push(dy, d, b.ctx2, inner, M, d, inner, G(l.co));
+      RC(wq.push(dy, d, b.ctx2, inner, M, d, inner, G(l.co), st));
       dctx_ready = false;
       klab_attn_args a;
       memset(&a, 0, sizeof(a));
@@ -942,17 +992,17 @@
       a.dv = eoff(c, dkv_all, (long)i * 2 * inner + inner); a.lddv = kv_ld;
       RC(attn_bwd(a, P[l.co].warena_off));
       if (kv_in_queue) {
-        wq.push(eoff(c, dkv_all, (long)i * 2 * inner), kv_ld, e->enc.out_t, d, B * Lkv, 2 * inner, d, Gflat + e->kvall_g_off + (long)i * 2 * inner * d);
+        RC(wq.push(eoff(c, dkv_all, (long)i * 2 * inner), kv_ld, e->enc.out_t, d, B * Lkv, 2 * inner, d, Gflat + e->kvall_g_off + (long)i * 2 * inner * d, st));
         e->kv_wgrad_done = true;
       }
-      wq.push(dqc, inner, b.xn2, d, M, inner, d, G(l.cq));
+      RC(wq.push(dqc, inner, b.xn2, d, M, inner, d, G(l.cq), st));
       RC(linear_dgrad(c, dqc, inner, M, inner, P[l.cq].warena_off, d, e->dxn, KLAB_F32));
       dy = next_dy();
       RC(rms_bwd(e->dxn, s.h[j], W[l.ln1], b.rstd2, dh_cur, dh_oth, dy, l.ln1, 0.f, 0, p, tag_of(stack_id, i, SITE_ATTN_OUT)));
       float* t = dh_cur; dh_cur = dh_oth; dh_oth = t;
     }
     --j;
-    wq.push(dy, d, b.ctx, inner, M, d, inner, G(l.o));
+    RC(wq.push(dy, d, b.ctx, inner, M, d, inner, G(l.o), st));
     dctx_ready = false;
     {
       klab_attn_args a;
@@ -974,7 +1024,7 @@
       if (arc == KLAB_ERR_UNSUPPORTED) { a.ds_defer = 0; a.ds_ws = nullptr; arc = attn_bwd(a, P[l.o].warena_off); }
       RC(arc);
     }
-    wq.push(dqkv, 3 * inner, b.xn1, d, M, 3 * inner, d, G(l.q));
+    RC(wq.push(dqkv, 3 * inner, b.xn1, d, M, 3 * inner, d, G(l.q), st));
     RC(linear_dgrad(c, dqkv, 3 * inner, M, 3 * inner, P[l.q].warena_off, d, e->dxn, KLAB_F32));
     {
       const bool first = (i == 0);
@@ -1313,6 +1363,7 @@
   e->frozen_valid = false;
   e->seg1_zeroed = e->dbias_zeroed[0] = e->dbias_zeroed[1] = e->denc_in_dxn = false;
   e->bias_ready[0] = e->bias_ready[1] = e->bias_ready[2] = e->dec_embed_ready = e->inv_n_ready = e->kv_wgrad_done = false;
+  e->wplan.valid = false;
   e->loss_out = nullptr;
   e->forced_armed = ForcedTable();
   e->attn_armed = AttnMaps();
@@ -2140,6 +2191,64 @@
                                hipMemcpyDeviceToDevice, (hipStream_t)stream);
 }
 
+static void wgrad_write_plan(klab_engine* e) {
+  klab_engine::WritePlan& w = e->wplan;
+  const klab_t5_cfg& cfg = e->cfg.main;
+  const auto& P = e->P[2];
+  const long d = cfg.d_model, inner = (long)cfg.n_heads * cfg.d_kv, ff = cfg.d_ff;
+  w = klab_engine::WritePlan();
+  w.graph = e->use_graph; w.kv = e->dkv_all != nullptr;
+  w.head_store = wgrad_store_on() && !e->use_graph && e->mi.head >= 0 && P[e->mi.head].grad_off >= 0;
+  if (w.head_store) w.stored.push_back({P[e->mi.head].grad_off, (long)cfg.vocab * d});
+  for (int stk = 0; stk < 2; ++stk) {
+    const bool dec = stk == 1;
+    const std::vector<T5LayerIdx>& L = dec ? e->mi.dec : e->mi.enc;
+    const WgradRelease rel = wgrad_release_plan(e, cfg, (int)L.size(), dec, dec && e->dkv_all != nullptr, e->G[2]);
+    w.store[stk] = rel.store;
+    for (size_t i = 0; i < L.size(); ++i) {
+      if (!rel.store[i]) continue;
+      const T5LayerIdx& l = L[i];
+      w.stored.push_back({P[l.wo].grad_off, d * ff});
+      w.stored.push_back({P[l.wi].grad_off, (cfg.ffn_gated ? 2 * ff : ff) * d});
+      w.stored.push_back({P[l.o].grad_off, d * inner});
+      w.stored.push_back({P[l.q].grad_off, 3 * inner * d});
+      if (dec) {
+        w.stored.push_back({P[l.co].grad_off, d * inner});
+        w.stored.push_back({P[l.cq].grad_off, inner * d});
+        if (rel.kv_in_queue) w.stored.push_back({e->kvall_g_off + (long)i * 2 * inner * d, 2 * inner * d});
+      }
+    }
+  }
+  std::sort(w.stored.begin(), w.stored.end());
+  w.any_store = !w.stored.empty();
+  for (int seg = 0; seg < 2; ++seg) {
+    const long end = e->seg_off[seg] + e->seg_len[seg];
+    long cur = e->seg_off[seg];
+    for (const auto& s : w.stored) {
+      if (s.first + s.second <= cur || s.first >= end) continue;
+      if (s.first > cur) w.clear[seg].push_back({cur, s.first - cur});
+      cur = s.first + s.second;
+    }
+    if (cur < end) w.clear[seg].push_back({cur, end - cur});
+  }
+  w.valid = true;
+}
+static bool wgrad_write_plan_current(const klab_engine* e) {
+  return e->wplan.valid && e->wplan.graph == e->use_graph && e->wplan.kv == (e->dkv_all != nullptr);
+}
+static int clear_planned(klab_engine* e, int seg_lo, int seg_hi, bool with_dbias, hipStream_t s) {
+  std::vector<float*> zp;
+  std::vector<long> zn;
+  for (int seg = seg_lo; seg <= seg_hi; ++seg)
+    for (const auto& r : e->wplan.clear[seg]) { zp.push_back(e->G[2] + r.first); zn.push_back(r.second); }
+  if (with_dbias) {
+    const long H = e->cfg.main.n_heads;
+    zp.push_back((float*)e->dec.dbias); zn.push_back(H * e->Lt * e->Lt);
+    zp.push_back((float*)e->enc.dbias); zn.push_back(H * e->Le * e->Le);
+  }
+  return klab::zero_ranges(zp.data(), zn.data(), (int)zp.size(), s);
+}
+
 static int backward_segment(klab_engine* e, int segment, const float* dloss_dev, void* stream) {
   Ctx c{e, (hipStream_t)stream, e->cfg.dtype, e->es};
   const klab_model_cfg& cfg = e->cfg;
@@ -2154,14 +2263,21 @@
     Ctx cs{e, e->side, c.dt, c.es};
     static const bool zero_side = klab::env_on("KLAB_ZERO_ON_SIDE");
     const bool zside = zero_side && !e->use_graph;
+    if (!wgrad_write_plan_current(e)) wgrad_write_plan(e);
+    const bool ranged = e->wplan.any_store;
     if (zside) {
       RC(side_after_main(c));
-      RC((int)hipMemsetAsync(Gm + e->seg_off[0], 0, (size_t)e->seg_len[0] * 4, e->side));
-      RC((int)hipMemsetAsync(Gm + e->seg_off[1], 0, (size_t)e->seg_len[1] * 4, e->side));
-      RC((int)hipMemsetAsync(e->dec.dbias, 0, (size_t)cfg.main.n_heads * e->Lt * e->Lt * 4, e->side));
-      RC((int)hipMemsetAsync(e->enc.dbias, 0, (size_t)cfg.main.n_heads * e->Le * e->Le * 4, e->side));
+      if (ranged) RC(clear_planned(e, 0, 1, true, e->side));
+      else {
+        RC((int)hipMemsetAsync(Gm + e->seg_off[0], 0, (size_t)e->seg_len[0] * 4, e->side));
+        RC((int)hipMemsetAsync(Gm + e->seg_off[1], 0, (size_t)e->seg_len[1] * 4, e->side));
+        RC((int)hipMemsetAsync(e->dec.dbias, 0, (size_t)cfg.main.n_heads * e->Lt * e->Lt * 4, e->side));
+        RC((int)hipMemsetAsync(e->enc.dbias, 0, (size_t)cfg.main.n_heads * e->Le * e->Le * 4, e->side));
+      }
       RC((int)hipEventRecord(e->ev_zero, e->side));
       e->seg1_zeroed = e->dbias_zeroed[0] = e->dbias_zeroed[1] = true;
+    } else if (ranged) {
+      RC(clear_planned(e, 0, 0, false, c.s));
     } else {
       RC((int)hipMemsetAsync(Gm + e->seg_off[0], 0, (size_t)e->seg_len[0] * 4, c.s));
     }
@@ -2175,7 +2291,7 @@
     RC(side_after_main(c));
     {
       klab_gemm_args g = G0(cs, V, d, Md, e->logits, V, 0, e->dec.out_t, d, 0, Gm + e->P[2][e->mi.head].grad_off, d, KLAB_F32);
-      g.alpha = alpha; g.alpha_dev = dloss_dev; g.accumulate = 1; g.atomic_ok = 1;
+      g.alpha = alpha; g.alpha_dev = dloss_dev; g.accumulate = e->wplan.head_store ? 0 : 1; g.atomic_ok = 1;
       RC(klab_gemm(&g, cs.ws()));
     }
     float* dh0 = nullptr;
@@ -2193,7 +2309,9 @@
   }
   if (segment == 1) {
     e->ev_next = 0;
+    if (!wgrad_write_plan_current(e)) { wgrad_write_plan(e); e->seg1_zeroed = false; }
     if (e->seg1_zeroed) e->seg1_zeroed = false;
+    else if (e->wplan.any_store) RC(clear_planned(e, 1, 1, false, c.s));
     else RC((int)hipMemsetAsync(Gm + e->seg_off[1], 0, (size_t)e->seg_len[1] * 4, c.s));
     const int Me = B * e->Le;
     if (e->denc_in_dxn) e->denc_in_dxn = false;
diff --git a/klab_multimodalmodel_amd/csrc/gemm.hip b/klab_multimodalmodel_amd/csrc/gemm.hip
--- a/klab_multimodalmodel_amd/csrc/gemm.hip
+++ b/klab_multimodalmodel_amd/csrc/gemm.hip
@@ -238,7 +238,7 @@
   const int nt = kt1 - kt0;                                                             \
   if (nt <= 0) return;
 
-template <int BM, int BN, bool AK, bool BKM, bool ATOMIC>
+template <int BM, int BN, bool AK, bool BKM, bool ATOMIC, bool MAY_STORE = false>
 __device__ __forceinline__ void gemm_glds_body(const GemmP& p, const int bid = blockIdx.x) {
   typedef bf16_t T;
   constexpr int WTM = BM / 2, WTN = BN / 2, MI = WTM / 16, NI = WTN / 16;
@@ -261,6 +261,8 @@
   if (p.alpha_dev) alpha *= p.alpha_dev[0];
   if constexpr (ATOMIC) {
     float* Cf = reinterpret_cast<float*>(p.C);
+    bool store = false;
+    if constexpr (MAY_STORE) store = !p.accumulate;
 #pragma unroll
     for (int i = 0; i < MI; ++i)
 #pragma unroll
@@ -270,7 +272,9 @@
 #pragma unroll
         for (int r = 0; r < 4; ++r) {
           const int m = bm0 + wm + i * 16 + (lane >> 4) * 4 + r;
-          if (m < p.M) atomicAdd(Cf + (long)m * p.ldc + n, acc[i][j][r] * alpha);
+          if (m >= p.M) continue;
+          if (store) Cf[(long)m * p.ldc + n] = acc[i][j][r] * alpha;
+          else atomicAdd(Cf + (long)m * p.ldc + n, acc[i][j][r] * alpha);
         }
       }
   } else {
@@ -309,7 +313,7 @@
 template <int BM, int BN, bool AK, bool BKM, bool ATOMIC>
 __global__ __launch_bounds__(256) void gemm_glds_kernel(GemmP p) { gemm_glds_body<BM, BN, AK, BKM, ATOMIC>(p); }
 
-struct GroupEntry { const void* A; long lda; const void* B; long ldb; float* C; long ldc; int M, N, K, splits, start; float alpha; };
+struct GroupEntry { const void* A; long lda; const void* B; long ldb; float* C; long ldc; int M, N, K, splits, start; float alpha; int accumulate; };
 struct GroupP { GroupEntry e[8]; int n; };
 template <int BN>
 __global__ __launch_bounds__(256) void gemm_glds_grouped_tn_kernel(GroupP g) {
@@ -321,11 +325,11 @@
   GemmP p;
   p.M = e.M; p.N = e.N; p.K = e.K;
   p.A = e.A; p.lda = e.lda; p.a_kmajor = 0; p.B = e.B; p.ldb = e.ldb; p.b_kmajor = 0;
-  p.C = e.C; p.ldc = e.ldc; p.c_f32 = 1; p.accumulate = 1;
+  p.C = e.C; p.ldc = e.ldc; p.c_f32 = 1; p.accumulate = e.accumulate;
   p.alpha = e.alpha; p.alpha_dev = nullptr; p.bias = nullptr; p.act = 0;
   p.aux = nullptr; p.ldaux = 0; p.aux_mode = 0; p.aux_scale = 1.f; p.residual = nullptr; p.ldr = 0; p.r_f32 = 1;
-  p.drop_p = 0.f; p.seed = nullptr; p.tag = 0; p.splits = e.splits; p.epi = 0;
-  gemm_glds_body<128, BN, false, false, true>(p, (int)blockIdx.x - e.start);
+  p.drop_p = 0.f; p.seed = nullptr; p.tag = 0; p.splits = e.accumulate ? e.splits : 1; p.epi = 0;
+  gemm_glds_body<128, BN, false, false, true, true>(p, (int)blockIdx.x - e.start);
 }
 
 template <typename T, int BM, int BN, bool AK, bool BKM, bool ATOMIC>
@@ -778,7 +782,7 @@
   g.n = 0;
   int blocks = 0;
   auto fits = [&](const klab_gemm_args* a) {
-    return a->dtype == KLAB_BF16 && !a->a_kmajor && !a->b_kmajor && a->c_dtype == KLAB_F32 && a->accumulate && a->atomic_ok &&
+    return a->dtype == KLAB_BF16 && !a->a_kmajor && !a->b_kmajor && a->c_dtype == KLAB_F32 && a->atomic_ok &&
            !a->bias && !a->act && !a->aux && !a->residual && a->drop_p == 0.f && !a->alpha_dev && a->name_tag == 0 && a->M >= 128 &&
            a->N >= 64 && (a->K % 32) == 0 && a->K >= 512 && !(a->M & 7) && !(a->N & 7) && !(a->lda & 7) && !(a->ldb & 7) &&
            !((uintptr_t)a->A & 15) && !((uintptr_t)a->B & 15) && !((uintptr_t)a->C & 15);
@@ -817,10 +821,10 @@
     long sp = (nt + per_wg / 2) / per_wg;
     if (sp > nt / 16) sp = nt / 16;
     if (sp > 16) sp = 16;
-    if (sp < 1) sp = 1;
+    if (sp < 1 || !a->accumulate) sp = 1;
     GroupEntry& e = g.e[g.n];
     e.A = a->A; e.lda = a->lda; e.B = a->B; e.ldb = a->ldb; e.C = (float*)a->C; e.ldc = a->ldc;
-    e.M = a->M; e.N = a->N; e.K = a->K; e.splits = (int)sp; e.start = blocks; e.alpha = a->alpha;
+    e.M = a->M; e.N = a->N; e.K = a->K; e.splits = (int)sp; e.start = blocks; e.alpha = a->alpha; e.accumulate = a->accumulate ? 1 : 0;
     blocks += (int)(t * sp);
     if (++g.n == 8) { const int rc = flush(); if (rc) return rc; }
   }
diff --git a/klab_multimodalmodel_amd/csrc/misc.hip b/klab_multimodalmodel_amd/csrc/misc.hip
--- a/klab_multimodalmodel_amd/csrc/misc.hip
+++ b/klab_multimodalmodel_amd/csrc/misc.hip
@@ -468,6 +468,37 @@
   return (unsigned)g;
 }
 
+struct ZeroRangesP { float* p[ZERO_RANGES_MAX]; long n[ZERO_RANGES_MAX]; };
+__global__ __launch_bounds__(256) void zero_ranges_kernel(ZeroRangesP r) {
+  float* p = r.p[blockIdx.y];
+  const long n = r.n[blockIdx.y];
+  long head = (long)((16 - ((uintptr_t)p & 15)) & 15) / 4;
+  if (head > n) head = n;
+  const long n4 = (n - head) / 4;
+  const long tid = (long)blockIdx.x * blockDim.x + threadIdx.x, step = (long)gridDim.x * blockDim.x;
+  f32x4* p4 = reinterpret_cast<f32x4*>(p + head);
+  for (long g = tid; g < n4; g += step) p4[g] = f32x4{0.f, 0.f, 0.f, 0.f};
+  if (tid < head) p[tid] = 0.f;
+  const long tail0 = head + n4 * 4;
+  if (tid < n - tail0) p[tail0 + tid] = 0.f;
+}
+int zero_ranges(float* const* ptrs, const long* counts, int n, hipStream_t s) {
+  for (int i0 = 0; i0 < n; i0 += ZERO_RANGES_MAX) {
+    ZeroRangesP r;
+    int m = 0;
+    long longest = 0;
+    for (int i = i0; i < n && m < ZERO_RANGES_MAX; ++i) {
+      if (!ptrs[i] || counts[i] <= 0) continue;
+      r.p[m] = ptrs[i]; r.n[m] = counts[i]; ++m;
+      if (counts[i] > longest) longest = counts[i];
+    }
+    if (!m) continue;
+    hipLaunchKernelGGL(zero_ranges_kernel, dim3(stream_grid(longest / 4 + 1), (unsigned)m), dim3(256), 0, s, r);
+    KLAB_LAUNCH_CHECK();
+  }
+  return KLAB_OK;
+}
+
 }
 
 using namespace klab;
diff --git a/klab_multimodalmodel_amd/csrc/mm8p.hip b/klab_multimodalmodel_amd/csrc/mm8p.hip
--- a/klab_multimodalmodel_amd/csrc/mm8p.hip
+++ b/klab_multimodalmodel_amd/csrc/mm8p.hip
@@ -377,7 +377,7 @@
 template <bool AK, bool BKM, bool ATOMIC>
 __global__ __launch_bounds__(512) void mm8p_kernel(GemmP p) { mm8p_body<AK, BKM, ATOMIC>(p, blockIdx.x); }
 
-struct Group8Entry { const void* A; long lda; const void* B; long ldb; float* C; long ldc; int M, N, K, start; float alpha; };
+struct Group8Entry { const void* A; long lda; const void* B; long ldb; float* C; long ldc; int M, N, K, start; float alpha; int accumulate; };
 constexpr int GROUP_MAX = 32;
 struct Group8P { Group8Entry e[GROUP_MAX]; int n; };
 __global__ __launch_bounds__(512) void mm8p_grouped_tn_kernel(Group8P g) {
@@ -390,7 +390,7 @@
   p.M = e.M; p.N = e.N; p.K = e.K;
   p.A = e.A; p.lda = e.lda; p.a_kmajor = 0;
   p.B = e.B; p.ldb = e.ldb; p.b_kmajor = 0;
-  p.C = e.C; p.ldc = e.ldc; p.c_f32 = 1; p.accumulate = 1;
+  p.C = e.C; p.ldc = e.ldc; p.c_f32 = 1; p.accumulate = e.accumulate;
   p.alpha = e.alpha; p.alpha_dev = nullptr; p.bias = nullptr; p.act = 0;
   p.aux = nullptr; p.ldaux = 0; p.aux_mode = 0; p.aux_scale = 1.f;
   p.residual = nullptr; p.ldr = 0; p.r_f32 = 1;
@@ -409,14 +409,14 @@
   int blocks = 0;
   for (int i = 0; i < n; ++i) {
     const klab_gemm_args* a = &list[i];
-    const bool ok = a->dtype == KLAB_BF16 && !a->a_kmajor && !a->b_kmajor && a->c_dtype == KLAB_F32 && a->accumulate && !a->bias && !a->act &&
+    const bool ok = a->dtype == KLAB_BF16 && !a->a_kmajor && !a->b_kmajor && a->c_dtype == KLAB_F32 && !a->bias && !a->act &&
                     !a->aux && !a->residual && a->drop_p == 0.f && !a->alpha_dev && a->M >= 128 && a->N >= 128 && (a->K % BK) == 0 &&
                     a->K >= 1024 && !(a->M & 7) && !(a->N & 7) && !(a->lda & 7) && !(a->ldb & 7) && !(a->ldc & 3) &&
                     !((uintptr_t)a->A & 15) && !((uintptr_t)a->B & 15) && !((uintptr_t)a->C & 15);
     if (!ok) return KLAB_ERR_UNSUPPORTED;
     Group8Entry& e = g.e[g.n++];
     e.A = a->A; e.lda = a->lda; e.B = a->B; e.ldb = a->ldb; e.C = (float*)a->C; e.ldc = a->ldc;
-    e.M = a->M; e.N = a->N; e.K = a->K; e.start = blocks; e.alpha = a->alpha;
+    e.M = a->M; e.N = a->N; e.K = a->K; e.start = blocks; e.alpha = a->alpha; e.accumulate = a->accumulate ? 1 : 0;
     blocks += ((a->M + BM - 1) / BM) * ((a->N + BN - 1) / BN);
   }
   const size_t epi_bytes = (size_t)128 * SLAB_PITCH;
```

Measured after the change: 12130 samples/s (median of 6 runs). 1.6% higher.
